# qope/starky-bn254

Hardware: AMD Instinct MI355X
Metric: G1 scalar-mult proofs/sec at trace height 2^16 (higher is better)
Workload: dtype u64

## Files before the change

starky_bn254_amd/csrc/kernels.cuh:

```cuda
#pragma once
#include "poseidon.cuh"
#include "air.cuh"

#include "kernels_ntt.cuh"

__global__ void pow_table_kernel(u64* out, size_t n, u64 base) {
  size_t i = (size_t)blockIdx.x * blockDim.x + threadIdx.x;
  if (i < n) out[i] = f_pow(F(base), i).v;
}
__global__ void shift_odd_table_kernel(u64* out, size_t n, const u64* __restrict__ shift, const u64* __restrict__ tw, u32 log_s) {
  size_t i = (size_t)blockIdx.x * blockDim.x + threadIdx.x;
  if (i < n) out[i] = (F(shift[i]) * F(tw[(i >> log_s) << log_s])).v;
}
__global__ void scale_pow_kernel(u64* v, size_t n, u64 base) {
  size_t i = (size_t)blockIdx.x * blockDim.x + threadIdx.x;
  if (i < n) v[i] = (F(v[i]) * f_pow(F(base), i)).v;
}

__global__ __launch_bounds__(256) __attribute__((amdgpu_waves_per_eu(4))) void leaf_hash_kernel(const u64* __restrict__ lde, size_t m, u32 lde_log, u32 ncols,
                                                        u64* __restrict__ digests) {
  size_t row = (size_t)blockIdx.x * blockDim.x + threadIdx.x;
  if (row >= m) return;
  F s[12];
#pragma unroll
  for (int i = 0; i < 12; i++) s[i] = F(0);
  size_t leaf = bitrev32((u32)row, lde_log);
  if (ncols <= 4) {
    for (u32 c = 0; c < 4; c++) digests[leaf * 4 + c] = c < ncols ? lde[(size_t)c * m + row] : 0;
    return;
  }
  for (u32 c = 0; c < ncols; c += 8) {
#pragma unroll
    for (u32 i = 0; i < 8; i++)
      if (c + i < ncols) s[i] = F(lde[(size_t)(c + i) * m + row]);
    poseidon_permute_keep(s, c + 8 >= ncols ? P_KEEP_DIGEST : (c + 16 <= ncols ? P_KEEP_CAPACITY : P_KEEP_ALL));
  }
#pragma unroll
  for (int i = 0; i < 4; i++) digests[leaf * 4 + i] = s[i].v;
}

__global__ __launch_bounds__(256) void merkle_level_kernel(const u64* __restrict__ child, u64* __restrict__ parent, size_t nparent) {
  size_t i = (size_t)blockIdx.x * blockDim.x + threadIdx.x;
  if (i >= nparent) return;
  F s[12];
#pragma unroll
  for (int k = 0; k < 8; k++) s[k] = F(child[i * 8 + k]);
#pragma unroll
  for (int k = 8; k < 12; k++) s[k] = F(0);
  poseidon_permute_keep(s, P_KEEP_DIGEST);
#pragma unroll
  for (int k = 0; k < 4; k++) parent[i * 4 + k] = s[k].v;
}

__global__ __launch_bounds__(256) __attribute__((amdgpu_waves_per_eu(4))) void leaf_absorb_kernel(const u64* __restrict__ lde_chunk, size_t m, u32 lde_log, u32 ncols_chunk,
                                                          u64* __restrict__ state, int first, int last, u64* __restrict__ digests, int next_full) {
  size_t row = (size_t)blockIdx.x * blockDim.x + threadIdx.x;
  if (row >= m) return;
  F s[12];
#pragma unroll
  for (int i = 0; i < 12; i++) s[i] = F(0);
  if (!first) {
#pragma unroll
    for (int i = 8; i < 12; i++) s[i] = F(state[(size_t)i * m + row]);
    if (ncols_chunk < 8) {
#pragma unroll
      for (int i = 0; i < 8; i++) s[i] = F(state[(size_t)i * m + row]);
    }
  }
  for (u32 c = 0; c < ncols_chunk; c += 8) {
#pragma unroll
    for (u32 i = 0; i < 8; i++)
      if (c + i < ncols_chunk) s[i] = F(lde_chunk[(size_t)(c + i) * m + row]);
    const bool end = c + 8 >= ncols_chunk;
    const int keep = end ? (last ? P_KEEP_DIGEST : (next_full ? P_KEEP_CAPACITY : P_KEEP_ALL)) : (c + 16 <= ncols_chunk ? P_KEEP_CAPACITY : P_KEEP_ALL);
    poseidon_permute_keep(s, keep);
  }
  u32 tid = threadIdx.x;
  asm volatile("" : "+v"(tid));
  const size_t row2 = (size_t)blockIdx.x * blockDim.x + tid;
  if (last) {
    size_t leaf = bitrev32((u32)row2, lde_log);
#pragma unroll
    for (int i = 0; i < 4; i++) digests[leaf * 4 + i] = s[i].v;
  } else {
#pragma unroll
    for (int i = 8; i < 12; i++) state[(size_t)i * m + row2] = s[i].v;
    if (!next_full) {
#pragma unroll
      for (int i = 0; i < 8; i++) state[(size_t)i * m + row2] = s[i].v;
    }
  }
}

static constexpr u32 MERKLE_SUBTREE_THREADS = 256;
__global__ __launch_bounds__(MERKLE_SUBTREE_THREADS) void merkle_subtree_kernel(u64* __restrict__ tree, size_t nleaf, u32 l0, u32 nlev, u32 nchild) {
  __shared__ u64 buf[2 * 256 * 4];
  const u32 tid = threadIdx.x, nt = blockDim.x;
  const u64* child = tree + (2 * nleaf - ((2 * nleaf) >> l0)) * 4;
  size_t base = (size_t)blockIdx.x * nchild;
  for (u32 e = tid; e < nchild * 4; e += nt) buf[e] = child[base * 4 + e];
  __syncthreads();
  u32 active = nchild / 2;
  const u32 groups = nt / 16, grp = tid / 16, lane = tid & 15;
  for (u32 lv = 1; lv <= nlev; lv++) {
    u64* out = tree + (2 * nleaf - ((2 * nleaf) >> (l0 + lv))) * 4;
    const size_t idx0 = ((size_t)blockIdx.x * nchild) >> lv;
    if (active > 4 * groups) {
      F s[12];
      if (tid < active) {
#pragma unroll
        for (int k = 0; k < 8; k++) s[k] = F(buf[tid * 8 + k]);
#pragma unroll
        for (int k = 8; k < 12; k++) s[k] = F(0);
        poseidon_permute_keep(s, P_KEEP_DIGEST);
      }
      __syncthreads();
      if (tid < active) {
#pragma unroll
        for (int k = 0; k < 4; k++) { buf[tid * 4 + k] = s[k].v; out[(idx0 + tid) * 4 + k] = s[k].v; }
      }
      __syncthreads();
    } else {
      u64 res[4];
      u32 nit = (active + groups - 1) / groups;
      for (u32 it = 0; it < nit; it++) {
        u32 parent = it * groups + grp;
        if (it * groups + (tid / 64) * 4 >= active) break;
        const u32 e = lane < 12 ? lane : lane - 12;
        u64 v = (parent < active && e < 8) ? buf[parent * 8 + e] : 0;
        res[it] = poseidon_permute_coop16(v, lane);
      }
      __syncthreads();
      for (u32 it = 0; it < nit; it++) {
        u32 parent = it * groups + grp;
        if (parent < active && lane < 4) { buf[parent * 4 + lane] = res[it]; out[(idx0 + parent) * 4 + lane] = res[it]; }
      }
      __syncthreads();
    }
    active >>= 1;
  }
}

__global__ __launch_bounds__(256) void merkle_level_thread_kernel(u64* __restrict__ tree, size_t nleaf, u32 l) {
  const size_t parents = nleaf >> (l + 1);
  const size_t i = (size_t)blockIdx.x * blockDim.x + threadIdx.x;
  if (i >= parents) return;
  const u64* child = tree + (2 * nleaf - ((2 * nleaf) >> l)) * 4;
  u64* out = tree + (2 * nleaf - ((2 * nleaf) >> (l + 1))) * 4;
  F s[12];
#pragma unroll
  for (int k = 0; k < 8; k++) s[k] = F(child[i * 8 + k]);
#pragma unroll
  for (int k = 8; k < 12; k++) s[k] = F(0);
  poseidon_permute_keep(s, P_KEEP_DIGEST);
#pragma unroll
  for (int k = 0; k < 4; k++) out[i * 4 + k] = s[k].v;
}
__global__ __launch_bounds__(256) void merkle_level_coop_kernel(u64* __restrict__ tree, size_t nleaf, u32 l) {
  const size_t parents = nleaf >> (l + 1);
  const size_t parent = ((size_t)blockIdx.x * blockDim.x + threadIdx.x) >> 4;
  const u32 lane = threadIdx.x & 15, e = lane < 12 ? lane : lane - 12;
  const u64* child = tree + (2 * nleaf - ((2 * nleaf) >> l)) * 4;
  u64* out = tree + (2 * nleaf - ((2 * nleaf) >> (l + 1))) * 4;
  const u64 v = (parent < parents && e < 8) ? child[parent * 8 + e] : 0;
  const u64 r = poseidon_permute_coop16(v, lane);
  if (parent < parents && lane < 4) out[parent * 4 + lane] = r;
}

__global__ __launch_bounds__(256) void fri_leaf_hash_kernel(const u64* __restrict__ va, const u64* __restrict__ vb, u32 log_m, u32 arity_bits,
                                                            u64* __restrict__ digests) {
  size_t leaf = (size_t)blockIdx.x * blockDim.x + threadIdx.x;
  size_t nleaf = (size_t)1 << (log_m - arity_bits);
  if (leaf >= nleaf) return;
  if (arity_bits == 1) {
    const u32 n0 = bitrev32((u32)(leaf * 2), log_m), n1 = bitrev32((u32)(leaf * 2 + 1), log_m);
    digests[leaf * 4 + 0] = va[n0]; digests[leaf * 4 + 1] = vb[n0]; digests[leaf * 4 + 2] = va[n1]; digests[leaf * 4 + 3] = vb[n1];
    return;
  }
  F s[12];
#pragma unroll
  for (int i = 0; i < 12; i++) s[i] = F(0);
  u32 arity = 1u << arity_bits;
  for (u32 t = 0; t < arity; t += 4) {
#pragma unroll
    for (u32 u = 0; u < 4; u++) {
      u32 nat = bitrev32((u32)(leaf * arity + t + u), log_m);
      s[2 * u] = F(va[nat]); s[2 * u + 1] = F(vb[nat]);
    }
    poseidon_permute_keep(s, t + 4 >= arity ? P_KEEP_DIGEST : P_KEEP_CAPACITY);
  }
#pragma unroll
  for (int i = 0; i < 4; i++) digests[leaf * 4 + i] = s[i].v;
}

__global__ __launch_bounds__(256) void fri_leaf_hash_coop_kernel(const u64* __restrict__ va, const u64* __restrict__ vb, u32 log_m, u32 arity_bits,
                                                                 u64* __restrict__ digests) {
  const size_t leaf = ((size_t)blockIdx.x * blockDim.x + threadIdx.x) >> 4;
  const size_t nleaf = (size_t)1 << (log_m - arity_bits);
  const u32 lane = threadIdx.x & 15, e = lane < 12 ? lane : lane - 12;
  const u32 arity = 1u << arity_bits;
  if (arity_bits == 1) {
    if (leaf < nleaf && lane < 4) {
      const u32 nat = bitrev32((u32)(leaf * 2 + (lane >> 1)), log_m);
      digests[leaf * 4 + lane] = (lane & 1) ? vb[nat] : va[nat];
    }
    return;
  }
  u64 st = 0;
  for (u32 t = 0; t < arity; t += 4) {
    if (leaf < nleaf && e < 8) {
      const u32 nat = bitrev32((u32)(leaf * arity + t + (e >> 1)), log_m);
      st = (e & 1) ? vb[nat] : va[nat];
    }
    st = poseidon_permute_coop16(st, lane);
  }
  if (leaf < nleaf && lane < 4) digests[leaf * 4 + lane] = st;
}

__global__ void field_mul_batch_kernel(const u64* a, const u64* b, u64* out, size_t count, int mode) {
  size_t i = (size_t)blockIdx.x * blockDim.x + threadIdx.x;
  if (i >= count) return;
#if defined(__HIP_DEVICE_COMPILE__)
  out[i] = mode ? nw::canon(nw::canon(nw::mul(a[i], b[i]))) : (F(a[i]) * F(b[i])).v;
#endif
}
__global__ void poseidon_batch_kernel(u64* states, size_t count) {
  size_t i = (size_t)blockIdx.x * blockDim.x + threadIdx.x;
  if (i >= count) return;
  F s[12];
  for (int k = 0; k < 12; k++) s[k] = F(states[i * 12 + k]);
  poseidon_permute(s);
  for (int k = 0; k < 12; k++) states[i * 12 + k] = s[k].v;
}

struct PairCols { int lhs, rhs; };

__device__ __forceinline__ F wave_scan_mul(F x, int lane) {
#pragma unroll
  for (int d = 1; d < 64; d <<= 1) {
    u64 o = __shfl_up((unsigned long long)x.v, d, 64);
    if (lane >= d) x = x * F(o);
  }
  return x;
}

template <int PZ_E>
__global__ __launch_bounds__(256) void permutation_z_kernel(const u64* __restrict__ trace, size_t n, const PairCols* __restrict__ pairs,
                                                            u64 gamma0, u64 gamma1, u64* __restrict__ zout) {
  __shared__ u64 wtot[4];
  __shared__ u64 carry_s;
  const int z = blockIdx.x;
  const u64* lhs = trace + (size_t)pairs[z].lhs * n;
  const u64* rhs = trace + (size_t)pairs[z].rhs * n;
  u64* zc = zout + (size_t)z * n;
  const int tid = threadIdx.x, lane = tid & 63, wv = tid >> 6;
  const F g0(gamma0), g1(gamma1);
  F carry(1), dprod(1);
  for (size_t base = 0; base < n; base += 256 * PZ_E) {
    const size_t i0 = base + (size_t)tid * PZ_E;
    u64 lv[PZ_E], rv[PZ_E];
#pragma unroll
    for (int e = 0; e < PZ_E; e++) { lv[e] = lhs[i0 + e]; rv[e] = rhs[i0 + e]; }
    F pr[PZ_E];
#pragma unroll
    for (int e = 0; e < PZ_E; e++) {
      const F l(lv[e]), r(rv[e]);
      const F num = (l + g0) * (l + g1);
      pr[e] = e ? pr[e - 1] * num : num;
      dprod = dprod * ((r + g0) * (r + g1));
    }
    F inc = wave_scan_mul(pr[PZ_E - 1], lane);
    if (lane == 63) wtot[wv] = inc.v;
    __syncthreads();
    F pre = carry;
    for (int w = 0; w < wv; w++) pre = pre * F(wtot[w]);
    const u64 prev = __shfl_up((unsigned long long)inc.v, 1, 64);
    const F excl = lane == 0 ? pre : pre * F(prev);
    zc[i0] = excl.v;
#pragma unroll
    for (int e = 1; e < PZ_E; e++) zc[i0 + e] = (excl * pr[e - 1]).v;
    carry = carry * F(wtot[0]) * F(wtot[1]) * F(wtot[2]) * F(wtot[3]);
    __syncthreads();
  }
  {
    F w = dprod;
#pragma unroll
    for (int d = 32; d >= 1; d >>= 1) w = w * F(__shfl_xor((unsigned long long)w.v, d, 64));
    if (lane == 0) wtot[wv] = w.v;
    __syncthreads();
    if (tid == 0) carry_s = f_inv(F(wtot[0]) * F(wtot[1]) * F(wtot[2]) * F(wtot[3])).v;
    __syncthreads();
  }
  carry = F(carry_s);
  __syncthreads();
  for (size_t base = n; base > 0; base -= 256 * PZ_E) {
    const size_t i0 = base - 1 - (size_t)tid * PZ_E;
    u64 rv[PZ_E], zv[PZ_E];
#pragma unroll
    for (int e = 0; e < PZ_E; e++) { rv[e] = rhs[i0 - e]; zv[e] = zc[i0 - e]; }
    F pr[PZ_E];
#pragma unroll
    for (int e = 0; e < PZ_E; e++) {
      const F r(rv[e]);
      const F den = (r + g0) * (r + g1);
      pr[e] = e ? pr[e - 1] * den : den;
    }
    F inc = wave_scan_mul(pr[PZ_E - 1], lane);
    if (lane == 63) wtot[wv] = inc.v;
    __syncthreads();
    F pre = carry;
    for (int w = 0; w < wv; w++) pre = pre * F(wtot[w]);
    const u64 prev = __shfl_up((unsigned long long)inc.v, 1, 64);
    const F excl = lane == 0 ? pre : pre * F(prev);
#pragma unroll
    for (int e = 0; e < PZ_E; e++) zc[i0 - e] = (F(zv[e]) * (excl * pr[e])).v;
    carry = carry * F(wtot[0]) * F(wtot[1]) * F(wtot[2]) * F(wtot[3]);
    __syncthreads();
  }
}

#include "kernels_quotient.cuh"
__global__ __launch_bounds__(256) void quotient_combine_kernel(QuotientParams p) {
  size_t i = (size_t)blockIdx.x * blockDim.x + threadIdx.x;
  if (i >= p.m) return;
  F dinv(p.zh_inv[((i << p.row_shift) | p.row_rho) & 1]);
#pragma unroll
  for (int j = 0; j < SBN_NCH; j++) {
    F acc(p.part[((size_t)(QSEG - 1) * SBN_NCH + j) * p.m + i]);
#pragma unroll
    for (u32 sgm = 0; sgm + 1 < QSEG; sgm++) acc += F(p.part[((size_t)sgm * SBN_NCH + j) * p.m + i]) * F(p.seg_shift[sgm][j]);
    p.qout[(size_t)j * p.m + i] = (acc * dinv).v;
  }
}

__global__ void domain_tables_kernel(u64* xs, u64* lag_first, u64* lag_last, size_t m, u32 lde_log, u32 degree_bits) {
  size_t i = (size_t)blockIdx.x * blockDim.x + threadIdx.x;
  if (i >= m) return;
  F w = f_root_of_unity(lde_log);
  F x = F(GL_GEN) * f_pow(w, i);
  F g = f_root_of_unity(degree_bits);
  F nn = F((u64)1 << degree_bits);
  F zx = f_exp_pow2(x, degree_bits) - F(1);
  xs[i] = x.v;
  lag_first[i] = (zx * f_inv(nn * (x - F(1)))).v;
  lag_last[i] = (zx * f_inv(nn * (g * x - F(1)))).v;
}

__device__ __forceinline__ F wave_scan_mul_rev(F x, int lane) {
#pragma unroll
  for (int d = 1; d < 64; d <<= 1) {
    u64 o = __shfl_down((unsigned long long)x.v, d, 64);
    if (lane + d < 64) x = x * F(o);
  }
  return x;
}
template <int PZ_E>
__global__ __launch_bounds__(256) void permz_chunk_products_kernel(const u64* __restrict__ trace, size_t n, const PairCols* __restrict__ pairs, u64 gamma0, u64 gamma1,
                                                                   u64* __restrict__ tot) {
  __shared__ u64 wn[4], wd[4];
  const int z = blockIdx.y;
  const size_t c = blockIdx.x, chunks = gridDim.x;
  const int tid = threadIdx.x, lane = tid & 63, wv = tid >> 6;
  const size_t i0 = c * 256 * PZ_E + (size_t)tid * PZ_E;
  const u64* lhs = trace + (size_t)pairs[z].lhs * n + i0;
  const u64* rhs = trace + (size_t)pairs[z].rhs * n + i0;
  const F g0(gamma0), g1(gamma1);
  u64 lv[PZ_E], rv[PZ_E];
#pragma unroll
  for (int e = 0; e < PZ_E; e++) { lv[e] = lhs[e]; rv[e] = rhs[e]; }
  F pn(1), pd(1);
#pragma unroll
  for (int e = 0; e < PZ_E; e++) { const F l(lv[e]), r(rv[e]); pn = pn * ((l + g0) * (l + g1)); pd = pd * ((r + g0) * (r + g1)); }
#pragma unroll
  for (int d = 32; d >= 1; d >>= 1) { pn = pn * F(__shfl_xor((unsigned long long)pn.v, d, 64)); pd = pd * F(__shfl_xor((unsigned long long)pd.v, d, 64)); }
  if (lane == 0) { wn[wv] = pn.v; wd[wv] = pd.v; }
  __syncthreads();
  if (tid == 0) {
    tot[((size_t)z * chunks + c) * 2] = (F(wn[0]) * F(wn[1]) * F(wn[2]) * F(wn[3])).v;
    tot[((size_t)z * chunks + c) * 2 + 1] = (F(wd[0]) * F(wd[1]) * F(wd[2]) * F(wd[3])).v;
  }
}
__global__ __launch_bounds__(64) void permz_chunk_scan_kernel(const u64* __restrict__ tot, u32 chunks, u64* __restrict__ pq) {
  const int z = blockIdx.x, lane = threadIdx.x;
  const u64* t = tot + (size_t)z * chunks * 2;
  u64* o = pq + (size_t)z * chunks * 2;
  F carry(1), all(1);
  for (u32 b = 0; b < chunks; b += 64) {
    const u32 idx = b + lane;
    const bool on = idx < chunks;
    const F inc = wave_scan_mul(on ? F(t[2 * idx]) : F(1), lane);
    const u64 pv = __shfl_up((unsigned long long)inc.v, 1, 64);
    if (on) o[2 * idx] = (lane == 0 ? carry : carry * F(pv)).v;
    carry = carry * F(__shfl((unsigned long long)inc.v, 63, 64));
    F d = on ? F(t[2 * idx + 1]) : F(1);
#pragma unroll
    for (int k = 32; k >= 1; k >>= 1) d = d * F(__shfl_xor((unsigned long long)d.v, k, 64));
    all = all * d;
  }
  F carry_s = f_inv(all);
  for (u32 b = ((chunks - 1) / 64) * 64;; b -= 64) {
    const u32 idx = b + lane;
    const bool on = idx < chunks;
    const F inc = wave_scan_mul_rev(on ? F(t[2 * idx + 1]) : F(1), lane);
    const u64 sv = __shfl_down((unsigned long long)inc.v, 1, 64);
    if (on) o[2 * idx + 1] = (lane == 63 ? carry_s : carry_s * F(sv)).v;
    carry_s = carry_s * F(__shfl((unsigned long long)inc.v, 0, 64));
    if (b == 0) break;
  }
}
template <int PZ_E>
__global__ __launch_bounds__(256) void permz_chunk_write_kernel(const u64* __restrict__ trace, size_t n, const PairCols* __restrict__ pairs, u64 gamma0, u64 gamma1,
                                                                const u64* __restrict__ pq, u64* __restrict__ zout) {
  __shared__ u64 wn[4], wd[4];
  const int z = blockIdx.y;
  const size_t c = blockIdx.x, chunks = gridDim.x;
  const int tid = threadIdx.x, lane = tid & 63, wv = tid >> 6;
  const size_t i0 = c * 256 * PZ_E + (size_t)tid * PZ_E;
  const u64* lhs = trace + (size_t)pairs[z].lhs * n + i0;
  const u64* rhs = trace + (size_t)pairs[z].rhs * n + i0;
  u64* zc = zout + (size_t)z * n + i0;
  const F g0(gamma0), g1(gamma1);
  u64 lv[PZ_E], rv[PZ_E];
#pragma unroll
  for (int e = 0; e < PZ_E; e++) { lv[e] = lhs[e]; rv[e] = rhs[e]; }
  F pn[PZ_E], sd[PZ_E];
#pragma unroll
  for (int e = 0; e < PZ_E; e++) { const F l(lv[e]); const F num = (l + g0) * (l + g1); pn[e] = e ? pn[e - 1] * num : num; }
#pragma unroll
  for (int e = PZ_E - 1; e >= 0; e--) { const F r(rv[e]); const F den = (r + g0) * (r + g1); sd[e] = e < PZ_E - 1 ? sd[e + 1] * den : den; }
  const F incn = wave_scan_mul(pn[PZ_E - 1], lane), incd = wave_scan_mul_rev(sd[0], lane);
  if (lane == 63) wn[wv] = incn.v;
  if (lane == 0) wd[wv] = incd.v;
  __syncthreads();
  F pre(pq[((size_t)z * chunks + c) * 2]), suf(pq[((size_t)z * chunks + c) * 2 + 1]);
  for (int w = 0; w < wv; w++) pre = pre * F(wn[w]);
  for (int w = 3; w > wv; w--) suf = suf * F(wd[w]);
  const u64 pv = __shfl_up((unsigned long long)incn.v, 1, 64), sv = __shfl_down((unsigned long long)incd.v, 1, 64);
  const F exn = lane == 0 ? pre : pre * F(pv);
  const F exd = lane == 63 ? suf : suf * F(sv);
  const F both = exn * exd;
  zc[0] = (both * sd[0]).v;
#pragma unroll
  for (int e = 1; e < PZ_E; e++) zc[e] = (both * pn[e - 1] * sd[e]).v;
}

__global__ void ext_pow_table_kernel(u64* pa, u64* pb, size_t n, u64 z0, u64 z1) {
  size_t i = (size_t)blockIdx.x * blockDim.x + threadIdx.x;
  if (i >= n) return;
  E2 r = e2_pow(E2(F(z0), F(z1)), i);
  pa[i] = r.a.v; pb[i] = r.b.v;
}
__device__ __forceinline__ F block_sum(F v, u64* sh) {
  const int lane = threadIdx.x & 63, wv = threadIdx.x >> 6;
#pragma unroll
  for (int d = 32; d >= 1; d >>= 1) v = v + F(__shfl_xor((unsigned long long)v.v, d, 64));
  __syncthreads();
  if (lane == 0) sh[wv] = v.v;
  __syncthreads();
  F t(0);
  for (unsigned w = 0; w < blockDim.x / 64; w++) t = t + F(sh[w]);
  return t;
}
template <u32 OPEN_UNROLL>
__global__ __launch_bounds__(256) void openings_kernel(const u64* __restrict__ coeffs, size_t n, const u64* __restrict__ pa0, const u64* __restrict__ pb0,
                                                       const u64* __restrict__ pa1, const u64* __restrict__ pb1, u64* __restrict__ out) {
  __shared__ u64 sh[4];
  const u64* c = coeffs + (size_t)blockIdx.x * n;
  Acc<F> s0, r0, s1, r1;
  s0.clear(); r0.clear(); s1.clear(); r1.clear();
  for (size_t i = threadIdx.x; i < n; i += 256 * OPEN_UNROLL) {
    u64 cv[OPEN_UNROLL], t0[OPEN_UNROLL], t1[OPEN_UNROLL], t2[OPEN_UNROLL], t3[OPEN_UNROLL];
#pragma unroll
    for (u32 k = 0; k < OPEN_UNROLL; k++) {
      const size_t ik = i + 256 * k;
      cv[k] = c[ik]; t0[k] = pa0[ik]; t1[k] = pb0[ik]; t2[k] = pa1[ik]; t3[k] = pb1[ik];
    }
    __builtin_amdgcn_sched_barrier(0);
#pragma unroll
    for (u32 k = 0; k < OPEN_UNROLL; k++) {
      const F v{cv[k]};
      s0.macv(v, F(t0[k])); r0.macv(v, F(t1[k]));
      s1.macv(v, F(t2[k])); r1.macv(v, F(t3[k]));
    }
  }
  const F a0 = block_sum(s0.value(), sh), b0 = block_sum(r0.value(), sh), a1 = block_sum(s1.value(), sh), b1 = block_sum(r1.value(), sh);
  if (threadIdx.x == 0) {
    u64* o = out + (size_t)blockIdx.x * 4;
    o[0] = a0.v; o[1] = b0.v; o[2] = a1.v; o[3] = b1.v;
  }
}

template <u32 OPEN_UNROLL>
__global__ __launch_bounds__(256) void openings1_kernel(const u64* __restrict__ coeffs, size_t n, const u64* __restrict__ pa, const u64* __restrict__ pb,
                                                        u64* __restrict__ out, u32 off) {
  __shared__ u64 sh[4];
  const u64* c = coeffs + (size_t)blockIdx.x * n;
  Acc<F> s0, r0;
  s0.clear(); r0.clear();
  for (size_t i = threadIdx.x; i < n; i += 256 * OPEN_UNROLL) {
    u64 cv[OPEN_UNROLL], t0[OPEN_UNROLL], t1[OPEN_UNROLL];
#pragma unroll
    for (u32 k = 0; k < OPEN_UNROLL; k++) {
      const size_t ik = i + 256 * k;
      cv[k] = c[ik]; t0[k] = pa[ik]; t1[k] = pb[ik];
    }
    __builtin_amdgcn_sched_barrier(0);
#pragma unroll
    for (u32 k = 0; k < OPEN_UNROLL; k++) {
      const F v{cv[k]};
      s0.macv(v, F(t0[k])); r0.macv(v, F(t1[k]));
    }
  }
  const F a0 = block_sum(s0.value(), sh), b0 = block_sum(r0.value(), sh);
  if (threadIdx.x == 0) {
    u64* o = out + (size_t)blockIdx.x * 4 + off;
    o[0] = a0.v; o[1] = b0.v;
  }
}

__global__ __launch_bounds__(256) void fri_combine_partial_kernel(const u64* __restrict__ coeffs, size_t n, u32 npoly, u32 group_size,
                                                                  const u64* __restrict__ pa, const u64* __restrict__ pb, u64* __restrict__ part_a,
                                                                  u64* __restrict__ part_b) {
  size_t i = (size_t)blockIdx.x * blockDim.x + threadIdx.x;
  if (i >= n) return;
  const u32 g = blockIdx.y;
  const u32 j0 = g * group_size, cnt = j0 + group_size < npoly ? group_size : npoly - j0;
  const u64* c = coeffs + (size_t)j0 * n + i;
  Acc<F> a, b;
  a.clear(); b.clear();
  u32 k = 0;
  for (; k + 8 <= cnt; k += 8) {
    u64 f[8];
#pragma unroll
    for (u32 u = 0; u < 8; u++) f[u] = c[(size_t)(k + u) * n];
#pragma unroll
    for (u32 u = 0; u < 8; u++) { const F v(f[u]); a.mac(v, F(pa[k + u])); b.mac(v, F(pb[k + u])); }
  }
  for (; k < cnt; k++) { const F v(c[(size_t)k * n]); a.mac(v, F(pa[k])); b.mac(v, F(pb[k])); }
  part_a[(size_t)g * n + i] = a.value().v; part_b[(size_t)g * n + i] = b.value().v;
}
__global__ void fri_combine_reduce_kernel(const u64* part_a, const u64* part_b, size_t n, u32 ngroups, const u64* w, u64* out_a, u64* out_b, int accumulate) {
  size_t i = (size_t)blockIdx.x * blockDim.x + threadIdx.x;
  if (i >= n) return;
  E2 acc = accumulate ? E2(F(out_a[i]), F(out_b[i])) : E2(F(0), F(0));
  for (u32 g = 0; g < ngroups; g++) acc += E2(F(part_a[(size_t)g * n + i]), F(part_b[(size_t)g * n + i])) * E2(F(w[2 * g]), F(w[2 * g + 1]));
  out_a[i] = acc.a.v; out_b[i] = acc.b.v;
}

static constexpr u32 DBL_CHUNK = 16;
__global__ __launch_bounds__(256) void divide_by_linear_pass1(const u64* __restrict__ ca, const u64* __restrict__ cb, size_t nchunks, u64 z0, u64 z1,
                                                              u64* __restrict__ ha, u64* __restrict__ hb) {
  const size_t t = (size_t)blockIdx.x * blockDim.x + threadIdx.x;
  if (t >= nchunks) return;
  const E2 z{F(z0), F(z1)};
  const size_t s = t * DBL_CHUNK;
  E2 h{F(0), F(0)};
  for (u32 k = DBL_CHUNK; k-- > 0;) h = h * z + E2(F(ca[s + k]), F(cb[s + k]));
  ha[t] = h.a.v; hb[t] = h.b.v;
}
template <u32 U> __device__ __forceinline__ void dbl_fold(const u64* ha, const u64* hb, size_t base, size_t per, const E2 zl, E2& g) {
  for (size_t j0 = per; j0 > 0; j0 -= U) {
    u64 va[U], vb[U];
#pragma unroll
    for (u32 k = 0; k < U; k++) { va[k] = ha[base + j0 - 1 - k]; vb[k] = hb[base + j0 - 1 - k]; }
#pragma unroll
    for (u32 k = 0; k < U; k++) g = E2(F(va[k]), F(vb[k])) + zl * g;
  }
}
template <u32 U> __device__ __forceinline__ void dbl_replay(u64* ha, u64* hb, size_t base, size_t per, const E2 zl, E2 carry) {
  for (size_t j0 = per; j0 > 0; j0 -= U) {
    u64 va[U], vb[U];
#pragma unroll
    for (u32 k = 0; k < U; k++) { va[k] = ha[base + j0 - 1 - k]; vb[k] = hb[base + j0 - 1 - k]; }
#pragma unroll
    for (u32 k = 0; k < U; k++) {
      ha[base + j0 - 1 - k] = carry.a.v; hb[base + j0 - 1 - k] = carry.b.v;
      carry = E2(F(va[k]), F(vb[k])) + zl * carry;
    }
  }
}
__global__ __launch_bounds__(256) void divide_by_linear_pass2(u64* __restrict__ ha, u64* __restrict__ hb, size_t nchunks, u64 z0, u64 z1) {
  __shared__ u64 sa[2][256], sb[2][256];
  const int tid = threadIdx.x;
  const int lanes = nchunks < 256 ? (int)nchunks : 256;
  const size_t per = nchunks / lanes, base = (size_t)tid * per;
  const bool live = tid < lanes;
  const E2 zl = e2_pow(E2{F(z0), F(z1)}, DBL_CHUNK);
  E2 g{F(0), F(0)};
  if (live) { if (per % 8 == 0) dbl_fold<8>(ha, hb, base, per, zl, g); else dbl_fold<1>(ha, hb, base, per, zl, g); }
  E2 m = e2_pow(zl, per);
  int cur = 0;
  sa[0][tid] = g.a.v; sb[0][tid] = g.b.v;
  __syncthreads();
  for (int d = 1; d < lanes; d <<= 1) {
    E2 v{F(sa[cur][tid]), F(sb[cur][tid])};
    if (tid + d < lanes) v = v + m * E2(F(sa[cur][tid + d]), F(sb[cur][tid + d]));
    sa[cur ^ 1][tid] = v.a.v; sb[cur ^ 1][tid] = v.b.v;
    m = m * m;
    cur ^= 1;
    __syncthreads();
  }
  E2 carry{F(0), F(0)};
  if (tid + 1 < lanes) carry = E2(F(sa[cur][tid + 1]), F(sb[cur][tid + 1]));
  if (live) { if (per % 8 == 0) dbl_replay<8>(ha, hb, base, per, zl, carry); else dbl_replay<1>(ha, hb, base, per, zl, carry); }
}
__global__ __launch_bounds__(256) void divide_by_linear_pass3(const u64* __restrict__ ca, const u64* __restrict__ cb, size_t nchunks, u64 z0, u64 z1,
                                                              const u64* __restrict__ ha, const u64* __restrict__ hb, u64 mul0, u64 mul1,
                                                              u64* __restrict__ oa, u64* __restrict__ ob, int accumulate, u32 times_x) {
  const size_t t = (size_t)blockIdx.x * blockDim.x + threadIdx.x;
  if (t >= nchunks) return;
  const E2 z{F(z0), F(z1)}, mul{F(mul0), F(mul1)};
  const size_t s = t * DBL_CHUNK, n = nchunks * DBL_CHUNK;
  E2 b{F(ha[t]), F(hb[t])};
  for (u32 k = DBL_CHUNK; k-- > 0;) {
    const size_t i = s + k;
    const E2 q = b;
    b = b * z + E2(F(ca[i]), F(cb[i]));
    const size_t j = i + times_x;
    if (j >= n) continue;
    const E2 o = accumulate ? E2(F(oa[j]), F(ob[j])) * mul + q : q;
    oa[j] = o.a.v; ob[j] = o.b.v;
  }
}

__global__ void fri_fold_kernel(const u64* ca, const u64* cb, size_t nout, u32 arity, u64 b0, u64 b1, u64* oa, u64* ob) {
  size_t i = (size_t)blockIdx.x * blockDim.x + threadIdx.x;
  if (i >= nout) return;
  E2 beta{F(b0), F(b1)}, acc(F(0), F(0));
  for (u32 t = arity; t-- > 0;) acc = acc * beta + E2(F(ca[i * arity + t]), F(cb[i * arity + t]));
  oa[i] = acc.a.v; ob[i] = acc.b.v;
}

struct PowParams { u64 state[12]; u32 wpos; u32 min_lz; u64 base; u64 count; u64* result; };
__global__ __launch_bounds__(256) void pow_kernel(PowParams p) {
  u64 gid = (u64)blockIdx.x * blockDim.x + threadIdx.x;
  if (gid >= p.count) return;
  F s[12];
#pragma unroll
  for (int i = 0; i < 12; i++) s[i] = F(p.state[i]);
  s[p.wpos] = F(p.base + gid);
  poseidon_permute(s);
  u64 resp = s[P_RATE - 1].v;
  u32 lz = resp ? (u32)__clzll((long long)resp) : 64;
  if (lz >= p.min_lz) atomicMin((unsigned long long*)p.result, (unsigned long long)(p.base + gid));
}

__global__ __launch_bounds__(256) void split_pack_kernel(const u64* __restrict__ lde, size_t m, u32 nc, u32 ob, u32 log_r, u32 me,
                                                         u64* __restrict__ send_l, u64* __restrict__ send_n, u64* __restrict__ self_l, u64* __restrict__ self_n) {
  const size_t i = (size_t)blockIdx.x * blockDim.x + threadIdx.x;
  const u32 c = blockIdx.y;
  if (i >= m || c >= nc) return;
  const u64 v = lde[(size_t)c * m + i];
  const size_t ml = m >> log_r, rmask = ((size_t)1 << log_r) - 1;
  const u32 s = bitrev32((u32)(i & rmask), log_r);
  if (s == me) self_l[(size_t)c * ml + (i >> log_r)] = v;
  else send_l[((size_t)s * ob + c) * ml + (i >> log_r)] = v;
  if (send_n) {
    const size_t p = (i + m - 2) & (m - 1);
    const u32 s2 = bitrev32((u32)(p & rmask), log_r);
    if (s2 == me) self_n[(size_t)c * ml + (p >> log_r)] = v;
    else send_n[((size_t)s2 * ob + c) * ml + (p >> log_r)] = v;
  }
}
__global__ void split_unpack_rows_kernel(const u64* __restrict__ in, size_t m, u32 nplanes, u32 log_r, u64* __restrict__ out) {
  const size_t i = (size_t)blockIdx.x * blockDim.x + threadIdx.x;
  if (i >= m) return;
  const size_t ml = m >> log_r;
  const u32 s = bitrev32((u32)(i & (((size_t)1 << log_r) - 1)), log_r);
  for (u32 p = 0; p < nplanes; p++) out[(size_t)p * m + i] = in[((size_t)s * nplanes + p) * ml + (i >> log_r)];
}
__global__ void split_modadd_kernel(const u64* __restrict__ in, size_t len, u32 nranks, u64* __restrict__ out) {
  const size_t k = (size_t)blockIdx.x * blockDim.x + threadIdx.x;
  if (k >= len) return;
  F acc(in[k]);
  for (u32 r = 1; r < nranks; r++) acc += F(in[(size_t)r * len + k]);
  out[k] = acc.v;
}

__global__ void gather_rows_kernel(const u64* mat, size_t m, u32 lde_log, u32 ncols, const u32* idx, u64* out, size_t qstride, size_t off) {
  u32 c = blockIdx.x * blockDim.x + threadIdx.x;
  u32 q = blockIdx.y;
  if (c >= ncols) return;
  size_t row = bitrev32(idx[q], lde_log);
  out[(size_t)q * qstride + off + c] = mat[(size_t)c * m + row];
}
__global__ void gather_siblings_kernel(const u64* tree, size_t nleaf, u32 nlevels, const u32* idx, u32 shift, u64* out, size_t qstride, size_t off) {
  u32 q = blockIdx.x;
  u32 e = threadIdx.x;
  if (e >= nlevels * 4) return;
  u32 l = e >> 2, k = e & 3;
  size_t x = idx[q] >> shift;
  size_t level_off = 2 * nleaf - ((2 * nleaf) >> l);
  size_t sib = (x >> l) ^ 1;
  out[(size_t)q * qstride + off + e] = tree[(level_off + sib) * 4 + k];
}
__global__ void gather_fri_leaf_kernel(const u64* va, const u64* vb, u32 log_m, u32 arity_bits, const u32* idx, u32 shift, u64* out, size_t qstride, size_t off) {
  u32 q = blockIdx.x;
  u32 e = threadIdx.x;
  u32 arity = 1u << arity_bits;
  if (e >= 2 * arity) return;
  size_t leaf = idx[q] >> shift;
  u32 nat = bitrev32((u32)(leaf * arity + (e >> 1)), log_m);
  out[(size_t)q * qstride + off + e] = (e & 1) ? vb[nat] : va[nat];
}

typedef unsigned long long u64x2_t __attribute__((ext_vector_type(2)));
__global__ __launch_bounds__(256) void first_non_canonical_kernel(const u64* __restrict__ w, size_t count, u64 base, unsigned long long* first_bad) {
  const size_t head = (((size_t)w & 8) && count) ? 1 : 0;
  const u64x2_t* __restrict__ v = reinterpret_cast<const u64x2_t*>(w + head);
  const size_t nvec = (count - head) >> 1;
  const size_t tid = (size_t)blockIdx.x * blockDim.x + threadIdx.x, stride = (size_t)gridDim.x * blockDim.x;
  u64 bad = ~(u64)0;
#pragma unroll 4
  for (size_t i = tid; i < nvec; i += stride) {
    const u64x2_t x = v[i];
    const bool b0 = x.x >= GLP, b1 = x.y >= GLP;
    if (b0 | b1) { const u64 j = head + 2 * i + (b0 ? 0 : 1); bad = bad < j ? bad : j; }
  }
  if (tid == 0) {
    const size_t last = head + 2 * nvec;
    if (last < count && w[last] >= GLP) bad = bad < last ? bad : last;
    if (head && w[0] >= GLP) bad = 0;
  }
  if (!__any(bad != ~(u64)0)) return;
  for (int d = 32; d >= 1; d >>= 1) { const u64 o = __shfl_xor((unsigned long long)bad, d, 64); bad = o < bad ? o : bad; }
  if ((threadIdx.x & 63) == 0) atomicMin(first_bad, (unsigned long long)(base + bad));
}
```

starky_bn254_amd/csrc/kernels_ntt.cuh:

```cuda
#pragma once
#include "gl.cuh"

struct NttPassParams {
  const u64* in; u64* out;
  size_t in_col_stride, out_col_stride;
  u32 log_r;
  u32 log_t;
  u32 log_n;
  size_t in_sr, in_st, out_sr, out_st;
  size_t n_in;
  u32 r_fast_load;
  u32 twiddle;
  const u64* tw;
  u32 tw_log;
  const u64* pre;
  const u64* post;
  u64 scale;
  const u64* pre2;
  u32 split;
  u32 xcd_order;
};

GL_HD F tw_lookup(const u64* tw, u32 tw_log, u64 e_of_order, u32 order_log) {
  u64 idx = (e_of_order << (tw_log - order_log)) & ((1ULL << tw_log) - 1);
  u64 half = 1ULL << (tw_log - 1);
  if (idx >= half) return -F(tw[idx - half]);
  return F(tw[idx]);
}

__device__ __forceinline__ u64 tw_full(const u64* __restrict__ tw, u32 tw_log, u32 e_of_order, u32 order_log) {
  return tw[(e_of_order << (tw_log - order_log)) & ((1u << tw_log) - 1u)];
}

static constexpr int NTT_THREADS = 256;

#ifdef SBN_NTT_KERNELS_HERE
__global__ __launch_bounds__(NTT_THREADS) void ntt_pass_kernel(NttPassParams p) {
  extern __shared__ u64 lds[];
  const u32 R = 1u << p.log_r, T = 1u << p.log_t;
  const u32 LDT = T + 1;
  const size_t col = blockIdx.y;
  const size_t t0 = (size_t)blockIdx.x << p.log_t;
  const u64* in = p.in + col * p.in_col_stride;
  u64* out = p.out + col * p.out_col_stride;
  const u32 total = R << p.log_t;
  for (u32 e = threadIdx.x; e < total; e += NTT_THREADS) {
    u32 r, t;
    if (p.r_fast_load) { r = e & (R - 1); t = e >> p.log_r; } else { t = e & (T - 1); r = e >> p.log_t; }
    size_t gi = (size_t)r * p.in_sr + (t0 + t) * p.in_st;
    u64 v = 0;
    if (gi < p.n_in) {
      v = in[gi];
      if (p.pre) v = (F(v) * F(p.pre[gi])).v;
    }
    lds[r * LDT + t] = v;
  }
  __syncthreads();
  for (u32 s = 0; s < p.log_r; s++) {
    u32 half = R >> (s + 1);
    u32 nb = total >> 1;
    for (u32 e = threadIdx.x; e < nb; e += NTT_THREADS) {
      u32 t = e & (T - 1), b = e >> p.log_t;
      u32 j = b & (half - 1), blk = b / half;
      u32 i0 = blk * 2 * half + j, i1 = i0 + half;
      F u{lds[i0 * LDT + t]}, v(lds[i1 * LDT + t]);
      F w = tw_lookup(p.tw, p.tw_log, (u64)j << s, p.log_r);
      lds[i0 * LDT + t] = (u + v).v;
      lds[i1 * LDT + t] = ((u - v) * w).v;
    }
    __syncthreads();
  }
  for (u32 e = threadIdx.x; e < total; e += NTT_THREADS) {
    u32 t = e & (T - 1), k = e >> p.log_t;
    u32 q = bitrev32(k, p.log_r);
    F v{lds[q * LDT + t]};
    if (p.twiddle) v = v * tw_lookup(p.tw, p.tw_log, (u64)k * (t0 + t), p.log_n);
    if (p.scale != 1) v = v * F(p.scale);
    size_t go = (size_t)k * p.out_sr + (t0 + t) * p.out_st;
    if (p.post) v = v * F(p.post[go]);
    out[go] = v.v;
  }
}
#else
__global__ void ntt_pass_kernel(NttPassParams p);
#endif

namespace nw {
#if !defined(SBN_NTT_CXX_ARITH)
using namespace gp;
__device__ __forceinline__ u64 repay_carry(u64 s, u64 k) { u64 k2, k3; u64 t = madm1(sel01(k), s, k2); return madm1(sel01(k2), t, k3); }
__device__ __forceinline__ u64 add(u64 a, u64 b) {
  u64 k1, k2; u32 lo = addco(lo32(a), lo32(b), k1); u32 hi = addc(hi32(a), hi32(b), k1, k2);
  return repay_carry(pack(lo, hi), k2);
}
__device__ __forceinline__ u64 sub(u64 a, u64 b) {
  u64 k1, k2, k3, k4, k5, k6;
  u32 lo = subco(lo32(a), lo32(b), k1); u32 hi = subb(hi32(a), hi32(b), k1, k2);
  u32 l2 = subco(lo, selm1(k2), k3); u32 h2 = subb0(hi, k3, k4);
  u32 l3 = subco(l2, selm1(k4), k5); u32 h3 = subb0(h2, k5, k6);
  return pack(l3, h3);
}
__device__ __forceinline__ u64 red32(u64 lo, u32 hi) { u64 k; u64 t = madm1(hi, lo, k); u64 k2; return madm1(sel01(k), t, k2); }
__device__ __forceinline__ u64 red(u64 lo, u64 hi) {
  u64 k1, k2, k3, k4, k5, k6;
  const u32 l = subco(lo32(lo), hi32(hi), k1), h = subb0(hi32(lo), k1, k2);
  const u32 t = subb0(lo32(hi), k2, k3);
  const u64 r = madm1(t, pack(l, h), k4);
  const u32 rl = addc(lo32(r), selm1(k4), k3, k5), rh = addc(hi32(r), 0u, k5, k6);
  return pack(rl, rh);
}
template <int E> __device__ __forceinline__ u64 mul_pow2(u64 x) {
  if constexpr (E == 0) return x;
  else if constexpr (E < 32) return red32(x << E, hi32(x) >> (32 - E));
  else if constexpr (E == 32) return red32(pack(0, lo32(x)), hi32(x));
  else if constexpr (E < 64) return red(pack(0, lo32(x) << (E - 32)), x >> (64 - E));
  else return mul_pow2<E - 48>(mul_pow2<48>(x));
}
__device__ __forceinline__ u64 mul(u64 a, u64 b) { return gl_mul_weak(a, b); }
__device__ __forceinline__ u64 canon(u64 x) { return gp::canon(x); }
#else
__device__ __forceinline__ u64 add(u64 a, u64 b) {
  u64 s = a + b;
  u64 c = s < a ? GLEPS : 0;
  s += c;
  if (s < c) s += GLEPS;
  return s;
}
__device__ __forceinline__ u64 sub(u64 a, u64 b) {
  u64 d = a - b;
  u64 c = a < b ? GLEPS : 0;
  u64 r = d - c;
  if (d < c) r -= GLEPS;
  return r;
}
__device__ __forceinline__ u64 red(u64 lo, u64 hi) {
  u32 hi_hi = (u32)(hi >> 32), hi_lo = (u32)hi;
  u64 t0 = lo - hi_hi;
  if (lo < hi_hi) t0 -= GLEPS;
  u64 t1 = ((u64)hi_lo << 32) - hi_lo;
  u64 r = t0 + t1;
  if (r < t1) r += GLEPS;
  return r;
}
template <int E> __device__ __forceinline__ u64 mul_pow2(u64 x) {
  if constexpr (E == 0) return x;
  else if constexpr (E < 64) return red(x << E, x >> (64 - E));
  else return mul_pow2<E - 48>(mul_pow2<48>(x));
}
__device__ __forceinline__ u64 mul(u64 a, u64 b) { return red(a * b, __umul64hi(a, b)); }
__device__ __forceinline__ u64 canon(u64 x) { return x >= GLP ? x - GLP : x; }
#endif

#define NW_BF(i, j, E) { u64 a_ = x[i], b_ = x[j]; x[i] = add(a_, b_); x[j] = mul_pow2<E>(sub(a_, b_)); }
__device__ __forceinline__ void dft16_rho(u64* x) {
  NW_BF(0, 8, 0) NW_BF(1, 9, 12) NW_BF(2, 10, 24) NW_BF(3, 11, 36) NW_BF(4, 12, 48) NW_BF(5, 13, 60) NW_BF(6, 14, 72) NW_BF(7, 15, 84)
  NW_BF(0, 4, 0) NW_BF(1, 5, 24) NW_BF(2, 6, 48) NW_BF(3, 7, 72) NW_BF(8, 12, 0) NW_BF(9, 13, 24) NW_BF(10, 14, 48) NW_BF(11, 15, 72)
  NW_BF(0, 2, 0) NW_BF(1, 3, 48) NW_BF(4, 6, 0) NW_BF(5, 7, 48) NW_BF(8, 10, 0) NW_BF(9, 11, 48) NW_BF(12, 14, 0) NW_BF(13, 15, 48)
  NW_BF(0, 1, 0) NW_BF(2, 3, 0) NW_BF(4, 5, 0) NW_BF(6, 7, 0) NW_BF(8, 9, 0) NW_BF(10, 11, 0) NW_BF(12, 13, 0) NW_BF(14, 15, 0)
}
#undef NW_BF
}

#ifdef SBN_NTT_KERNELS_HERE
template <int LOG_B>
__global__ __launch_bounds__(256) void ntt_fast_pass_kernel(NttPassParams p, u32 kperm) {
  extern __shared__ u64 lds[];
  constexpr u32 NB = 1u << LOG_B;
  constexpr u32 R = 256u << LOG_B;
  const size_t col = p.xcd_order ? blockIdx.x : blockIdx.y;
  const size_t t0 = (size_t)(p.xcd_order ? blockIdx.y : blockIdx.x) << 4;
  const u32 half = p.split ? blockIdx.z : 0u;
  const u64* __restrict__ pre = half ? p.pre2 : p.pre;
  const u64* in = p.in + col * p.in_col_stride;
  u64* out = p.out + col * p.out_col_stride;
  u32 g, t;
  if (p.r_fast_load) { g = threadIdx.x & 15; t = threadIdx.x >> 4; } else { t = threadIdx.x & 15; g = threadIdx.x >> 4; }
  const size_t tg = t0 + t;
  const u32 S1 = p.r_fast_load ? 257u : 272u;
  const u32 lane_off = p.r_fast_load ? (t * 16) : t;
  const u32 g_mul = p.r_fast_load ? 1u : 16u;
  u64 x[NB][16];
#pragma unroll
  for (u32 b = 0; b < NB; b++)
#pragma unroll
    for (u32 q = 0; q < 16; q++) {
      u32 r = g + 16 * q + 256 * b;
      size_t gi = (size_t)r * p.in_sr + tg * p.in_st;
      u64 v = 0;
      if (gi < p.n_in) {
        v = in[gi];
        if (pre) v = nw::mul(v, pre[gi]);
      }
      x[b][q] = v;
    }
  if (LOG_B == 1) {
    const bool upper_zero = p.in_st == 1 && (size_t)256 * p.in_sr >= p.n_in;
#pragma unroll
    for (u32 q = 0; q < 16; q++) {
      u32 r = g + 16 * q;
      u64 a = x[0][q], bb = x[NB - 1][q];
      u64 w = tw_full(p.tw, p.tw_log, r, 9);
      if (upper_zero) { x[NB - 1][q] = nw::mul(a, w); }
      else { x[0][q] = nw::add(a, bb); x[NB - 1][q] = nw::mul(nw::sub(a, bb), w); }
    }
  }
#pragma unroll
  for (u32 b = 0; b < NB; b++) {
    nw::dft16_rho(x[b]);
#pragma unroll
    for (u32 pidx = 0; pidx < 16; pidx++) {
      u32 m = __brev(pidx) >> 28;
      u32 k1 = (kperm * m) & 15;
      u64 v = x[b][pidx];
      if (g && k1) v = nw::mul(v, tw_full(p.tw, p.tw_log, (u32)(g * k1), 8));
      lds[(b * 16 + k1) * S1 + lane_off + g * g_mul] = v;
    }
  }
  __syncthreads();
  const u32 k1 = g;
#pragma unroll
  for (u32 b = 0; b < NB; b++) {
#pragma unroll
    for (u32 gp = 0; gp < 16; gp++) x[b][gp] = lds[(b * 16 + k1) * S1 + lane_off + gp * g_mul];
    nw::dft16_rho(x[b]);
#pragma unroll
    for (u32 pidx = 0; pidx < 16; pidx++) {
      u32 m = __brev(pidx) >> 28;
      u32 k2 = (kperm * m) & 15;
      u32 k256 = k1 + 16 * k2;
      u32 k = LOG_B == 0 ? k256 : (k256 * NB + b);
      if (LOG_B == 1) k = (k << p.split) + half;
      u64 v = x[b][pidx];
      if (p.twiddle) v = nw::mul(v, tw_full(p.tw, p.tw_log, (u32)(k * tg), p.log_n));
      if (p.scale != 1) v = nw::mul(v, p.scale);
      size_t go = (size_t)k * p.out_sr + tg * p.out_st;
      if (p.post) v = nw::mul(v, p.post[go]);
      out[go] = nw::canon(v);
    }
  }
  (void)R;
}
#else
template <int LOG_B> __global__ void ntt_fast_pass_kernel(NttPassParams p, u32 kperm);
#endif

struct NttFusedParams {
  const u64* in; size_t in_col_stride;
  u64* coef; size_t coef_col_stride;
  u64* out; size_t out_col_stride;
  size_t n1;
  u32 log_n;
  const u64* tw_i; const u64* tw_f; u32 tw_log;
  const u64* pre;
  u64 scale;
  const u64* pre2;
};
#ifdef SBN_NTT_KERNELS_HERE
__global__ __launch_bounds__(256) __attribute__((amdgpu_waves_per_eu(4))) void ntt_fused_inv_b_lde_a_kernel(NttFusedParams p) {
  extern __shared__ u64 lds[];
  const size_t col = blockIdx.x;
  const size_t t0 = (size_t)blockIdx.y << 4;
  const u64* in = p.in + col * p.in_col_stride;
  u64* coef = p.coef + col * p.coef_col_stride;
  u64* out = p.out + col * p.out_col_stride;
  const u32 g = threadIdx.x & 15, t = threadIdx.x >> 4;
  const size_t tg = t0 + t;
  u64 x[2][16];
#pragma unroll
  for (u32 q = 0; q < 16; q++) x[0][q] = in[(size_t)(g + 16 * q) + tg * 256];
  nw::dft16_rho(x[0]);
#pragma unroll
  for (u32 pidx = 0; pidx < 16; pidx++) {
    const u32 m = __brev(pidx) >> 28, k1 = (11u * m) & 15;
    u64 v = x[0][pidx];
    if (g && k1) v = nw::mul(v, tw_full(p.tw_i, p.tw_log, (u32)(g * k1), 8));
    lds[k1 * 257 + t * 16 + g] = v;
  }
  __syncthreads();
#pragma unroll
  for (u32 gp = 0; gp < 16; gp++) x[0][gp] = lds[g * 257 + t * 16 + gp];
  nw::dft16_rho(x[0]);
  u64 a[16];
#pragma unroll
  for (u32 pidx = 0; pidx < 16; pidx++) {
    const u32 m = __brev(pidx) >> 28, k2 = (11u * m) & 15;
    const u32 k = g + 16 * k2;
    const u64 v = nw::mul(x[0][pidx], p.scale);
    coef[(size_t)k * p.n1 + tg] = nw::canon(v);
    a[k2] = v;
  }
  __syncthreads();
#pragma unroll
  for (u32 q = 0; q < 16; q++) {
    const u32 r = g + 16 * q;
    const u64 v = nw::mul(a[q], p.pre[(size_t)r * p.n1 + tg]);
    x[0][q] = v;
    x[1][q] = nw::mul(v, tw_full(p.tw_f, p.tw_log, r, 9));
  }
#pragma unroll
  for (u32 b = 0; b < 2; b++) {
    nw::dft16_rho(x[b]);
#pragma unroll
    for (u32 pidx = 0; pidx < 16; pidx++) {
      const u32 m = __brev(pidx) >> 28, k1 = (5u * m) & 15;
      u64 v = x[b][pidx];
      if (g && k1) v = nw::mul(v, tw_full(p.tw_f, p.tw_log, (u32)(g * k1), 8));
      lds[(b * 16 + k1) * 272 + g * 17 + t] = v;
    }
  }
  __syncthreads();
  const u32 t2 = threadIdx.x & 15, k1o = threadIdx.x >> 4;
  const size_t tg2 = t0 + t2;
#pragma unroll
  for (u32 b = 0; b < 2; b++) {
#pragma unroll
    for (u32 gp = 0; gp < 16; gp++) x[b][gp] = lds[(b * 16 + k1o) * 272 + gp * 17 + t2];
    nw::dft16_rho(x[b]);
#pragma unroll
    for (u32 pidx = 0; pidx < 16; pidx++) {
      const u32 m = __brev(pidx) >> 28, k2 = (5u * m) & 15;
      const u32 k = (k1o + 16 * k2) * 2 + b;
      const u64 v = nw::mul(x[b][pidx], tw_full(p.tw_f, p.tw_log, (u32)(k * tg2), p.log_n + 1));
      out[(size_t)k * p.n1 + tg2] = nw::canon(v);
    }
  }
}
#else
__global__ void ntt_fused_inv_b_lde_a_kernel(NttFusedParams p);
#endif

#ifdef SBN_NTT_KERNELS_HERE
__global__ __launch_bounds__(256) __attribute__((amdgpu_waves_per_eu(4))) void ntt_fused512_inv_b_lde_a_kernel(NttFusedParams p) {
  extern __shared__ u64 lds[];
  const size_t col = blockIdx.x;
  const size_t t0 = (size_t)blockIdx.y << 4;
  const u64* in = p.in + col * p.in_col_stride;
  u64* coef = p.coef + col * p.coef_col_stride;
  u64* out = p.out + col * p.out_col_stride;
  const u32 g = threadIdx.x & 15, t = threadIdx.x >> 4;
  const size_t tg = t0 + t;
  u64 x[2][16];
#pragma unroll
  for (u32 q0 = 0; q0 < 16; q0 += 8) {
#pragma unroll
    for (u32 q = q0; q < q0 + 8; q++) {
      const u64 lo = in[(size_t)(g + 16 * q) + tg * 512], hi = in[(size_t)(g + 16 * q + 256) + tg * 512];
      x[0][q] = nw::add(lo, hi);
      x[1][q] = nw::mul(nw::sub(lo, hi), tw_full(p.tw_i, p.tw_log, g + 16 * q, 9));
    }
    asm volatile("" ::: "memory");
  }
#pragma unroll
  for (u32 b = 0; b < 2; b++) {
    nw::dft16_rho(x[b]);
#pragma unroll
    for (u32 pidx = 0; pidx < 16; pidx++) {
      const u32 m = __brev(pidx) >> 28, k1 = (11u * m) & 15;
      u64 v = x[b][pidx];
      if (g && k1) v = nw::mul(v, tw_full(p.tw_i, p.tw_log, (u32)(g * k1), 8));
      lds[(b * 16 + k1) * 257 + t * 16 + g] = v;
    }
  }
  __syncthreads();
#pragma unroll
  for (u32 b = 0; b < 2; b++) {
    u64 z[16];
#pragma unroll
    for (u32 gp = 0; gp < 16; gp++) z[gp] = lds[(b * 16 + g) * 257 + t * 16 + gp];
    nw::dft16_rho(z);
#pragma unroll
    for (u32 pidx = 0; pidx < 16; pidx++) {
      const u32 m = __brev(pidx) >> 28, k2 = (11u * m) & 15;
      const u64 v = nw::mul(z[pidx], p.scale);
      coef[(size_t)((g + 16 * k2) * 2 + b) * 512 + tg] = nw::canon(v);
      x[b][k2] = v;
    }
    asm volatile("" ::: "memory");
  }
  __syncthreads();
#pragma unroll 1
  for (u32 h = 0; h < 2; h++) {
    u32 t2 = threadIdx.x & 15, k1o = threadIdx.x >> 4;
    u32 gl = g, tl = t;
    asm volatile("" : "+v"(t2), "+v"(k1o), "+v"(gl), "+v"(tl));
    const size_t tg2 = t0 + t2, tgl = t0 + tl;
    const u64* __restrict__ pre = h ? p.pre2 : p.pre;
#pragma unroll
    for (u32 b = 0; b < 2; b++)
#pragma unroll
      for (u32 q0 = 0; q0 < 16; q0 += 8) {
#pragma unroll
        for (u32 q = q0; q < q0 + 8; q++) {
          const size_t ci = (size_t)(2 * (gl + 16 * q) + b) * 512 + tgl;
          u64 c = x[b][q];
          if (h) c = coef[ci];
          x[b][q] = nw::mul(c, pre[ci]);
        }
        asm volatile("" ::: "memory");
      }
#pragma unroll
    for (u32 b = 0; b < 2; b++) {
      nw::dft16_rho(x[b]);
#pragma unroll
      for (u32 pidx = 0; pidx < 16; pidx++) {
        const u32 m = __brev(pidx) >> 28, k1 = (5u * m) & 15;
        u64 v = x[b][pidx];
        if (gl && k1) v = nw::mul(v, tw_full(p.tw_f, p.tw_log, (u32)(gl * k1), 8));
        lds[(b * 16 + k1) * 272 + gl * 17 + tl] = v;
      }
    }
    __syncthreads();
#pragma unroll
    for (u32 b = 0; b < 2; b++) {
#pragma unroll
      for (u32 gp = 0; gp < 16; gp++) x[b][gp] = lds[(b * 16 + k1o) * 272 + gp * 17 + t2];
      nw::dft16_rho(x[b]);
    }
#pragma unroll
    for (u32 pidx = 0; pidx < 16; pidx++) {
      const u32 m = __brev(pidx) >> 28, k2 = (5u * m) & 15;
      const u32 j = k1o + 16 * k2;
      const u64 e = x[0][pidx], o = nw::mul(x[1][pidx], tw_full(p.tw_f, p.tw_log, j, 9));
      const u32 ka = 2 * j + h, kb = 2 * (j + 256) + h;
      out[(size_t)ka * 512 + tg2] = nw::canon(nw::mul(nw::add(e, o), tw_full(p.tw_f, p.tw_log, (u32)(ka * tg2), 19)));
      out[(size_t)kb * 512 + tg2] = nw::canon(nw::mul(nw::sub(e, o), tw_full(p.tw_f, p.tw_log, (u32)(kb * tg2), 19)));
    }
    __syncthreads();
  }
}
#else
__global__ void ntt_fused512_inv_b_lde_a_kernel(NttFusedParams p);
#endif
```

starky_bn254_amd/csrc/prover.hip:

```cpp
#include "prover_ctx.hpp"
#include "kernels.cuh"
#include <algorithm>
#include <cstring>
#include <cstdlib>
#include <thread>
#include <atomic>
#include <chrono>
#include <functional>

namespace sbn { thread_local std::string g_last_error; }

static std::atomic<int> g_default_device{0};
static thread_local int t_device = -1;
static inline int cur_device() { return t_device >= 0 ? t_device : g_default_device.load(); }
#define g_device (cur_device())
namespace sbn {
int current_device() { return cur_device(); }
int use_current_device(const char* why) {
  int ndev = 0;
  if (hipGetDeviceCount(&ndev) != hipSuccess || ndev == 0) return fail(SBN_ERR_NO_DEVICE, "no HIP device available: %s", why);
  HIPC(hipSetDevice(g_device));
  return 0;
}
}

static const char* STAGE_NAMES[ST_COUNT + EX_COUNT] = {
  "trace_commit", "perm_z", "z_commit", "quotient_eval", "quotient_commit",
  "openings", "fri_combine", "fri_layers", "pow", "queries",
  "trace_absorb_kernels_ms", "trace_absorb_launches", "z_absorb_kernels_ms", "z_absorb_launches", "device_tracegen_ms",
  "split_exchange_ms"};

static int dmalloc(u64** p, size_t words, size_t* bytes = nullptr) {
  HIPC(hipMalloc((void**)p, words * sizeof(u64)));
  if (bytes) *bytes += words * sizeof(u64);
  return 0;
}

static u32 pick_log_t(u32 log_r, u32 log_s) {
  u32 lt = 4;
  while (lt > 0 && ((size_t)(1u << log_r) * ((1u << lt) + 1) * 8) > 48 * 1024) lt--;
  return std::min(lt, log_s);
}
static int ntt_columns(sbn_prover* P, const u64* in, size_t in_cs, u64* out, size_t out_cs, u64* tmp, size_t tmp_cs, size_t ncols,
                       u32 log_n, bool inverse, size_t n_in, const u64* pre, const u64* post, u64 scale, hipStream_t st = nullptr, int which = 3) {
  if (ncols == 0) return 0;
  if (!st) st = P->stream;
  u32 log_n1 = (log_n + 1) / 2, log_n2 = log_n - log_n1;
  size_t n1 = (size_t)1 << log_n1, n2 = (size_t)1 << log_n2;
  NttPassParams a{};
  a.in = in; a.out = tmp; a.in_col_stride = in_cs; a.out_col_stride = tmp_cs;
  a.log_r = log_n1; a.log_t = pick_log_t(log_n1, log_n2); a.log_n = log_n;
  a.in_sr = n2; a.in_st = 1; a.out_sr = n2; a.out_st = 1; a.n_in = n_in;
  a.r_fast_load = 0; a.twiddle = 1; a.tw = inverse ? P->d_tw_i : P->d_tw_f; a.tw_log = P->lde_log;
  a.pre = pre; a.post = nullptr; a.scale = 1;
  NttPassParams b{};
  b.in = tmp; b.out = out; b.in_col_stride = tmp_cs; b.out_col_stride = out_cs;
  b.log_r = log_n2; b.log_t = pick_log_t(log_n2, log_n1); b.log_n = log_n;
  b.in_sr = 1; b.in_st = n2; b.out_sr = n1; b.out_st = 1; b.n_in = (size_t)1 << log_n;
  b.r_fast_load = 1; b.twiddle = 0; b.tw = a.tw; b.tw_log = P->lde_log;
  b.pre = nullptr; b.post = post; b.scale = scale;
  for (size_t c0 = 0; c0 < ncols; c0 += 32768) {
    size_t nc = std::min<size_t>(32768, ncols - c0);
    NttPassParams pa = a, pb = b;
    pa.in = a.in + c0 * in_cs; pa.out = a.out + c0 * tmp_cs;
    pb.in = b.in + c0 * tmp_cs; pb.out = b.out + c0 * out_cs;
    dim3 ga((unsigned)(n2 >> pa.log_t), (unsigned)nc), gb((unsigned)(n1 >> pb.log_t), (unsigned)nc);
    size_t la = ((size_t)1 << pa.log_r) * ((1u << pa.log_t) + 1) * 8, lb = ((size_t)1 << pb.log_r) * ((1u << pb.log_t) + 1) * 8;
    const u32 kperm = inverse ? 11u : 5u;
    auto launch = [&](NttPassParams q, dim3 grid, size_t lds_bytes) {
      const bool fast = q.log_t == 4 && (q.log_r == 8 || q.log_r == 9);
      if (fast) { q.xcd_order = 1; std::swap(grid.x, grid.y); }
      if (fast && q.log_r == 8) hipLaunchKernelGGL(ntt_fast_pass_kernel<0>, grid, dim3(256), 16 * 272 * 8, st, q, kperm);
      else if (fast) hipLaunchKernelGGL(ntt_fast_pass_kernel<1>, grid, dim3(256), 32 * 272 * 8, st, q, kperm);
      else hipLaunchKernelGGL(ntt_pass_kernel, grid, dim3(NTT_THREADS), lds_bytes, st, q);
    };
    if (pa.log_r == 9 && log_n2 >= 4) pa.log_t = 4;
    if (pb.log_r == 9 && log_n1 >= 4) pb.log_t = 4;
    const bool split_a = !inverse && pa.log_r == 10 && log_n2 >= 4 && pa.in_st == 1 && n_in <= (size_t)512 * pa.in_sr && pre == P->d_shift && P->d_shift_odd;
    if (split_a) { pa.log_r = 9; pa.log_t = 4; pa.split = 1; pa.pre2 = P->d_shift_odd; }
    ga = dim3((unsigned)(n2 >> pa.log_t), (unsigned)nc, split_a ? 2u : 1u); gb = dim3((unsigned)(n1 >> pb.log_t), (unsigned)nc);
    la = ((size_t)1 << pa.log_r) * ((1u << pa.log_t) + 1) * 8; lb = ((size_t)1 << pb.log_r) * ((1u << pb.log_t) + 1) * 8;
    if (which & 1) launch(pa, ga, la);
    if (which & 2) launch(pb, gb, lb);
  }
  HIPC(hipGetLastError());
  return 0;
}

static u64 host_inv_pow2(u32 k) { return f_inv(F((u64)1 << k)).v; }
static int ntt_fast_setup() {
  static std::atomic<bool> done[SBN_MAX_DEVICES];
  const int d = g_device >= 0 && g_device < SBN_MAX_DEVICES ? g_device : 0;
  if (!done[d].load()) {
    HIPC(hipFuncSetAttribute((const void*)ntt_fast_pass_kernel<1>, hipFuncAttributeMaxDynamicSharedMemorySize, 32 * 272 * 8));
    HIPC(hipFuncSetAttribute((const void*)ntt_fused_inv_b_lde_a_kernel, hipFuncAttributeMaxDynamicSharedMemorySize, 32 * 272 * 8));
    HIPC(hipFuncSetAttribute((const void*)ntt_fused512_inv_b_lde_a_kernel, hipFuncAttributeMaxDynamicSharedMemorySize, 32 * 272 * 8));
    done[d].store(true);
  }
  return 0;
}
static void ntt_plan(sbn_prover* P) {
  P->ntt_fused = P->degree_bits == 16 || P->degree_bits == 17;
  P->ntt_fused512 = P->degree_bits == 18 && P->lde_log == 19;
}

static int intt_values(sbn_prover* P, const u64* vals, u64* coef, size_t ncols) {
  for (size_t c0 = 0; c0 < ncols; c0 += P->ntt_chunk) {
    size_t nc = std::min(P->ntt_chunk, ncols - c0);
    int rc = ntt_columns(P, vals + c0 * P->n, P->n, coef + c0 * P->n, P->n, P->d_tmp, P->m, nc, P->degree_bits, true, P->n, nullptr, nullptr,
                         host_inv_pow2(P->degree_bits));
    if (rc) return rc;
  }
  return 0;
}
static int lde_coeffs(sbn_prover* P, const u64* coef, u64* lde, size_t ncols) {
  for (size_t c0 = 0; c0 < ncols; c0 += P->ntt_chunk) {
    size_t nc = std::min(P->ntt_chunk, ncols - c0);
    int rc = ntt_columns(P, coef + c0 * P->n, P->n, lde + c0 * P->m, P->m, P->d_tmp, P->m, nc, P->lde_log, false, P->n, P->d_shift, nullptr, 1);
    if (rc) return rc;
  }
  return 0;
}
static int intt_then_lde(sbn_prover* P, const u64* vals, u64* coef, u64* lde, size_t ncols) {
  for (size_t c0 = 0; c0 < ncols; c0 += P->ntt_chunk) {
    size_t nc = std::min(P->ntt_chunk, ncols - c0);
    int rc = ntt_columns(P, vals + c0 * P->n, P->n, coef + c0 * P->n, P->n, P->d_tmp, P->m, nc, P->degree_bits, true, P->n, nullptr, nullptr,
                         host_inv_pow2(P->degree_bits));
    if (rc) return rc;
    rc = ntt_columns(P, coef + c0 * P->n, P->n, lde + c0 * P->m, P->m, P->d_tmp, P->m, nc, P->lde_log, false, P->n, P->d_shift, nullptr, 1);
    if (rc) return rc;
  }
  return 0;
}

static int intt_lde_cols_fused(sbn_prover* P, const u64* v, u64* cf, u64* lde_out, size_t nc, u64* tmp2, hipStream_t lde_stream, hipEvent_t handoff) {
  int rc = ntt_columns(P, v, P->n, cf, P->n, P->d_tmp, P->m, nc, P->degree_bits, true, P->n, nullptr, nullptr, host_inv_pow2(P->degree_bits), nullptr, 1);
  if (rc) return rc;
  NttFusedParams f{};
  const u32 log_n1 = (P->degree_bits + 1) / 2;
  f.in = P->d_tmp; f.in_col_stride = P->m; f.coef = cf; f.coef_col_stride = P->n; f.out = tmp2; f.out_col_stride = P->m;
  f.n1 = (size_t)1 << log_n1; f.log_n = P->degree_bits; f.tw_i = P->d_tw_i; f.tw_f = P->d_tw_f; f.tw_log = P->lde_log; f.pre = P->d_shift; f.pre2 = P->d_shift_odd;
  f.scale = host_inv_pow2(P->degree_bits);
  if (P->ntt_fused512) hipLaunchKernelGGL(ntt_fused512_inv_b_lde_a_kernel, dim3((unsigned)nc, 32u), dim3(256), 32 * 272 * 8, P->stream, f);
  else hipLaunchKernelGGL(ntt_fused_inv_b_lde_a_kernel, dim3((unsigned)nc, (unsigned)(f.n1 >> 4)), dim3(256), 32 * 272 * 8, P->stream, f);
  if (lde_stream != P->stream) {
    HIPC(hipEventRecord(handoff, P->stream));
    HIPC(hipStreamWaitEvent(lde_stream, handoff, 0));
  }
  return ntt_columns(P, cf, P->n, lde_out, P->m, tmp2, P->m, nc, P->lde_log, false, P->n, P->d_shift, nullptr, 1, lde_stream, 2);
}
static int intt_lde_cols(sbn_prover* P, const u64* v, u64* cf, u64* lde_out, size_t nc) {
  if ((P->ntt_fused || P->ntt_fused512) && P->d_tmp2) return intt_lde_cols_fused(P, v, cf, lde_out, nc, P->d_tmp2, P->stream, nullptr);
  int rc = ntt_columns(P, v, P->n, cf, P->n, P->d_tmp, P->m, nc, P->degree_bits, true, P->n, nullptr, nullptr, host_inv_pow2(P->degree_bits));
  if (rc) return rc;
  return ntt_columns(P, cf, P->n, lde_out, P->m, P->d_tmp, P->m, nc, P->lde_log, false, P->n, P->d_shift, nullptr, 1);
}

static int tree_alloc(DevTree& t, size_t nleaf, u32 cap_height, size_t* bytes = nullptr) {
  t.nleaf = nleaf;
  u32 lg = 0; while (((size_t)1 << lg) < nleaf) lg++;
  t.nlevels = lg - cap_height;
  return dmalloc(&t.d, 2 * nleaf * 4, bytes);
}
static int tree_build_inner(sbn_prover* P, DevTree& t, hipStream_t st) {
  u32 l0 = 0;
  while (l0 < t.nlevels) {
    const size_t parents = t.nleaf >> (l0 + 1);
    if (parents <= 8192 && parents >= 16 && ((t.nleaf >> l0) % 32) == 0) {
      const u32 nlev = std::min<u32>(t.nlevels - l0, 5);
      hipLaunchKernelGGL(merkle_subtree_kernel, dim3((unsigned)((t.nleaf >> l0) / 32)), dim3(MERKLE_SUBTREE_THREADS), 0, st, t.d, t.nleaf, l0, nlev, 32u);
      l0 += nlev;
      continue;
    }
    if (parents >= 16384) {
      hipLaunchKernelGGL(merkle_level_thread_kernel, dim3((unsigned)((parents + 255) / 256)), dim3(256), 0, st, t.d, t.nleaf, l0);
      l0++;
    } else if (parents > 16) {
      hipLaunchKernelGGL(merkle_level_coop_kernel, dim3((unsigned)((parents * 16 + 255) / 256)), dim3(256), 0, st, t.d, t.nleaf, l0);
      l0++;
    } else {
      const size_t nodes = t.nleaf >> l0;
      u32 nchild = (u32)std::min<size_t>(512, nodes);
      u32 lg = 0; while ((2u << lg) < nchild) lg++;
      u32 nlev = std::min(t.nlevels - l0, lg + 1);
      hipLaunchKernelGGL(merkle_subtree_kernel, dim3((unsigned)(nodes / nchild)), dim3(MERKLE_SUBTREE_THREADS), 0, st, t.d, t.nleaf, l0, nlev, nchild);
      l0 += nlev;
    }
  }
  HIPC(hipGetLastError());
  return 0;
}
static int tree_from_matrix(sbn_prover* P, DevTree& t, const u64* lde, size_t ncols) {
  hipLaunchKernelGGL(leaf_hash_kernel, dim3((unsigned)((P->m + 255) / 256)), dim3(256), 0, P->stream, lde, P->m, P->lde_log, (u32)ncols, t.d);
  return tree_build_inner(P, t, P->stream);
}
struct HostUpload { const u64* src; hipEvent_t* done; };
static int upload_setup(sbn_prover* P) {
  if (!P->ustream) HIPC(hipStreamCreate(&P->ustream));
  for (auto& e : P->upload_done) if (!e) HIPC(hipEventCreateWithFlags(&e, hipEventDisableTiming));
  for (auto& e : P->slot_copied) if (!e) HIPC(hipEventCreateWithFlags(&e, hipEventDisableTiming));
  if (!P->h_ring) HIPC(hipHostMalloc((void**)&P->h_ring, UPLOAD_SLOTS * UPLOAD_SLOT_WORDS * sizeof(u64), hipHostMallocDefault));
  if (!P->h_first_bad) HIPC(hipHostMalloc((void**)&P->h_first_bad, sizeof(unsigned long long), hipHostMallocDefault));
  if (!P->d_first_bad) { HIPC(hipMalloc((void**)&P->d_first_bad, sizeof(unsigned long long))); P->dev_bytes += sizeof(unsigned long long); }
  return 0;
}
static void launch_first_non_canonical(const u64* d_words, size_t count, u64 base, unsigned long long* d_first_bad, hipStream_t st) {
  const size_t blocks = std::min<size_t>(std::max<size_t>((count / 2 + 255) / 256, 1), 2048);
  hipLaunchKernelGGL(first_non_canonical_kernel, dim3((unsigned)blocks), dim3(256), 0, st, d_words, count, base, d_first_bad);
}
static int upload_chunk(sbn_prover* P, const HostUpload& up, size_t k, size_t c0, size_t nc) {
  const size_t w0 = c0 * P->n, w1 = w0 + nc * P->n;
  const size_t threads = std::min<size_t>(tracegen_host_threads(), 16);
  for (size_t a = w0; a < w1; a += UPLOAD_SLOT_WORDS) {
    const size_t len = std::min(UPLOAD_SLOT_WORDS, w1 - a);
    const unsigned s = P->slot_next; P->slot_next = (s + 1) % UPLOAD_SLOTS;
    if (P->slot_used[s]) HIPC(hipEventSynchronize(P->slot_copied[s]));
    u64* slot = P->h_ring + (size_t)s * UPLOAD_SLOT_WORDS;
    const u64* from = up.src + a;
    const size_t parts = std::max<size_t>(1, std::min(threads, len >> 15)), per = (len + parts - 1) / parts;
    host_parallel_for(parts, [&](size_t t) { const size_t b0 = t * per, b1 = std::min(len, b0 + per); if (b0 < b1) memcpy(slot + b0, from + b0, (b1 - b0) * sizeof(u64)); });
    HIPC(hipMemcpyAsync(P->d_trace + a, slot, len * sizeof(u64), hipMemcpyHostToDevice, P->ustream));
    HIPC(hipEventRecord(P->slot_copied[s], P->ustream));
    P->slot_used[s] = true;
  }
  launch_first_non_canonical(P->d_trace + w0, w1 - w0, (u64)w0, P->d_first_bad, P->ustream);
  HIPC(hipGetLastError());
  HIPC(hipEventRecord(up.done[k], P->ustream));
  return 0;
}

static int commit_pipeline(sbn_prover* P, const u64* vals, u64* coef, u64* lde, size_t ncols, DevTree& t, int ex_ms, int ex_launches, const HostUpload* up = nullptr) {
  size_t ch = P->ntt_chunk;
  size_t nchunks = (ncols + ch - 1) / ch;
  if (nchunks > (size_t)MAX_CHUNKS) return fail(SBN_ERR_UNSUPPORTED, "too many column chunks");
  if (ncols <= 4) {
    if (up) {
      int rc = upload_chunk(P, *up, 0, 0, ncols);
      if (rc) return rc;
      HIPC(hipStreamWaitEvent(P->stream, up->done[0], 0));
    }
    int rc = intt_then_lde(P, vals, coef, lde, ncols);
    if (rc) return rc;
    P->stage_ms[ST_COUNT + ex_launches] = 0;
    return tree_from_matrix(P, t, lde, ncols);
  }
  for (size_t k = 0; k < nchunks; k++) {
    size_t c0 = k * ch, nc = std::min(ch, ncols - c0);
    int rc;
    if (up) {
      if ((rc = upload_chunk(P, *up, k, c0, nc))) return rc;
      HIPC(hipStreamWaitEvent(P->stream, up->done[k], 0));
    }
    if (P->ntt_two_streams && (P->ntt_fused || P->ntt_fused512) && P->d_tmp3) {
      if (k >= 2) HIPC(hipStreamWaitEvent(P->stream, P->chunk_ready[k - 2], 0));
      rc = intt_lde_cols_fused(P, vals + c0 * P->n, coef + c0 * P->n, lde + c0 * P->m, nc, (k & 1) ? P->d_tmp3 : P->d_tmp2, P->nstream, P->intt_done[k]);
      if (rc) return rc;
      HIPC(hipEventRecord(P->chunk_ready[k], P->nstream));
    } else if (P->ntt_two_streams && !P->ntt_fused && !P->ntt_fused512) {
      rc = ntt_columns(P, vals + c0 * P->n, P->n, coef + c0 * P->n, P->n, P->d_tmp, P->m, nc, P->degree_bits, true, P->n, nullptr, nullptr, host_inv_pow2(P->degree_bits));
      if (rc) return rc;
      HIPC(hipEventRecord(P->intt_done[k], P->stream));
      HIPC(hipStreamWaitEvent(P->nstream, P->intt_done[k], 0));
      rc = ntt_columns(P, coef + c0 * P->n, P->n, lde + c0 * P->m, P->m, P->d_tmp2, P->m, nc, P->lde_log, false, P->n, P->d_shift, nullptr, 1, P->nstream);
      if (rc) return rc;
      HIPC(hipEventRecord(P->chunk_ready[k], P->nstream));
    } else {
      rc = intt_lde_cols(P, vals + c0 * P->n, coef + c0 * P->n, lde + c0 * P->m, nc);
      if (rc) return rc;
      HIPC(hipEventRecord(P->chunk_ready[k], P->stream));
    }
    HIPC(hipStreamWaitEvent(P->hstream, P->chunk_ready[k], 0));
    HIPC(hipEventRecord(P->abs_ev[2 * k], P->hstream));
    hipLaunchKernelGGL(leaf_absorb_kernel, dim3((unsigned)((P->m + 255) / 256)), dim3(256), 0, P->hstream, lde + c0 * P->m, P->m, P->lde_log, (u32)nc,
                       P->d_sponge, k == 0 ? 1 : 0, k + 1 == nchunks ? 1 : 0, t.d,
                       (k + 1 < nchunks && std::min(ch, ncols - (c0 + nc)) >= 8) ? 1 : 0);
    HIPC(hipEventRecord(P->abs_ev[2 * k + 1], P->hstream));
  }
  int rc = tree_build_inner(P, t, P->hstream);
  if (rc) return rc;
  HIPC(hipEventRecord(P->hash_done, P->hstream));
  HIPC(hipStreamWaitEvent(P->stream, P->hash_done, 0));
  P->stage_ms[ST_COUNT + ex_launches] = (float)nchunks;
  (void)ex_ms;
  return 0;
}
static thread_local double t_wait_deadline_s = 0;
static inline void poll_backoff(unsigned spins) {
  if (spins < 2000) std::this_thread::yield();
  else std::this_thread::sleep_for(std::chrono::microseconds(spins < 20000 ? 20 : 200));
}
static inline hipError_t stream_wait(hipStream_t st) {
  if (t_wait_deadline_s <= 0) return hipStreamSynchronize(st);
  const auto t0 = std::chrono::steady_clock::now();
  unsigned spins = 0;
  for (;;) {
    const hipError_t e = hipStreamQuery(st);
    if (e != hipErrorNotReady) return e;
    if (std::chrono::duration<double>(std::chrono::steady_clock::now() - t0).count() > t_wait_deadline_s) return hipErrorNotReady;
    poll_backoff(++spins);
  }
}
static inline hipError_t event_wait(hipEvent_t ev) {
  if (t_wait_deadline_s <= 0) return hipEventSynchronize(ev);
  const auto t0 = std::chrono::steady_clock::now();
  unsigned spins = 0;
  for (;;) {
    const hipError_t e = hipEventQuery(ev);
    if (e != hipErrorNotReady) return e;
    if (std::chrono::duration<double>(std::chrono::steady_clock::now() - t0).count() > t_wait_deadline_s) return hipErrorNotReady;
    poll_backoff(++spins);
  }
}
static int split_exchange(sbn_prover* P, hipStream_t st, const std::vector<uint64_t>& so, const std::vector<uint64_t>& sl, const std::vector<uint64_t>& ro,
                          const std::vector<uint64_t>& rl) {
  SplitCtx* S = P->sp;
  bool any = false;
  for (u32 r = 0; r < S->comm.world; r++) any = any || sl[r] || rl[r];
  if (!any) return 0;
  const bool timed = S->tev_used + 2 <= S->tev.size();
  if (timed) HIPC(hipEventRecord(S->tev[S->tev_used], st));
  const int rc = S->comm.all_to_all(S->comm.ctx, (void*)st, so.data(), sl.data(), ro.data(), rl.data());
  if (rc) return fail(SBN_ERR_HIP, "sbn_comm.all_to_all failed (%d)", rc);
  if (timed) { HIPC(hipEventRecord(S->tev[S->tev_used + 1], st)); S->tev_used += 2; }
  return 0;
}
static int split_all_gather_host(sbn_prover* P, const void* send, void* recv, size_t bytes) {
  SplitCtx* S = P->sp;
  const int rc = S->comm.all_gather_host(S->comm.ctx, send, recv, bytes);
  if (rc) return fail(SBN_ERR_HIP, "sbn_comm.all_gather_host failed (%d)", rc);
  return 0;
}
static int split_all_gather_device(sbn_prover* P, size_t words) {
  SplitCtx* S = P->sp;
  const u32 R = S->comm.world;
  if (words * R > S->scratch_words || words * sizeof(u64) > S->comm.send_bytes) return fail(SBN_ERR_HIP, "internal: split scratch too small");
  const uint64_t base = (uint64_t)((const char*)S->scratch - (const char*)S->comm.recv_buf);
  std::vector<uint64_t> so(R, 0), sl(R, words * sizeof(u64)), ro(R), rl(R, words * sizeof(u64));
  for (u32 r = 0; r < R; r++) ro[r] = base + (uint64_t)r * words * sizeof(u64);
  return split_exchange(P, P->stream, so, sl, ro, rl);
}
static int commit_split(sbn_prover* P, const ColShare& sh, const u64* vals, bool vals_global, u64* coef_own, u64* plane_l, u64* plane_n, DevTree& t) {
  SplitCtx* S = P->sp;
  const u32 R = S->comm.world, me = S->comm.rank;
  const size_t n = P->n, m = P->m, ml = S->ml, ob = sh.ob;
  const size_t steps = sh.steps();
  if (steps > (size_t)MAX_CHUNKS) return fail(SBN_ERR_UNSUPPORTED, "too many column blocks");
  const char* rbase = (const char*)S->comm.recv_buf;
  const char* sbase = (const char*)S->comm.send_buf;
  const u32 row_log = P->lde_log - S->log_r;
  for (size_t k = 0; k < steps; k++) {
    const size_t b = k * R + me, nc = sh.block_cols(b);
    hipStream_t tstream = P->stream;
    u64* const slot = (u64*)S->comm.send_buf + (k & 1) * S->slot_words;
    u64* const slot_n = S->planes == 2 ? slot + (size_t)R * ob * ml : nullptr;
    if (nc) {
      const u64* v = vals + (vals_global ? b : k) * ob * n;
      u64* cf = coef_own + k * ob * n;
      u64* lde_out = R == 1 ? plane_l + b * ob * m : S->d_ldechunk;
      const bool fused = P->ntt_fused || P->ntt_fused512;
      const bool two = P->ntt_two_streams && P->d_tmp2 && (!fused || P->d_tmp3);
      tstream = two ? P->nstream : P->stream;
      int rc;
      if (two && fused) {
        if (k >= 2) HIPC(hipStreamWaitEvent(P->stream, P->chunk_ready[k - 2], 0));
        rc = intt_lde_cols_fused(P, v, cf, lde_out, nc, (k & 1) ? P->d_tmp3 : P->d_tmp2, P->nstream, P->intt_done[k]);
      } else if (two) {
        rc = ntt_columns(P, v, n, cf, n, P->d_tmp, m, nc, P->degree_bits, true, n, nullptr, nullptr, host_inv_pow2(P->degree_bits));
        if (rc) return rc;
        HIPC(hipEventRecord(P->intt_done[k], P->stream));
        HIPC(hipStreamWaitEvent(P->nstream, P->intt_done[k], 0));
        rc = ntt_columns(P, cf, n, lde_out, m, P->d_tmp2, m, nc, P->lde_log, false, n, P->d_shift, nullptr, 1, P->nstream);
      } else rc = intt_lde_cols(P, v, cf, lde_out, nc);
      if (rc) return rc;
      if (R > 1 && k >= 2) HIPC(hipStreamWaitEvent(tstream, S->xchg_done[k - 2], 0));
      if (R > 1)
        hipLaunchKernelGGL(split_pack_kernel, dim3((unsigned)((m + 255) / 256), (unsigned)nc), dim3(256), 0, tstream, S->d_ldechunk, m, (u32)nc, (u32)ob, S->log_r, me,
                           slot, slot_n, plane_l + b * ob * ml, plane_n ? plane_n + b * ob * ml : nullptr);
      HIPC(hipGetLastError());
    }
    HIPC(hipEventRecord(P->chunk_ready[k], tstream));
    hipEvent_t arrived = P->chunk_ready[k];
    if (R > 1) {
      HIPC(hipStreamWaitEvent(S->cstream, P->chunk_ready[k], 0));
      for (u32 pl = 0; pl < S->planes; pl++) {
        const u64* dst = pl ? plane_n : plane_l;
        std::vector<uint64_t> so(R, 0), sl(R, 0), ro(R, 0), rl(R, 0);
        for (u32 r = 0; r < R; r++) {
          if (r == me) continue;
          so[r] = (uint64_t)((const char*)(slot + ((size_t)pl * R + r) * ob * ml) - sbase);
          sl[r] = (uint64_t)(nc * ml * sizeof(u64));
          const size_t br = k * R + r;
          ro[r] = (uint64_t)((const char*)(dst + br * ob * ml) - rbase);
          rl[r] = (uint64_t)(sh.block_cols(br) * ml * sizeof(u64));
        }
        int rc = split_exchange(P, S->cstream, so, sl, ro, rl);
        if (rc) return rc;
      }
      HIPC(hipEventRecord(S->xchg_done[k], S->cstream));
      arrived = S->xchg_done[k];
    }
    HIPC(hipStreamWaitEvent(P->hstream, arrived, 0));
    const size_t c_begin = k * R * ob, c_end = std::min(sh.total, (k + 1) * R * ob);
    for (size_t c0 = c_begin; c0 < c_end; c0 += ob) {
      const size_t ncs = std::min(ob, c_end - c0);
      hipLaunchKernelGGL(leaf_absorb_kernel, dim3((unsigned)((ml + 255) / 256)), dim3(256), 0, P->hstream, plane_l + c0 * ml, ml, row_log, (u32)ncs,
                         P->d_sponge, c0 == 0 ? 1 : 0, c0 + ncs == sh.total ? 1 : 0, t.d,
                         (c0 + ncs < sh.total && sh.total - (c0 + ncs) >= 8) ? 1 : 0);
    }
    HIPC(hipGetLastError());
  }
  int rc = tree_build_inner(P, t, P->hstream);
  if (rc) return rc;
  HIPC(hipEventRecord(P->hash_done, P->hstream));
  HIPC(hipStreamWaitEvent(P->stream, P->hash_done, 0));
  return 0;
}
static int split_cap_to_host(sbn_prover* P, const DevTree& t, std::vector<u64>& cap) {
  SplitCtx* S = P->sp;
  const size_t capn = (size_t)1 << P->cfg.cap_height, own = capn >> S->log_r;
  std::vector<u64> mine(own * 4);
  HIPC(hipMemcpyAsync(mine.data(), t.level(t.nlevels), own * 4 * sizeof(u64), hipMemcpyDeviceToHost, P->stream));
  HIPC(stream_wait(P->stream));
  cap.resize(capn * 4);
  return split_all_gather_host(P, mine.data(), cap.data(), own * 4 * sizeof(u64));
}
static int absorb_times(sbn_prover* P, size_t ncols, int ex_ms) {
  size_t nchunks = (ncols + P->ntt_chunk - 1) / P->ntt_chunk;
  float tot = 0;
  for (size_t k = 0; k < nchunks; k++) { float ms = 0; HIPC(hipEventElapsedTime(&ms, P->abs_ev[2 * k], P->abs_ev[2 * k + 1])); tot += ms; }
  P->stage_ms[ST_COUNT + ex_ms] = tot;
  return 0;
}
static int tree_cap_to_host(sbn_prover* P, const DevTree& t, std::vector<u64>& cap, bool first_bad = false) {
  size_t capn = (size_t)1 << P->cfg.cap_height;
  cap.resize(capn * 4);
  HIPC(hipMemcpyAsync(cap.data(), t.level(t.nlevels), capn * 4 * sizeof(u64), hipMemcpyDeviceToHost, P->stream));
  if (first_bad) HIPC(hipMemcpyAsync(P->h_first_bad, P->d_first_bad, sizeof(unsigned long long), hipMemcpyDeviceToHost, P->stream));
  HIPC(stream_wait(P->stream));
  return 0;
}

static constexpr size_t SPLIT_BLOCK = 64;
static int split_sizes(const AirShape& as, u32 degree_bits, u32 rate_bits, u32 world, size_t ob, uint64_t* send_bytes, uint64_t* recv_bytes, size_t* scratch_words,
                       size_t* slot_words) {
  const size_t n = (size_t)1 << degree_bits, m = n << rate_bits;
  const u32 planes = world >= 4 ? 2 : 1;
  const size_t sw = std::max<size_t>(2 * m, 2 * n * world);
  const size_t slot = world > 1 ? (size_t)planes * ob * m : 0;
  *send_bytes = (uint64_t)(std::max(std::max(2 * slot, 2 * (m / world)), 2 * n) * sizeof(u64));
  *recv_bytes = (uint64_t)(((as.ncols + as.nzs) * (m / world) * planes + sw) * sizeof(u64));
  *scratch_words = sw;
  if (slot_words) *slot_words = slot;
  return 0;
}
static int create_ctx(const sbn_air_desc* air, const sbn_config* cfg, uint32_t degree_bits, const sbn_comm* comm, sbn_prover** out);
extern "C" int sbn_prover_create(const sbn_air_desc* air, const sbn_config* cfg, uint32_t degree_bits, sbn_prover** out) {
  return create_ctx(air, cfg, degree_bits, nullptr, out);
}
static int create_ctx(const sbn_air_desc* air, const sbn_config* cfg, uint32_t degree_bits, const sbn_comm* comm, sbn_prover** out) {
  if (!air || !cfg || !out) return fail(SBN_ERR_BAD_ARG, "null argument");
  *out = nullptr;
  if (!config_supported(cfg)) return fail(SBN_ERR_UNSUPPORTED, "unsupported StarkConfig (need num_challenges=2, rate_bits=1)");
  AirShape as;
  if (!air_shape(air, cfg, as)) return fail(SBN_ERR_BAD_ARG, "unknown air kind / num_io");
  if (degree_bits < 9 || degree_bits > 22) return fail(SBN_ERR_UNSUPPORTED, "degree_bits out of range");
  if (as.kind == SBN_AIR_FLAGS && (512 * (size_t)as.num_io) != ((size_t)1 << degree_bits)) return fail(SBN_ERR_BAD_ARG, "FlagStark needs 512*num_io rows");
  if (as.kind == SBN_AIR_FLAGS_U64 && (128 * (size_t)as.num_io) != ((size_t)1 << degree_bits)) return fail(SBN_ERR_BAD_ARG, "the u64 FlagStark needs 128*num_io rows");
  if (is_exp_air(as.kind)) {
    if ((exp_rows_per_instance(as.kind) * as.num_io) != ((size_t)1 << degree_bits)) return fail(SBN_ERR_BAD_ARG, "the Exp tables need 512*num_io rows (FQ12_EXP_U64: 128*num_io)");
    if (as.kind != SBN_AIR_FQ12_EXP && as.kind != SBN_AIR_FQ12_EXP_U64 && degree_bits < 16)
      return fail(SBN_ERR_UNSUPPORTED, "G1_EXP / G2_EXP / FQ_EXP need >= 2^16 rows (u16 range check, range_check.rs:26)");
  }
  if (int rc = use_current_device("the prover path has no CPU fallback")) return rc;
  sbn_prover* P = new sbn_prover();
  P->air = as; P->cfg = *cfg; P->degree_bits = degree_bits; P->lde_log = degree_bits + cfg->rate_bits;
  P->n = (size_t)1 << degree_bits; P->m = (size_t)1 << P->lde_log;
  P->fri = fri_shape(*cfg, degree_bits);
  P->device = g_device;
  int rc = 0;
  auto acc = [&](int r) { if (!rc) rc = r; };
  auto hipc = [&](hipError_t e, const char* what) { if (e != hipSuccess && !rc) rc = fail(SBN_ERR_HIP, "%s failed: %s", what, hipGetErrorString(e)); };
  if (P->fri.total_arity() > degree_bits + cfg->rate_bits - cfg->cap_height) { sbn_prover_destroy(P); return fail(SBN_ERR_UNSUPPORTED, "FRI total reduction arity is too large"); }
  P->ntt_chunk = P->lde_log >= 18 ? 48 : 64;
  {
    std::string serr;
    if (!P->set.load(serr)) { sbn_prover_destroy(P); return fail(SBN_ERR_BAD_ARG, "%s", serr.c_str()); }
  }
  const Settings& set = P->set;
  if (set.ntt_chunk) P->ntt_chunk = (size_t)set.ntt_chunk;
  ntt_plan(P);
  if (P->ntt_fused512 && !set.ntt_chunk) P->ntt_chunk = 40;
  P->chain_mode = set.device_chain >= 0 ? set.device_chain : ((tracegen_host_chains_vectorized() || tracegen_host_threads() >= 8) ? 0 : 2);
  acc(ntt_fast_setup());
  hipc(hipStreamCreate(&P->stream), "hipStreamCreate");
  hipc(hipStreamCreate(&P->hstream), "hipStreamCreate");
  P->ntt_two_streams = P->lde_log >= 19;
  if (P->ntt_two_streams) {
    hipc(hipStreamCreate(&P->nstream), "hipStreamCreate");
    for (auto& e : P->intt_done) hipc(hipEventCreateWithFlags(&e, hipEventDisableTiming), "hipEventCreate");
  }
  for (auto& e : P->ev) hipc(hipEventCreate(&e), "hipEventCreate");
  for (auto& e : P->abs_ev) hipc(hipEventCreate(&e), "hipEventCreate");
  for (auto& e : P->chunk_ready) hipc(hipEventCreateWithFlags(&e, hipEventDisableTiming), "hipEventCreate");
  hipc(hipEventCreateWithFlags(&P->hash_done, hipEventDisableTiming), "hipEventCreate");
  for (auto& v : P->stage_ms) v = 0;
  if (rc) { sbn_prover_destroy(P); return rc; }
  const size_t n = P->n, m = P->m, C = as.ncols, Z = as.nzs;
  if (comm && (C <= 4 || Z == 0)) { sbn_prover_destroy(P); return fail(SBN_ERR_UNSUPPORTED, "the split prover covers the wide tables (this one has %zu columns and %zu permutation Zs)", C, Z); }
  if (comm) {
    const u32 R = comm->world;
    u32 lr = 0; while ((1u << lr) < R) lr++;
    uint64_t sb = 0, rb = 0; size_t sw = 0, slotw = 0;
    if (comm->struct_size != sizeof(sbn_comm)) { sbn_prover_destroy(P); return fail(SBN_ERR_BAD_ARG, "sbn_comm.struct_size does not match this library (ABI %d)", SBN_ABI_VERSION); }
    if (!set.ntt_chunk) P->ntt_chunk = SPLIT_BLOCK;
    if (P->ntt_chunk != SPLIT_BLOCK) { sbn_prover_destroy(P); return fail(SBN_ERR_UNSUPPORTED, "the split prover deals columns in blocks of %zu: unset SBN_NTT_CHUNK", SPLIT_BLOCK); }
    split_sizes(as, degree_bits, cfg->rate_bits, R, SPLIT_BLOCK, &sb, &rb, &sw, &slotw);
    if ((1u << lr) != R || lr > cfg->cap_height || comm->rank >= R || !comm->all_to_all || !comm->all_gather_host || !comm->send_buf || !comm->recv_buf ||
        comm->send_bytes < sb || comm->recv_bytes < rb) {
      sbn_prover_destroy(P);
      return fail(SBN_ERR_BAD_ARG, "bad sbn_comm (world must be a power of two <= 2^cap_height; staging buffers of sbn_split_exchange_bytes)");
    }
    for (const void* buf : {(const void*)comm->send_buf, (const void*)comm->recv_buf}) {
      hipPointerAttribute_t pa{};
      if (hipPointerGetAttributes(&pa, buf) != hipSuccess || pa.device != P->device) {
        (void)hipGetLastError();
        sbn_prover_destroy(P);
        return fail(SBN_ERR_BAD_ARG, "sbn_comm staging buffers do not live on this prover's device %d (call sbn_set_device before creating the transport)", g_device);
      }
    }
    SplitCtx* S = P->sp = new SplitCtx();
    for (auto& e : S->xchg_done) e = nullptr;
    S->comm = *comm; S->log_r = lr; S->rho = bitrev32(comm->rank, lr); S->ml = m >> lr; S->planes = R >= 4 ? 2 : 1;
    S->slot_words = slotw;
    S->cs.total = C; S->cs.ob = SPLIT_BLOCK; S->cs.R = R; S->cs.rank = comm->rank;
    S->zs = S->cs; S->zs.total = Z;
    S->cr = S->cs.own(); S->zr = S->zs.own();
    hipc(hipStreamCreate(&S->cstream), "hipStreamCreate");
    for (auto& e : S->xchg_done) hipc(hipEventCreateWithFlags(&e, hipEventDisableTiming), "hipEventCreate");
    S->tev.assign(2 * (2 * (S->cs.steps() + S->zs.steps()) + 8), nullptr);
    for (auto& e : S->tev) hipc(hipEventCreate(&e), "hipEventCreate");
    u64* rbuf = (u64*)comm->recv_buf;
    S->lde_l = rbuf; rbuf += C * S->ml;
    if (S->planes == 2) { S->lde_n = rbuf; rbuf += C * S->ml; }
    S->zlde_l = rbuf; rbuf += Z * S->ml;
    if (S->planes == 2) { S->zlde_n = rbuf; rbuf += Z * S->ml; }
    S->scratch = rbuf; S->scratch_words = sw;
    P->lde_scratch_words = (size_t)(rb / sizeof(u64));
    acc(dmalloc(&P->d_trace, C * n, &P->dev_bytes)); acc(dmalloc(&P->d_coef, std::max<size_t>(S->cr, 1) * n, &P->dev_bytes));
    acc(dmalloc(&P->d_zval, std::max<size_t>(S->zr, 1) * n, &P->dev_bytes)); acc(dmalloc(&P->d_zcoef, std::max<size_t>(S->zr, 1) * n, &P->dev_bytes));
    acc(dmalloc(&S->d_ldechunk, P->ntt_chunk * m, &P->dev_bytes));
    hipc(hipMalloc((void**)&S->d_idx_local, cfg->num_query_rounds * sizeof(u32)), "hipMalloc"); P->dev_bytes += cfg->num_query_rounds * sizeof(u32);
    acc(tree_alloc(P->tree_t, S->ml, cfg->cap_height - lr, &P->dev_bytes)); acc(tree_alloc(P->tree_z, S->ml, cfg->cap_height - lr, &P->dev_bytes));
  } else {
    P->lde_scratch_words = C * m;
    acc(dmalloc(&P->d_trace, C * n, &P->dev_bytes)); acc(dmalloc(&P->d_coef, C * n, &P->dev_bytes)); acc(dmalloc(&P->d_lde, C * m, &P->dev_bytes));
    acc(dmalloc(&P->d_zval, std::max<size_t>(Z, 1) * n, &P->dev_bytes)); acc(dmalloc(&P->d_zcoef, std::max<size_t>(Z, 1) * n, &P->dev_bytes)); acc(dmalloc(&P->d_zlde, std::max<size_t>(Z, 1) * m, &P->dev_bytes));
    acc(tree_alloc(P->tree_t, m, cfg->cap_height, &P->dev_bytes)); acc(tree_alloc(P->tree_z, m, cfg->cap_height, &P->dev_bytes));
  }
  acc(dmalloc(&P->d_tmp, std::max(P->ntt_chunk, (size_t)4) * m, &P->dev_bytes));
  if (P->ntt_fused || P->ntt_fused512 || P->ntt_two_streams) acc(dmalloc(&P->d_tmp2, std::max(P->ntt_chunk, (size_t)4) * m, &P->dev_bytes));
  if ((P->ntt_fused || P->ntt_fused512) && P->ntt_two_streams) acc(dmalloc(&P->d_tmp3, std::max(P->ntt_chunk, (size_t)4) * m, &P->dev_bytes));
  acc(dmalloc(&P->d_q, 2 * m, &P->dev_bytes)); acc(dmalloc(&P->d_qlde, 4 * m, &P->dev_bytes));
  acc(tree_alloc(P->tree_q, m, cfg->cap_height, &P->dev_bytes));
  acc(dmalloc(&P->d_tw_f, m, &P->dev_bytes)); acc(dmalloc(&P->d_tw_i, m, &P->dev_bytes)); acc(dmalloc(&P->d_shift, m, &P->dev_bytes)); acc(dmalloc(&P->d_shift_inv, m, &P->dev_bytes));
  if (P->ntt_fused512) acc(dmalloc(&P->d_shift_odd, n, &P->dev_bytes));
  acc(dmalloc(&P->d_xs, m, &P->dev_bytes)); acc(dmalloc(&P->d_lag_first, m, &P->dev_bytes)); acc(dmalloc(&P->d_lag_last, m, &P->dev_bytes));
  P->apow_n = apow_len(as.nconstraints, as.nzs);
  acc(dmalloc(&P->d_apow, (size_t)SBN_NCH * P->apow_n, &P->dev_bytes));
  acc(dmalloc(&P->d_zpow, 4 * n, &P->dev_bytes)); acc(dmalloc(&P->d_open, (C + Z + 4) * 4, &P->dev_bytes));
  hipc(hipHostMalloc((void**)&P->h_open, (C + Z + 4) * 4 * sizeof(u64), hipHostMallocDefault), "hipHostMalloc");
  hipc(hipHostMalloc((void**)&P->h_open2, (C + Z) * 4 * sizeof(u64), hipHostMallocDefault), "hipHostMalloc");
  acc(dmalloc(&P->d_part, 2 * 32 * n, &P->dev_bytes)); acc(dmalloc(&P->d_w, 4096, &P->dev_bytes)); acc(dmalloc(&P->d_sponge, 12 * m, &P->dev_bytes));
  acc(dmalloc(&P->d_fa, 4 * n, &P->dev_bytes)); acc(dmalloc(&P->d_fcoef, 2 * m, &P->dev_bytes)); acc(dmalloc(&P->d_fcoef2, 2 * m, &P->dev_bytes));
  acc(dmalloc(&P->d_pow, 1, &P->dev_bytes));
  if (rc) { sbn_prover_destroy(P); return rc; }
  P->d_fb = P->d_fa + 2 * n;
  hipc(hipMalloc((void**)&P->d_pic, sizeof(ExpPiConsts<F>)), "hipMalloc"); P->dev_bytes += sizeof(ExpPiConsts<F>);
  hipc(hipMalloc((void**)&P->d_idx, cfg->num_query_rounds * sizeof(u32)), "hipMalloc"); P->dev_bytes += cfg->num_query_rounds * sizeof(u32);
  {
    u32 bits = P->lde_log;
    for (u32 ab : P->fri.arity_bits) {
      u64* v = nullptr; acc(dmalloc(&v, 2 * ((size_t)1 << bits), &P->dev_bytes)); P->fri_vals.push_back(v);
      DevTree t; acc(tree_alloc(t, (size_t)1 << (bits - ab), cfg->cap_height, &P->dev_bytes)); P->fri_trees.push_back(t);
      bits -= ab;
    }
    if (rc) { sbn_prover_destroy(P); return rc; }
  }
  {
    size_t sib = (size_t)(P->lde_log - cfg->cap_height) * 4;
    size_t s = C + sib + (Z ? Z + sib : 0) + 4 + sib;
    u32 bits = P->lde_log;
    for (u32 ab : P->fri.arity_bits) { bits -= ab; s += 2 * ((size_t)1 << ab) + (size_t)(bits - cfg->cap_height) * 4; }
    P->qstride = s;
    acc(dmalloc(&P->d_qbuf, s * cfg->num_query_rounds, &P->dev_bytes));
    if (rc) { sbn_prover_destroy(P); return rc; }
  }
  auto blocks = [](size_t k) { return dim3((unsigned)((k + 255) / 256)); };
  F w = f_root_of_unity(P->lde_log);
  hipLaunchKernelGGL(pow_table_kernel, blocks(m), dim3(256), 0, P->stream, P->d_tw_f, m, w.v);
  hipLaunchKernelGGL(pow_table_kernel, blocks(m), dim3(256), 0, P->stream, P->d_tw_i, m, f_inv(w).v);
  hipLaunchKernelGGL(pow_table_kernel, blocks(m), dim3(256), 0, P->stream, P->d_shift, m, (u64)GL_GEN);
  hipLaunchKernelGGL(pow_table_kernel, blocks(m), dim3(256), 0, P->stream, P->d_shift_inv, m, f_inv(F(GL_GEN)).v);
  hipLaunchKernelGGL(domain_tables_kernel, blocks(m), dim3(256), 0, P->stream, P->d_xs, P->d_lag_first, P->d_lag_last, m, P->lde_log, degree_bits);
  if (P->d_shift_odd) hipLaunchKernelGGL(shift_odd_table_kernel, blocks(n), dim3(256), 0, P->stream, P->d_shift_odd, n, P->d_shift, P->d_tw_f, 9u);
  {
    std::vector<PairCols> pairs(Z);
    for (size_t z = 0; z < Z; z++) {
      int l, r;
      if (as.kind == SBN_AIR_G1_OP) G1OpShape::pair((int)z, l, r);
      else if (as.kind == SBN_AIR_LOOKUP) LookupShape().pair((int)z, l, r);
      else if (is_op_air(as.kind)) OpShape(as.kind).pair((int)z, l, r);
      else exp_shape(as).pair((int)z, l, r);
      pairs[z].lhs = l; pairs[z].rhs = r;
    }
    hipc(hipMalloc((void**)&P->d_pairs, std::max<size_t>(Z, 1) * sizeof(PairCols)), "hipMalloc"); P->dev_bytes += std::max<size_t>(Z, 1) * sizeof(PairCols);
    if (!rc && Z) hipc(hipMemcpy(P->d_pairs, pairs.data(), Z * sizeof(PairCols), hipMemcpyHostToDevice), "hipMemcpy");
    if (P->sp && P->sp->zr) {
      SplitCtx* S = P->sp;
      std::vector<PairCols> own(S->zr);
      for (size_t l = 0; l < S->zr; l++) own[l] = pairs[S->zs.global_col(S->zs.rank, l)];
      hipc(hipMalloc((void**)&S->d_pairs_own, S->zr * sizeof(PairCols)), "hipMalloc"); P->dev_bytes += S->zr * sizeof(PairCols);
      if (!rc) hipc(hipMemcpy(S->d_pairs_own, own.data(), S->zr * sizeof(PairCols), hipMemcpyHostToDevice), "hipMemcpy");
    }
  }
  hipc(hipStreamSynchronize(P->stream), "hipStreamSynchronize");
  hipc(hipGetLastError(), "table kernels");
  if (rc) { sbn_prover_destroy(P); return rc; }
  *out = P;
  return SBN_OK;
}

namespace sbn { size_t prover_device_bytes(const sbn_prover* P) { return P ? P->dev_bytes : 0; } }
extern "C" void sbn_prover_destroy(sbn_prover* P) {
  if (!P) return;
  (void)hipSetDevice(P->device);
  u64* bufs[] = {P->d_trace, P->d_coef, P->d_lde, P->d_tmp, P->d_tmp2, P->d_tmp3, P->d_zval, P->d_zcoef, P->d_zlde, P->d_q, P->d_qlde, P->tree_t.d, P->tree_z.d,
                 P->tree_q.d, P->d_tw_f, P->d_tw_i, P->d_shift, P->d_shift_inv, P->d_xs, P->d_lag_first, P->d_lag_last, P->d_apow, P->d_zpow,
                 P->d_open, P->d_part, P->d_w, P->d_fa, P->d_fcoef, P->d_fcoef2, P->d_pow, P->d_qbuf, P->d_shift_odd};
  for (u64* b : bufs) if (b) (void)hipFree(b);
  for (u64* b : P->fri_vals) if (b) (void)hipFree(b);
  for (auto& t : P->fri_trees) if (t.d) (void)hipFree(t.d);
  if (P->sp) {
    if (P->sp->d_ldechunk) (void)hipFree(P->sp->d_ldechunk);
    if (P->sp->d_idx_local) (void)hipFree(P->sp->d_idx_local);
    if (P->sp->d_pairs_own) (void)hipFree(P->sp->d_pairs_own);
    for (auto& e : P->sp->xchg_done) if (e) (void)hipEventDestroy(e);
    for (auto& e : P->sp->tev) if (e) (void)hipEventDestroy(e);
    if (P->sp->cstream) (void)hipStreamDestroy(P->sp->cstream);
    delete P->sp;
  }
  if (P->d_pic) (void)hipFree(P->d_pic);
  if (P->d_idx) (void)hipFree(P->d_idx);
  if (P->d_pairs) (void)hipFree(P->d_pairs);
  for (auto& e : P->ev) if (e) (void)hipEventDestroy(e);
  for (auto& e : P->abs_ev) if (e) (void)hipEventDestroy(e);
  for (auto& e : P->chunk_ready) if (e) (void)hipEventDestroy(e);
  if (P->hash_done) (void)hipEventDestroy(P->hash_done);
  if (P->d_sponge) (void)hipFree(P->d_sponge);
  if (P->h_chain) (void)hipHostFree(P->h_chain);
  if (P->h_io) (void)hipHostFree(P->h_io);
  if (P->h_open) (void)hipHostFree(P->h_open);
  if (P->h_open2) (void)hipHostFree(P->h_open2);
  if (P->ustream) (void)hipStreamSynchronize(P->ustream);
  for (auto& e : P->upload_done) if (e) (void)hipEventDestroy(e);
  for (auto& e : P->slot_copied) if (e) (void)hipEventDestroy(e);
  if (P->h_ring) (void)hipHostFree(P->h_ring);
  if (P->h_first_bad) (void)hipHostFree(P->h_first_bad);
  if (P->d_first_bad) (void)hipFree(P->d_first_bad);
  if (P->ustream) (void)hipStreamDestroy(P->ustream);
  if (P->hstream) (void)hipStreamDestroy(P->hstream);
  if (P->nstream) { (void)hipStreamDestroy(P->nstream); for (auto& e : P->intt_done) if (e) (void)hipEventDestroy(e); }
  if (P->stream) (void)hipStreamDestroy(P->stream);
  delete P;
}

static int check_pi(sbn_prover* P, const uint64_t* pi, size_t n_pi) {
  if (n_pi != P->air.npi) return fail(SBN_ERR_BAD_ARG, "expected %zu public inputs, got %zu", P->air.npi, n_pi);
  if (n_pi && !pi) return fail(SBN_ERR_BAD_ARG, "null public inputs");
  for (size_t i = 0; i < n_pi; i++) if (pi[i] >= GLP) return fail(SBN_ERR_NON_CANONICAL, "public input %zu is not canonical", i);
  P->pi.assign(pi, pi + n_pi);
  return 0;
}
extern "C" int sbn_prover_load_trace(sbn_prover* P, const uint64_t* trace, const uint64_t* pi, size_t n_pi) {
  if (!P || !trace) return fail(SBN_ERR_BAD_ARG, "null argument");
  int rc = check_pi(P, pi, n_pi); if (rc) return rc;
  size_t words = P->air.ncols * P->n;
  {
    unsigned nt = tracegen_host_threads(); if (nt == 0) nt = 1; if (nt > 16) nt = 16;
    std::atomic<size_t> bad(words);
    std::vector<std::thread> th;
    size_t per = (words + nt - 1) / nt;
    for (unsigned t = 0; t < nt; t++)
      th.emplace_back([&, t] {
        size_t a = t * per, b = std::min(words, a + per);
        for (size_t i = a; i < b; i++) if (trace[i] >= GLP) { size_t cur = bad.load(); while (i < cur && !bad.compare_exchange_weak(cur, i)) {} break; }
      });
    for (auto& x : th) x.join();
    if (bad.load() < words) return fail(SBN_ERR_NON_CANONICAL, "trace word %zu is not canonical", bad.load());
  }
  HIPC(hipSetDevice(P->device));
  HIPC(hipMemcpy(P->d_trace, trace, words * sizeof(u64), hipMemcpyHostToDevice));
  P->loaded = true;
  return SBN_OK;
}
extern "C" int sbn_prover_load_trace_device(sbn_prover* P, const uint64_t* d_trace, const uint64_t* pi, size_t n_pi) {
  if (!P || !d_trace) return fail(SBN_ERR_BAD_ARG, "null argument");
  int rc = check_pi(P, pi, n_pi); if (rc) return rc;
  HIPC(hipSetDevice(P->device));
  if (d_trace != P->d_trace) HIPC(hipMemcpy(P->d_trace, d_trace, P->air.ncols * P->n * sizeof(u64), hipMemcpyDeviceToDevice));
  P->loaded = true;
  return SBN_OK;
}

extern "C" int sbn_prover_read_trace(sbn_prover* P, uint64_t* out) {
  if (!P || !out) return fail(SBN_ERR_BAD_ARG, "null argument");
  if (!P->loaded) return fail(SBN_ERR_BAD_ARG, "no trace loaded");
  HIPC(hipSetDevice(P->device));
  HIPC(hipMemcpy(out, P->d_trace, P->air.ncols * P->n * sizeof(u64), hipMemcpyDeviceToHost));
  return SBN_OK;
}
extern "C" uint64_t* sbn_prover_trace_device_ptr(sbn_prover* P) {
  if (!P) return nullptr;
  (void)hipSetDevice(P->device);
  return P->d_trace;
}

extern "C" int sbn_prover_stage_times(const sbn_prover* P, float* ms, int cap) {
  if (!P || !ms) return 0;
  int k = std::min(cap, (int)(ST_COUNT + EX_COUNT));
  for (int i = 0; i < k; i++) ms[i] = P->stage_ms[i];
  return k;
}
extern "C" const char* sbn_prover_stage_name(int i) { return (i >= 0 && i < ST_COUNT + EX_COUNT) ? STAGE_NAMES[i] : ""; }

template <int KIND>
static void launch_quotient_kind(sbn_prover* P, const QuotientParams& qp, size_t qblocks) {
  const dim3 g1((unsigned)qblocks, 1), g2((unsigned)qblocks, 2);
  if (qp.seg_mask & 12u) hipLaunchKernelGGL((quotient_kernel<KIND, 2>), g2, dim3(256), 0, P->hstream, qp, qp.apow[0], qp.apow[1], qp.pic);
  if (qp.seg_mask & 1u) hipLaunchKernelGGL((quotient_kernel<KIND, 0>), g1, dim3(256), 0, P->stream, qp, qp.apow[0], qp.apow[1], qp.pic);
  if (qp.seg_mask & 2u) hipLaunchKernelGGL((quotient_kernel<KIND, 1>), g1, dim3(256), 0, P->stream, qp, qp.apow[0], qp.apow[1], qp.pic);
}
static int launch_quotient_parts(sbn_prover* P, const QuotientParams& qp, size_t qblocks) {
  switch (P->air.kind) {
    case SBN_AIR_G1_OP: launch_quotient_kind<1>(P, qp, qblocks); break;
    case SBN_AIR_G1_EXP: launch_quotient_kind<2>(P, qp, qblocks); break;
    case SBN_AIR_G2_EXP: launch_quotient_kind<3>(P, qp, qblocks); break;
    case SBN_AIR_FQ_EXP: launch_quotient_kind<5>(P, qp, qblocks); break;
    case SBN_AIR_FQ12_EXP_U64: launch_quotient_kind<6>(P, qp, qblocks); break;
    case SBN_AIR_MODULAR: launch_quotient_kind<7>(P, qp, qblocks); break;
    case SBN_AIR_FQ12_MUL: launch_quotient_kind<8>(P, qp, qblocks); break;
    case SBN_AIR_LOOKUP: launch_quotient_kind<9>(P, qp, qblocks); break;
    case SBN_AIR_FLAGS: launch_quotient_kind<10>(P, qp, qblocks); break;
    case SBN_AIR_FLAGS_U64: launch_quotient_kind<11>(P, qp, qblocks); break;
    default: launch_quotient_kind<4>(P, qp, qblocks); break;
  }
  HIPC(hipGetLastError());
  return 0;
}

static int prove_impl(sbn_prover* P, sbn_proof** out, const HostUpload* up) {
  if (!P || !out) return fail(SBN_ERR_BAD_ARG, "null argument");
  *out = nullptr;
  if (!up && !P->loaded && !(P->sp && P->sp->comm.world > 1)) return fail(SBN_ERR_BAD_ARG, "no trace loaded");
  HIPC(hipSetDevice(P->device));
  hipStream_t st = P->stream;
  const size_t n = P->n, m = P->m, C = P->air.ncols, Z = P->air.nzs;
  const sbn_config& cfg = P->cfg;
  const size_t capw = ((size_t)1 << cfg.cap_height) * 4;
  auto blocks = [](size_t k) { return dim3((unsigned)((k + 255) / 256)); };
  int rc;
  Challenger ch;
  std::vector<u64> trace_cap, z_cap, q_cap;

  HIPC(hipEventRecord(P->ev[ST_TRACE_COMMIT], st));
  SplitCtx* const S = P->sp;
  struct DeadlineScope { ~DeadlineScope() { t_wait_deadline_s = 0; } } deadline_scope;
  if (S && S->comm.world > 1) {
    t_wait_deadline_s = P->set.comm_timeout_s;
    std::vector<uint32_t> st_all(S->comm.world, 0);
    const uint32_t mine = P->loaded ? 1u : 0u;
    if ((rc = split_all_gather_host(P, &mine, st_all.data(), sizeof(uint32_t)))) return rc;
    for (u32 r = 0; r < S->comm.world; r++) if (!st_all[r]) return fail(SBN_ERR_BAD_ARG, "split proof abandoned: rank %u has no trace loaded", r);
  }
  if (!up && !P->loaded) return fail(SBN_ERR_BAD_ARG, "no trace loaded");
  if (up) HIPC(hipMemsetAsync(P->d_first_bad, 0xff, sizeof(unsigned long long), P->ustream));
  if (S) {
    S->tev_used = 0;
    if ((rc = commit_split(P, S->cs, P->d_trace, true, P->d_coef, S->lde_l, S->lde_n, P->tree_t))) return rc;
  } else if ((rc = commit_pipeline(P, P->d_trace, P->d_coef, P->d_lde, C, P->tree_t, EX_TRACE_ABSORB_MS, EX_TRACE_ABSORB_LAUNCHES, up))) return rc;
  HIPC(hipEventRecord(P->ev[ST_PERM_Z], st));
  if ((rc = S ? split_cap_to_host(P, P->tree_t, trace_cap) : tree_cap_to_host(P, P->tree_t, trace_cap, up != nullptr))) return rc;
  if (up && *P->h_first_bad != ~0ull) return fail(SBN_ERR_NON_CANONICAL, "trace word %zu is not canonical", (size_t)*P->h_first_bad);
  ch.observe_words(trace_cap.data(), capw);

  F gam[2][2] = {};
  if (Z) for (int s = 0; s < 2; s++) for (int c = 0; c < (int)cfg.num_challenges; c++) { (void)ch.challenge(); gam[s][c] = ch.challenge(); }
  const F gamma0 = gam[0][0], gamma1 = gam[1][1];
  {
    const size_t zn = S ? S->zr : Z;
    const PairCols* pairs = S ? S->d_pairs_own : P->d_pairs;
    auto launch_z = [&](size_t z0, size_t cnt, hipStream_t s) {
      if (cnt == 0) return;
      const PairCols* pp = pairs + z0; u64* out = P->d_zval + z0 * n;
      const size_t chunks = n / 2048;
      if (n >= 8192 && n % 2048 == 0 && cnt <= 65535 && cnt * chunks * 4 <= 2 * 32 * n) {
        u64* tot = P->d_part; u64* pq = P->d_part + cnt * chunks * 2;
        hipLaunchKernelGGL(permz_chunk_products_kernel<8>, dim3((unsigned)chunks, (unsigned)cnt), dim3(256), 0, s, P->d_trace, n, pp, gamma0.v, gamma1.v, tot);
        hipLaunchKernelGGL(permz_chunk_scan_kernel, dim3((unsigned)cnt), dim3(64), 0, s, tot, (u32)chunks, pq);
        hipLaunchKernelGGL(permz_chunk_write_kernel<8>, dim3((unsigned)chunks, (unsigned)cnt), dim3(256), 0, s, P->d_trace, n, pp, gamma0.v, gamma1.v, pq, out);
        return;
      }
      if (n % 2048 == 0) hipLaunchKernelGGL(permutation_z_kernel<8>, dim3((unsigned)cnt), dim3(256), 0, s, P->d_trace, n, pp, gamma0.v, gamma1.v, out);
      else if (n % 1024 == 0) hipLaunchKernelGGL(permutation_z_kernel<4>, dim3((unsigned)cnt), dim3(256), 0, s, P->d_trace, n, pp, gamma0.v, gamma1.v, out);
      else hipLaunchKernelGGL(permutation_z_kernel<2>, dim3((unsigned)cnt), dim3(256), 0, s, P->d_trace, n, pp, gamma0.v, gamma1.v, out);
    };
    launch_z(0, zn, st);
  }
  HIPC(hipGetLastError());
  HIPC(hipEventRecord(P->ev[ST_Z_COMMIT], st));
  if (S) {
    if ((rc = commit_split(P, S->zs, P->d_zval, false, P->d_zcoef, S->zlde_l, S->zlde_n, P->tree_z))) return rc;
  } else {
    if (C > 4) if ((rc = absorb_times(P, C, EX_TRACE_ABSORB_MS))) return rc;
    if (Z) if ((rc = commit_pipeline(P, P->d_zval, P->d_zcoef, P->d_zlde, Z, P->tree_z, EX_Z_ABSORB_MS, EX_Z_ABSORB_LAUNCHES))) return rc;
  }
  HIPC(hipEventRecord(P->ev[ST_QUOTIENT_EVAL], st));
  if (Z) {
    if ((rc = S ? split_cap_to_host(P, P->tree_z, z_cap) : tree_cap_to_host(P, P->tree_z, z_cap))) return rc;
    ch.observe_words(z_cap.data(), capw);
  }

  F alphas[SBN_NCH];
  for (int j = 0; j < SBN_NCH; j++) alphas[j] = ch.challenge();
  {
    const size_t APN = P->apow_n;
    std::vector<u64> apow((size_t)SBN_NCH * APN);
    std::vector<F> ap[SBN_NCH];
    for (int j = 0; j < SBN_NCH; j++) {
      ap[j].resize(APN);
      F a(1);
      for (size_t k = 0; k < APN; k++) { ap[j][k] = a; apow[(size_t)j * APN + k] = a.v; a = a * alphas[j]; }
    }
    HIPC(hipMemcpyAsync(P->d_apow, apow.data(), apow.size() * sizeof(u64), hipMemcpyHostToDevice, st));
    if (is_exp_air(P->air.kind)) {
      static thread_local ExpPiConsts<F> pic;
      const F* app[SBN_NCH] = {ap[0].data(), ap[1].data()};
      std::vector<F> pif(P->pi.size());
      for (size_t i = 0; i < pif.size(); i++) pif[i] = F(P->pi[i]);
      exp_pi_consts<F>(exp_shape(P->air), app, pif.data(), pic);
      HIPC(hipMemcpyAsync(P->d_pic, &pic, sizeof(pic), hipMemcpyHostToDevice, st));
    }
    HIPC(stream_wait(st));
  }
  {
    QuotientParams qp{};
    qp.lde = P->d_lde; qp.zlde = P->d_zlde; qp.m = m; qp.next_step = 2;
    qp.lde_next = qp.lde; qp.zlde_next = qp.zlde; qp.row_shift = 0; qp.row_rho = 0;
    if (S) {
      qp.lde = S->lde_l; qp.zlde = S->zlde_l; qp.m = S->ml; qp.row_shift = S->log_r; qp.row_rho = S->rho;
      qp.lde_next = S->planes == 2 ? S->lde_n : S->lde_l; qp.zlde_next = S->planes == 2 ? S->zlde_n : S->zlde_l;
      qp.next_step = S->comm.world == 1 ? 2 : (S->comm.world == 2 ? 1 : 0);
    }
    qp.xs = P->d_xs; qp.lag_first = P->d_lag_first; qp.lag_last = P->d_lag_last;
    F gn = f_exp_pow2(F(GL_GEN), P->degree_bits);
    qp.zh_inv[0] = f_inv(gn - F(1)).v; qp.zh_inv[1] = f_inv(-gn - F(1)).v;
    qp.last = f_inv(f_root_of_unity(P->degree_bits)).v;
    for (int j = 0; j < SBN_NCH; j++) { qp.alpha[j] = alphas[j].v; qp.apow[j] = P->d_apow + (size_t)j * P->apow_n; }
    qp.gamma0 = gamma0.v; qp.gamma1 = gamma1.v; qp.num_zs = (int)Z; qp.num_io = (int)P->air.num_io; qp.pic = P->d_pic; qp.qout = P->d_q;
    if (S) qp.qout = (u64*)S->comm.send_buf;
    qp.part = P->d_part;
    {
      qp.zsplit = (int)(Z / 2);
      qp.lookups_in_perm = P->set.quotient_lookups == 1;
      const u64 n_tail = is_exp_air(P->air.kind) ? (u64)ExpShape(exp_e(P->air.kind), (int)P->air.num_io).num_tail_constraints() : 0;
      const u64 after[4] = {n_tail + 2 * (u64)Z, 2 * (u64)Z, 0, 0};
      qp.seg_count[0] = (int)(P->air.nconstraints - n_tail); qp.seg_count[1] = (int)n_tail;
      qp.seg_count[2] = qp.seg_count[3] = 2 * (int)Z;
      for (int sgm = 0; sgm < 4; sgm++) for (int j = 0; j < SBN_NCH; j++) qp.seg_shift[sgm][j] = f_pow(alphas[j], after[sgm]).v;
    }
    const size_t qblocks = (qp.m + 255) / 256;
    qp.seg_mask = 0xfu;
#ifdef SBN_DIAG
    { const char* e = std::getenv("SBN_DIAG_QUOTIENT_SEGMASK"); if (e) qp.seg_mask = (u32)atoi(e) & 0xfu; }
    if (qp.seg_mask != 0xfu) HIPC(hipMemsetAsync(qp.part, 0, (size_t)QSEG * SBN_NCH * qp.m * sizeof(u64), st));
#endif
    HIPC(hipEventRecord(P->chunk_ready[3], st));
    HIPC(hipStreamWaitEvent(P->hstream, P->chunk_ready[3], 0));
    if ((rc = launch_quotient_parts(P, qp, qblocks))) return rc;
    HIPC(hipEventRecord(P->hash_done, P->hstream));
    HIPC(hipStreamWaitEvent(st, P->hash_done, 0));
    hipLaunchKernelGGL(quotient_combine_kernel, blocks(qp.m), dim3(256), 0, st, qp);
    HIPC(hipGetLastError());
    if (S) {
      if ((rc = split_all_gather_device(P, 2 * S->ml))) return rc;
      hipLaunchKernelGGL(split_unpack_rows_kernel, blocks(m), dim3(256), 0, st, S->scratch, m, 2u, S->log_r, P->d_q);
      HIPC(hipGetLastError());
    } else if (Z > 4) { if ((rc = absorb_times(P, Z, EX_Z_ABSORB_MS))) return rc; }
  }
  HIPC(hipEventRecord(P->ev[ST_QUOTIENT_COMMIT], st));
  if ((rc = ntt_columns(P, P->d_q, m, P->d_q, m, P->d_tmp, m, 2, P->lde_log, true, m, nullptr, P->d_shift_inv, host_inv_pow2(P->lde_log)))) return rc;
  if ((rc = lde_coeffs(P, P->d_q, P->d_qlde, 4))) return rc;
  if ((rc = tree_from_matrix(P, P->tree_q, P->d_qlde, 4))) return rc;
  HIPC(hipEventRecord(P->ev[ST_OPENINGS], st));
  if ((rc = tree_cap_to_host(P, P->tree_q, q_cap))) return rc;
  ch.observe_words(q_cap.data(), capw);

  E2 zeta = ch.ext_challenge();
  F g = f_root_of_unity(P->degree_bits);
  if (e2_exp_pow2(zeta, P->degree_bits) == E2(F(1), F(0))) return fail(SBN_ERR_HIP, "opening point is in the subgroup");
  E2 zeta_next = zeta * g;
  hipLaunchKernelGGL(ext_pow_table_kernel, blocks(n), dim3(256), 0, st, P->d_zpow, P->d_zpow + n, n, zeta.a.v, zeta.b.v);
  hipLaunchKernelGGL(ext_pow_table_kernel, blocks(n), dim3(256), 0, st, P->d_zpow + 2 * n, P->d_zpow + 3 * n, n, zeta_next.a.v, zeta_next.b.v);
  const u64* open = P->h_open;
  const u64* open2 = P->h_open2;
  if (S && S->comm.world > 1) {
    const u64 *zp0 = P->d_zpow, *zp1 = P->d_zpow + n, *zp2 = P->d_zpow + 2 * n, *zp3 = P->d_zpow + 3 * n;
    auto open_k = n % 1024 == 0 ? openings_kernel<4> : openings_kernel<1>;
    if (S->cr) hipLaunchKernelGGL(open_k, dim3((unsigned)S->cr), dim3(256), 0, st, P->d_coef, n, zp0, zp1, zp2, zp3, P->d_open);
    if (S->zr) hipLaunchKernelGGL(open_k, dim3((unsigned)S->zr), dim3(256), 0, st, P->d_zcoef, n, zp0, zp1, zp2, zp3, P->d_open + C * 4);
    hipLaunchKernelGGL(open_k, dim3(4), dim3(256), 0, st, P->d_q, n, zp0, zp1, zp2, zp3, P->d_open + (C + Z) * 4);
    HIPC(hipGetLastError());
    HIPC(hipMemcpyAsync(P->h_open, P->d_open, (C + Z + 4) * 4 * sizeof(u64), hipMemcpyDeviceToHost, st));
    HIPC(hipEventRecord(P->ev[ST_FRI_COMBINE], st));
    HIPC(stream_wait(st));
    const u32 R = S->comm.world;
    const size_t cmax = S->cs.max_own(), zmax = S->zs.max_own(), per = (cmax + zmax) * 4;
    std::vector<u64> mine(per, 0), all((size_t)R * per);
    memcpy(mine.data(), P->h_open, S->cr * 4 * sizeof(u64));
    memcpy(mine.data() + cmax * 4, P->h_open + C * 4, S->zr * 4 * sizeof(u64));
    if ((rc = split_all_gather_host(P, mine.data(), all.data(), per * sizeof(u64)))) return rc;
    for (u32 r = 0; r < R; r++) {
      const u64* src = all.data() + (size_t)r * per;
      for (size_t l = 0, cnt = S->cs.own_cols(r); l < cnt; l++) memcpy(P->h_open + S->cs.global_col(r, l) * 4, src + l * 4, 4 * sizeof(u64));
      for (size_t l = 0, cnt = S->zs.own_cols(r); l < cnt; l++) memcpy(P->h_open + (C + S->zs.global_col(r, l)) * 4, src + (cmax + l) * 4, 4 * sizeof(u64));
    }
    open2 = open;
    for (size_t p = 0; p < C + Z + 4; p++) { ch.observe(F(open[4 * p])); ch.observe(F(open[4 * p + 1])); }
    for (size_t p = 0; p < C + Z; p++) { ch.observe(F(open[4 * p + 2])); ch.observe(F(open[4 * p + 3])); }
  } else {
    const bool u4 = n % 1024 == 0;
    auto open1_k = u4 ? openings1_kernel<4> : openings1_kernel<1>;
    const u64 *zp0 = P->d_zpow, *zp1 = P->d_zpow + n, *zp2 = P->d_zpow + 2 * n, *zp3 = P->d_zpow + 3 * n;
    size_t sl[5] = {0, C / 16, C / 16 + C / 8, C / 16 + C / 8 + C / 4, C};
    for (int k = 0; k < 4; k++) {
      const size_t a = sl[k], cnt = sl[k + 1] - sl[k];
      if (cnt) {
        hipLaunchKernelGGL(open1_k, dim3((unsigned)cnt), dim3(256), 0, st, P->d_coef + a * n, n, zp0, zp1, P->d_open + a * 4, 0u);
        HIPC(hipMemcpyAsync(P->h_open + a * 4, P->d_open + a * 4, cnt * 4 * sizeof(u64), hipMemcpyDeviceToHost, st));
      }
      HIPC(hipEventRecord(P->chunk_ready[8 + k], st));
    }
    if (Z) hipLaunchKernelGGL(open1_k, dim3((unsigned)Z), dim3(256), 0, st, P->d_zcoef, n, zp0, zp1, P->d_open + C * 4, 0u);
    hipLaunchKernelGGL(open1_k, dim3(4), dim3(256), 0, st, P->d_q, n, zp0, zp1, P->d_open + (C + Z) * 4, 0u);
    HIPC(hipMemcpyAsync(P->h_open + C * 4, P->d_open + C * 4, (Z + 4) * 4 * sizeof(u64), hipMemcpyDeviceToHost, st));
    HIPC(hipEventRecord(P->chunk_ready[1], st));
    size_t sn[5] = {0, C / 4, C / 2, C / 2 + C / 4, C};
    for (int k = 0; k < 4; k++) {
      const size_t a = sn[k], cnt = sn[k + 1] - sn[k];
      if (cnt) {
        hipLaunchKernelGGL(open1_k, dim3((unsigned)cnt), dim3(256), 0, st, P->d_coef + a * n, n, zp2, zp3, P->d_open + a * 4, 2u);
        HIPC(hipMemcpyAsync(P->h_open2 + a * 4, P->d_open + a * 4, cnt * 4 * sizeof(u64), hipMemcpyDeviceToHost, st));
      }
      HIPC(hipEventRecord(P->chunk_ready[12 + k], st));
    }
    if (Z) hipLaunchKernelGGL(open1_k, dim3((unsigned)Z), dim3(256), 0, st, P->d_zcoef, n, zp2, zp3, P->d_open + C * 4, 2u);
    HIPC(hipGetLastError());
    HIPC(hipMemcpyAsync(P->h_open2 + C * 4, P->d_open + C * 4, Z * 4 * sizeof(u64), hipMemcpyDeviceToHost, st));
    HIPC(hipEventRecord(P->ev[ST_FRI_COMBINE], st));
    for (int k = 0; k < 4; k++) {
      HIPC(event_wait(P->chunk_ready[8 + k]));
      for (size_t p = sl[k]; p < sl[k + 1]; p++) { ch.observe(F(open[4 * p])); ch.observe(F(open[4 * p + 1])); }
    }
    HIPC(event_wait(P->chunk_ready[1]));
    for (size_t p = C; p < C + Z + 4; p++) { ch.observe(F(open[4 * p])); ch.observe(F(open[4 * p + 1])); }
    for (int k = 0; k < 4; k++) {
      HIPC(event_wait(P->chunk_ready[12 + k]));
      for (size_t p = sn[k]; p < sn[k + 1]; p++) { ch.observe(F(open2[4 * p + 2])); ch.observe(F(open2[4 * p + 3])); }
    }
    HIPC(stream_wait(st));
    for (size_t p = C; p < C + Z; p++) { ch.observe(F(open2[4 * p + 2])); ch.observe(F(open2[4 * p + 3])); }
  }

  E2 fri_alpha = ch.ext_challenge();
  {
    const u32 RW = S ? S->comm.world : 1;
    const u32 GS = RW > 1 ? (u32)SPLIT_BLOCK : 128;
    std::vector<u64> wall;
    auto plan = [&](u32 npoly, E2 weight0, u64 stride) { size_t off = wall.size(); u32 ng = (npoly + GS - 1) / GS; E2 ag = e2_pow(fri_alpha, stride), cur = weight0;
                                                         for (u32 k = 0; k < ng; k++) { wall.push_back(cur.a.v); wall.push_back(cur.b.v); cur = cur * ag; } return off; };
    const size_t tc0 = S ? (size_t)S->comm.rank * GS : 0, tcn = S ? S->cr : C, tzn = S ? S->zr : Z;
    const u64 gstride = (u64)GS * RW;
    size_t w_t = tcn ? plan((u32)tcn, e2_pow(fri_alpha, RW > 1 ? tc0 : 0), gstride) : 0, w_z = tzn ? plan((u32)tzn, e2_pow(fri_alpha, C + (RW > 1 ? tc0 : 0)), gstride) : 0,
           w_q = plan(4, e2_pow(fri_alpha, C + Z), GS);
    if (wall.size() > 4096) return fail(SBN_ERR_UNSUPPORTED, "too many FRI combine groups");
    HIPC(hipMemcpyAsync(P->d_w, wall.data(), wall.size() * sizeof(u64), hipMemcpyHostToDevice, st));
    hipLaunchKernelGGL(ext_pow_table_kernel, dim3(1), dim3(GS), 0, st, P->d_apow, P->d_apow + GS, (size_t)GS, fri_alpha.a.v, fri_alpha.b.v);
    auto combine = [&](const u64* coeffs, u32 npoly, size_t woff, u64* oa, u64* ob, int accumulate) -> int {
      u32 ng = (npoly + GS - 1) / GS;
      for (u32 g0 = 0; g0 < ng; g0 += 32) {
        u32 gc = std::min<u32>(32, ng - g0);
        hipLaunchKernelGGL(fri_combine_partial_kernel, dim3((unsigned)((n + 255) / 256), gc), dim3(256), 0, st, coeffs + (size_t)g0 * GS * n, n,
                           npoly - g0 * GS, GS, P->d_apow, P->d_apow + GS, P->d_part, P->d_part + 32 * n);
        hipLaunchKernelGGL(fri_combine_reduce_kernel, blocks(n), dim3(256), 0, st, P->d_part, P->d_part + 32 * n, n, gc, P->d_w + woff + 2 * g0, oa, ob,
                           (accumulate || g0 > 0) ? 1 : 0);
      }
      HIPC(hipGetLastError());
      return 0;
    };
    u64 *f1a = P->d_fb, *f1b = P->d_fb + n, *f0a = P->d_fa, *f0b = P->d_fa + n;
    if (!tcn) HIPC(hipMemsetAsync(f1a, 0, 2 * n * sizeof(u64), st));
    if (tcn) if ((rc = combine(P->d_coef, (u32)tcn, w_t, f1a, f1b, 0))) return rc;
    if (tzn) if ((rc = combine(P->d_zcoef, (u32)tzn, w_z, f1a, f1b, 1))) return rc;
    if (S) {
      HIPC(hipMemcpyAsync(S->comm.send_buf, f1a, 2 * n * sizeof(u64), hipMemcpyDeviceToDevice, st));
      if ((rc = split_all_gather_device(P, 2 * n))) return rc;
      hipLaunchKernelGGL(split_modadd_kernel, blocks(2 * n), dim3(256), 0, st, S->scratch, 2 * n, S->comm.world, f1a);
      HIPC(hipGetLastError());
    }
    HIPC(hipMemcpyAsync(f0a, f1a, 2 * n * sizeof(u64), hipMemcpyDeviceToDevice, st));
    if ((rc = combine(P->d_q, 4, w_q, f0a, f0b, 1))) return rc;
    HIPC(stream_wait(st));
    HIPC(hipMemsetAsync(P->d_fcoef, 0, 2 * m * sizeof(u64), st));
    E2 shift2 = e2_pow(fri_alpha, C + Z);
    auto divide = [&](const u64* ca, const u64* cb, E2 z, E2 mul, int accumulate) {
      const size_t nch = n / DBL_CHUNK;
      u64 *ha = P->d_part, *hb = P->d_part + nch;
      hipLaunchKernelGGL(divide_by_linear_pass1, blocks(nch), dim3(256), 0, st, ca, cb, nch, z.a.v, z.b.v, ha, hb);
      hipLaunchKernelGGL(divide_by_linear_pass2, dim3(1), dim3(256), 0, st, ha, hb, nch, z.a.v, z.b.v);
      hipLaunchKernelGGL(divide_by_linear_pass3, blocks(nch), dim3(256), 0, st, ca, cb, nch, z.a.v, z.b.v, ha, hb, mul.a.v, mul.b.v, P->d_fcoef, P->d_fcoef + m, accumulate, fri_times_x(cfg));
    };
    divide(f0a, f0b, zeta, E2{F(0), F(0)}, 0);
    divide(f1a, f1b, zeta_next, shift2, 1);
    HIPC(hipGetLastError());
  }
  HIPC(hipEventRecord(P->ev[ST_FRI_LAYERS], st));
  std::vector<std::vector<u64>> fri_caps;
  std::vector<u64> final_poly;
  {
    u32 bits = P->lde_log;
    u64* coef = P->d_fcoef; u64* coef_alt = P->d_fcoef2;
    size_t clen = m;
    F shift(GL_GEN);
    for (size_t li = 0; li < P->fri.arity_bits.size(); li++) {
      u32 ab = P->fri.arity_bits[li];
      u64* va = P->fri_vals[li]; u64* vb = va + clen;
      HIPC(hipMemcpyAsync(va, coef, 2 * clen * sizeof(u64), hipMemcpyDeviceToDevice, st));
      hipLaunchKernelGGL(scale_pow_kernel, blocks(clen), dim3(256), 0, st, va, clen, shift.v);
      hipLaunchKernelGGL(scale_pow_kernel, blocks(clen), dim3(256), 0, st, vb, clen, shift.v);
      if ((rc = ntt_columns(P, va, clen, va, clen, P->d_tmp, m, 2, bits, false, clen, nullptr, nullptr, 1))) return rc;
      DevTree& t = P->fri_trees[li];
      if (t.nleaf <= 16384) hipLaunchKernelGGL(fri_leaf_hash_coop_kernel, blocks(t.nleaf * 16), dim3(256), 0, st, va, vb, bits, ab, t.d);
      else hipLaunchKernelGGL(fri_leaf_hash_kernel, blocks(t.nleaf), dim3(256), 0, st, va, vb, bits, ab, t.d);
      if ((rc = tree_build_inner(P, t, st))) return rc;
      std::vector<u64> cap;
      if ((rc = tree_cap_to_host(P, t, cap))) return rc;
      ch.observe_words(cap.data(), capw);
      fri_caps.push_back(cap);
      E2 beta = ch.ext_challenge();
      size_t nout = clen >> ab;
      hipLaunchKernelGGL(fri_fold_kernel, blocks(nout), dim3(256), 0, st, coef, coef + clen, nout, 1u << ab, beta.a.v, beta.b.v, coef_alt, coef_alt + nout);
      HIPC(hipGetLastError());
      std::swap(coef, coef_alt);
      clen = nout; bits -= ab;
      shift = f_pow(shift, (u64)1 << ab);
    }
    size_t fl = clen >> cfg.rate_bits;
    final_poly.resize(2 * fl);
    std::vector<u64> fa(fl), fb(fl);
    HIPC(hipMemcpyAsync(fa.data(), coef, fl * sizeof(u64), hipMemcpyDeviceToHost, st));
    HIPC(hipMemcpyAsync(fb.data(), coef + clen, fl * sizeof(u64), hipMemcpyDeviceToHost, st));
    HIPC(stream_wait(st));
    for (size_t i = 0; i < fl; i++) { final_poly[2 * i] = fa[i]; final_poly[2 * i + 1] = fb[i]; ch.observe(F(fa[i])); ch.observe(F(fb[i])); }
  }
  HIPC(hipEventRecord(P->ev[ST_POW], st));
  u64 pow_witness = ~0ULL;
  {
    PowParams pp{};
    for (int i = 0; i < 12; i++) pp.state[i] = ch.st[i].v;
    for (size_t i = 0; i < ch.in.size(); i++) pp.state[i] = ch.in[i].v;
    pp.wpos = (u32)ch.in.size(); pp.min_lz = cfg.proof_of_work_bits; pp.result = P->d_pow;
    u64 base = 0;
    for (int round = 0; pow_witness == ~0ULL; round++) {
      const u64 BATCH = round == 0 ? (1ULL << 17) : (1ULL << 20);
      if (base >= GLP - BATCH) return fail(SBN_ERR_HIP, "proof of work failed");
      u64 init = ~0ULL;
      HIPC(hipMemcpyAsync(P->d_pow, &init, sizeof(u64), hipMemcpyHostToDevice, st));
      pp.base = base; pp.count = BATCH;
      hipLaunchKernelGGL(pow_kernel, blocks(BATCH), dim3(256), 0, st, pp);
      HIPC(hipMemcpyAsync(&pow_witness, P->d_pow, sizeof(u64), hipMemcpyDeviceToHost, st));
      HIPC(stream_wait(st));
      base += BATCH;
    }
    ch.observe(F(pow_witness));
    F resp = ch.challenge();
    u32 lz = resp.v ? (u32)__builtin_clzll(resp.v) : 64;
    if (lz < cfg.proof_of_work_bits) return fail(SBN_ERR_HIP, "proof-of-work witness check failed");
  }
  HIPC(hipEventRecord(P->ev[ST_QUERIES], st));
  const u32 nq = cfg.num_query_rounds;
  std::vector<u64> qwords(P->qstride * nq);
  std::vector<u32> idx(nq), idx_local(nq);
  size_t split_section = 0;
  {
    for (u32 q = 0; q < nq; q++) idx[q] = (u32)(ch.challenge().v % m);
    HIPC(hipMemcpyAsync(P->d_idx, idx.data(), nq * sizeof(u32), hipMemcpyHostToDevice, st));
    size_t off = 0;
    const u32 nsib = P->lde_log - cfg.cap_height;
    auto initial = [&](const u64* mat, size_t ncols, const DevTree& t, size_t rows, u32 log_rows, const u32* d_index) {
      hipLaunchKernelGGL(gather_rows_kernel, dim3((unsigned)((ncols + 255) / 256), nq), dim3(256), 0, st, mat, rows, log_rows, (u32)ncols, d_index, P->d_qbuf, P->qstride, off);
      off += ncols;
      hipLaunchKernelGGL(gather_siblings_kernel, dim3(nq), dim3(128), 0, st, t.d, t.nleaf, nsib, d_index, 0u, P->d_qbuf, P->qstride, off);
      off += (size_t)nsib * 4;
    };
    if (S) {
      for (u32 q = 0; q < nq; q++) idx_local[q] = idx[q] & (u32)(S->ml - 1);
      HIPC(hipMemcpyAsync(S->d_idx_local, idx_local.data(), nq * sizeof(u32), hipMemcpyHostToDevice, st));
      initial(S->lde_l, C, P->tree_t, S->ml, P->lde_log - S->log_r, S->d_idx_local);
      if (Z) initial(S->zlde_l, Z, P->tree_z, S->ml, P->lde_log - S->log_r, S->d_idx_local);
      split_section = off;
    } else {
      initial(P->d_lde, C, P->tree_t, m, P->lde_log, P->d_idx);
      if (Z) initial(P->d_zlde, Z, P->tree_z, m, P->lde_log, P->d_idx);
    }
    initial(P->d_qlde, 4, P->tree_q, m, P->lde_log, P->d_idx);
    u32 bits = P->lde_log, shift = 0;
    for (size_t li = 0; li < P->fri.arity_bits.size(); li++) {
      u32 ab = P->fri.arity_bits[li];
      shift += ab;
      size_t len = (size_t)1 << bits;
      hipLaunchKernelGGL(gather_fri_leaf_kernel, dim3(nq), dim3(64), 0, st, P->fri_vals[li], P->fri_vals[li] + len, bits, ab, P->d_idx, shift, P->d_qbuf, P->qstride, off);
      off += 2 * ((size_t)1 << ab);
      const DevTree& t = P->fri_trees[li];
      hipLaunchKernelGGL(gather_siblings_kernel, dim3(nq), dim3(128), 0, st, t.d, t.nleaf, t.nlevels, P->d_idx, shift, P->d_qbuf, P->qstride, off);
      off += (size_t)t.nlevels * 4;
      bits -= ab;
    }
    HIPC(hipGetLastError());
    if (off != P->qstride) return fail(SBN_ERR_HIP, "internal: query layout mismatch (%zu vs %zu)", off, P->qstride);
    HIPC(hipMemcpyAsync(qwords.data(), P->d_qbuf, qwords.size() * sizeof(u64), hipMemcpyDeviceToHost, st));
  }
  HIPC(hipEventRecord(P->ev[ST_COUNT], st));
  HIPC(stream_wait(st));
  for (int i = 0; i < ST_COUNT; i++) HIPC(hipEventElapsedTime(&P->stage_ms[i], P->ev[i], P->ev[i + 1]));
  if (S) {
    const u32 R = S->comm.world;
    std::vector<u64> mine((size_t)nq * split_section), all((size_t)R * nq * split_section);
    for (u32 q = 0; q < nq; q++) memcpy(mine.data() + (size_t)q * split_section, qwords.data() + (size_t)q * P->qstride, split_section * sizeof(u64));
    if ((rc = split_all_gather_host(P, mine.data(), all.data(), mine.size() * sizeof(u64)))) return rc;
    for (u32 q = 0; q < nq; q++) {
      const u32 owner = idx[q] >> (P->lde_log - S->log_r);
      memcpy(qwords.data() + (size_t)q * P->qstride, all.data() + ((size_t)owner * nq + q) * split_section, split_section * sizeof(u64));
    }
    float xms = 0;
    for (size_t i = 0; i + 1 < S->tev_used; i += 2) { float t = 0; HIPC(hipEventElapsedTime(&t, S->tev[i], S->tev[i + 1])); xms += t; }
    P->stage_ms[ST_COUNT + EX_COMM_MS] = xms;
  }

  sbn_proof* pr = new sbn_proof();
  pr->degree_bits = P->degree_bits;
  std::vector<u64>& w = pr->words;
  w.reserve(12 + 3 * capw + (C + Z + 4) * 4 + fri_caps.size() * capw + qwords.size() + final_poly.size() + 1 + P->pi.size());
  u64 hdr[12] = {PROOF_MAGIC, P->degree_bits, C, Z, 4, P->pi.size(), cfg.cap_height, cfg.rate_bits, fri_caps.size(), cfg.fri_arity_bits,
                 final_poly.size() / 2, nq};
  w.insert(w.end(), hdr, hdr + 12);
  w.insert(w.end(), trace_cap.begin(), trace_cap.end());
  if (Z) w.insert(w.end(), z_cap.begin(), z_cap.end());
  w.insert(w.end(), q_cap.begin(), q_cap.end());
  for (size_t p = 0; p < C; p++) { w.push_back(open[4 * p]); w.push_back(open[4 * p + 1]); }
  for (size_t p = 0; p < C; p++) { w.push_back(open2[4 * p + 2]); w.push_back(open2[4 * p + 3]); }
  for (size_t p = C; p < C + Z; p++) { w.push_back(open[4 * p]); w.push_back(open[4 * p + 1]); }
  for (size_t p = C; p < C + Z; p++) { w.push_back(open2[4 * p + 2]); w.push_back(open2[4 * p + 3]); }
  for (size_t p = C + Z; p < C + Z + 4; p++) { w.push_back(open[4 * p]); w.push_back(open[4 * p + 1]); }
  for (auto& cap : fri_caps) w.insert(w.end(), cap.begin(), cap.end());
  w.insert(w.end(), qwords.begin(), qwords.end());
  w.insert(w.end(), final_poly.begin(), final_poly.end());
  w.push_back(pow_witness);
  w.insert(w.end(), P->pi.begin(), P->pi.end());
  *out = pr;
  return SBN_OK;
}
extern "C" int sbn_prover_prove(sbn_prover* P, sbn_proof** out) { return prove_impl(P, out, nullptr); }

extern "C" int sbn_prover_prove_host_trace(sbn_prover* P, const uint64_t* trace, const uint64_t* pi, size_t n_pi, sbn_proof** out) {
  if (!P || !out) return fail(SBN_ERR_BAD_ARG, "null argument");
  *out = nullptr;
  P->loaded = false;
  if (!trace) return fail(SBN_ERR_BAD_ARG, "null argument");
  if (P->sp) return fail(SBN_ERR_UNSUPPORTED, "sbn_prover_prove_host_trace covers single-GPU provers");
  int rc = check_pi(P, pi, n_pi); if (rc) return rc;
  HIPC(hipSetDevice(P->device));
  if ((rc = upload_setup(P))) return rc;
  const HostUpload up{trace, P->upload_done};
  if ((rc = prove_impl(P, out, &up))) {
    for (hipStream_t s : {P->ustream, P->stream, P->hstream, P->nstream}) if (s) (void)hipStreamSynchronize(s);
    return rc;
  }
  P->loaded = true;
  return SBN_OK;
}

extern "C" int sbn_commit_values(const uint64_t* cols, size_t ncols, size_t n, uint32_t rate_bits, uint32_t cap_height, uint64_t* cap_out,
                                 uint64_t* coeffs_out, uint64_t* lde_out) {
  if (!cols || !cap_out || ncols == 0) return fail(SBN_ERR_BAD_ARG, "null argument");
  if (rate_bits != 1 || n < 512 || (n & (n - 1))) return fail(SBN_ERR_UNSUPPORTED, "need rate_bits=1 and n a power of two >= 512");
  u32 lg = 0; while (((size_t)1 << lg) < n) lg++;
  if (cap_height < 1 || cap_height > 8) return fail(SBN_ERR_UNSUPPORTED, "cap_height must be 1..8");
  sbn_prover P{};
  sbn_standard_fast_config(&P.cfg); P.cfg.cap_height = cap_height;
  P.degree_bits = lg; P.lde_log = lg + 1; P.n = n; P.m = 2 * n; P.ntt_chunk = 64; P.device = g_device;
  if (int rc = use_current_device("no CPU fallback")) return rc;
  { int rc0 = ntt_fast_setup(); if (rc0) return rc0; }
  { std::string serr; if (!P.set.load(serr)) return fail(SBN_ERR_BAD_ARG, "%s", serr.c_str()); }
  ntt_plan(&P);
  HIPC(hipStreamCreate(&P.stream));
  u64 *d_vals = nullptr, *d_coef = nullptr, *d_lde = nullptr;
  int rc = 0;
  rc |= dmalloc(&d_vals, ncols * n); rc |= dmalloc(&d_coef, ncols * n); rc |= dmalloc(&d_lde, ncols * P.m); rc |= dmalloc(&P.d_tmp, 64 * P.m);
  if (P.ntt_fused || P.ntt_fused512) rc |= dmalloc(&P.d_tmp2, 64 * P.m);
  if (P.ntt_fused512) rc |= dmalloc(&P.d_shift_odd, n);
  rc |= dmalloc(&P.d_tw_f, P.m); rc |= dmalloc(&P.d_tw_i, P.m); rc |= dmalloc(&P.d_shift, P.m);
  rc |= tree_alloc(P.tree_t, P.m, cap_height);
  if (!rc) {
    auto blocks = [](size_t k) { return dim3((unsigned)((k + 255) / 256)); };
    F w = f_root_of_unity(P.lde_log);
    hipLaunchKernelGGL(pow_table_kernel, blocks(P.m), dim3(256), 0, P.stream, P.d_tw_f, P.m, w.v);
    hipLaunchKernelGGL(pow_table_kernel, blocks(P.m), dim3(256), 0, P.stream, P.d_tw_i, P.m, f_inv(w).v);
    hipLaunchKernelGGL(pow_table_kernel, blocks(P.m), dim3(256), 0, P.stream, P.d_shift, P.m, (u64)GL_GEN);
    if (P.d_shift_odd) hipLaunchKernelGGL(shift_odd_table_kernel, blocks(n), dim3(256), 0, P.stream, P.d_shift_odd, n, P.d_shift, P.d_tw_f, 9u);
    if (hipMemcpy(d_vals, cols, ncols * n * sizeof(u64), hipMemcpyHostToDevice) != hipSuccess) rc = fail(SBN_ERR_HIP, "H2D failed");
  }
  for (size_t c0 = 0; !rc && c0 < ncols; c0 += P.ntt_chunk) rc = intt_lde_cols(&P, d_vals + c0 * n, d_coef + c0 * n, d_lde + c0 * P.m, std::min(P.ntt_chunk, ncols - c0));
  if (!rc && ncols <= 4) rc = tree_from_matrix(&P, P.tree_t, d_lde, ncols);
  if (!rc && ncols > 4) {
    rc = dmalloc(&P.d_sponge, 12 * P.m);
    for (size_t c0 = 0; !rc && c0 < ncols; c0 += 64) {
      size_t nc = std::min<size_t>(64, ncols - c0);
      hipLaunchKernelGGL(leaf_absorb_kernel, dim3((unsigned)((P.m + 255) / 256)), dim3(256), 0, P.stream, d_lde + c0 * P.m, P.m, P.lde_log, (u32)nc, P.d_sponge,
                         c0 == 0 ? 1 : 0, c0 + 64 >= ncols ? 1 : 0, P.tree_t.d, (c0 + 64 < ncols && ncols - (c0 + 64) >= 8) ? 1 : 0);
    }
    if (!rc) rc = tree_build_inner(&P, P.tree_t, P.stream);
  }
  std::vector<u64> cap;
  if (!rc) rc = tree_cap_to_host(&P, P.tree_t, cap);
  if (!rc) memcpy(cap_out, cap.data(), cap.size() * sizeof(u64));
  if (!rc && coeffs_out && hipMemcpy(coeffs_out, d_coef, ncols * n * sizeof(u64), hipMemcpyDeviceToHost) != hipSuccess) rc = fail(SBN_ERR_HIP, "D2H failed");
  if (!rc && lde_out && hipMemcpy(lde_out, d_lde, ncols * P.m * sizeof(u64), hipMemcpyDeviceToHost) != hipSuccess) rc = fail(SBN_ERR_HIP, "D2H failed");
  for (u64* b : {d_vals, d_coef, d_lde, P.d_tmp, P.d_tmp2, P.d_shift_odd, P.d_tw_f, P.d_tw_i, P.d_shift, P.tree_t.d, P.d_sponge}) if (b) (void)hipFree(b);
  (void)hipStreamDestroy(P.stream);
  return rc;
}

extern "C" int sbn_poseidon_permute_batch(uint64_t* states, size_t count) {
  if (!states) return fail(SBN_ERR_BAD_ARG, "null argument");
  if (int rc = use_current_device("no CPU fallback")) return rc;
  for (size_t i = 0; i < count * 12; i++) if (states[i] >= GLP) return fail(SBN_ERR_NON_CANONICAL, "state word %zu is not canonical", i);
  u64* d = nullptr;
  HIPC(hipMalloc((void**)&d, count * 12 * sizeof(u64)));
  HIPC(hipMemcpy(d, states, count * 12 * sizeof(u64), hipMemcpyHostToDevice));
  hipLaunchKernelGGL(poseidon_batch_kernel, dim3((unsigned)((count + 255) / 256)), dim3(256), 0, 0, d, count);
  HIPC(hipMemcpy(states, d, count * 12 * sizeof(u64), hipMemcpyDeviceToHost));
  (void)hipFree(d);
  return SBN_OK;
}

extern "C" int sbn_field_mul_batch(const uint64_t* a, const uint64_t* b, uint64_t* out, size_t count, int mode) {
  if (!a || !b || !out) return fail(SBN_ERR_BAD_ARG, "null argument");
  if (int rc = use_current_device("no CPU fallback")) return rc;
  if (count == 0) return SBN_OK;
  u64* d = nullptr;
  HIPC(hipMalloc((void**)&d, 3 * count * sizeof(u64)));
  hipError_t e = hipMemcpy(d, a, count * sizeof(u64), hipMemcpyHostToDevice);
  if (e == hipSuccess) e = hipMemcpy(d + count, b, count * sizeof(u64), hipMemcpyHostToDevice);
  if (e == hipSuccess) {
    hipLaunchKernelGGL(field_mul_batch_kernel, dim3((unsigned)((count + 255) / 256)), dim3(256), 0, 0, d, d + count, d + 2 * count, count, mode);
    e = hipMemcpy(out, d + 2 * count, count * sizeof(u64), hipMemcpyDeviceToHost);
  }
  (void)hipFree(d);
  if (e != hipSuccess) return fail(SBN_ERR_HIP, "sbn_field_mul_batch: %s", hipGetErrorString(e));
  return SBN_OK;
}


extern "C" int sbn_first_non_canonical(const uint64_t* words, size_t count, int on_device, uint64_t* index_out) {
  if (!index_out || (!words && count)) return fail(SBN_ERR_BAD_ARG, "null argument");
  *index_out = count;
  if (!on_device) {
    for (size_t i = 0; i < count; i++) if (words[i] >= GLP) { *index_out = i; break; }
    return SBN_OK;
  }
  if (int rc = use_current_device("no CPU fallback")) return rc;
  if (count == 0) return SBN_OK;
  const size_t off = ((size_t)words & 8) ? 1 : 0;
  u64* d = nullptr;
  HIPC(hipMalloc((void**)&d, (2 + off + count) * sizeof(u64)));
  unsigned long long first = ~0ull;
  hipError_t e = hipMemset(d, 0xff, sizeof(u64));
  if (e == hipSuccess) e = hipMemcpy(d + 2 + off, words, count * sizeof(u64), hipMemcpyHostToDevice);
  if (e == hipSuccess) {
    launch_first_non_canonical(d + 2 + off, count, 0, (unsigned long long*)d, 0);
    e = hipGetLastError();
    if (e == hipSuccess) e = hipMemcpy(&first, d, sizeof first, hipMemcpyDeviceToHost);
  }
  (void)hipFree(d);
  if (e != hipSuccess) return fail(SBN_ERR_HIP, "sbn_first_non_canonical: %s", hipGetErrorString(e));
  if (first != ~0ull) *index_out = first;
  return SBN_OK;
}

extern "C" int sbn_poseidon_permute_host(uint64_t* states, size_t count, int use_definition) {
  if (!states) return fail(SBN_ERR_BAD_ARG, "null argument");
  for (size_t i = 0; i < count * 12; i++) if (states[i] >= GLP) return fail(SBN_ERR_NON_CANONICAL, "state word %zu is not canonical", i);
  for (size_t k = 0; k < count; k++) {
    F st[12];
    for (int i = 0; i < 12; i++) st[i] = F(states[12 * k + i]);
    if (use_definition) poseidon_permute_generic(st); else poseidon_permute(st);
    for (int i = 0; i < 12; i++) states[12 * k + i] = st[i].v;
  }
  return SBN_OK;
}

extern "C" int sbn_set_device(int device) {
  int ndev = 0;
  if (hipGetDeviceCount(&ndev) != hipSuccess || device < 0 || device >= ndev) return fail(SBN_ERR_NO_DEVICE, "device %d not available", device);
  HIPC(hipSetDevice(device));
  t_device = device; g_default_device.store(device);
  return SBN_OK;
}
extern "C" int sbn_set_thread_device(int device) {
  int ndev = 0;
  if (hipGetDeviceCount(&ndev) != hipSuccess || device < 0 || device >= ndev) return fail(SBN_ERR_NO_DEVICE, "device %d not available", device);
  HIPC(hipSetDevice(device));
  t_device = device;
  return SBN_OK;
}
extern "C" int sbn_prover_describe(const sbn_prover* P, char* out, size_t cap) {
  if (!P || !out || cap == 0) return fail(SBN_ERR_BAD_ARG, "null argument");
  const Settings& s = P->set;
  static const char* const CH[] = {"host_pool", "device_lane", "device_wave"};
  const char* chain = P->chain_mode == 0 && tracegen_host_chains_vectorized() ? "host_pool_ifma_x8" : CH[P->chain_mode < 0 || P->chain_mode > 2 ? 0 : P->chain_mode];
  char buf[1024];
  snprintf(buf, sizeof buf,
           "abi=%d device=%d ntt_chunk=%zu ntt_fused=%d ntt_streams=%d ntt_split1024=%d "
           "curve_chains=%s host_threads=%u fq12_host_chain=%d fq12_row_kernel=%d range_check=%d quotient_lookups=%d comm_timeout_s=%g experimental=%d ignored=[%s]",
           SBN_ABI_VERSION, P->device, P->ntt_chunk, (int)(P->ntt_fused || P->ntt_fused512), P->ntt_two_streams ? 2 : 1, P->d_shift_odd ? 1 : 0,
           chain, tracegen_host_threads(), (int)s.fq12_host_chain,
           (int)s.fq12_row_kernel, s.range_check, s.quotient_lookups, s.comm_timeout_s, (int)s.experimental, s.ignored.c_str());
  snprintf(out, cap, "%s", buf);
  return SBN_OK;
}
extern "C" int sbn_device_count(void) { int n = 0; return hipGetDeviceCount(&n) == hipSuccess ? n : 0; }

struct sbn_split_prover { sbn_prover* P; };
extern "C" int sbn_split_exchange_bytes(const sbn_air_desc* air, const sbn_config* cfg, uint32_t degree_bits, uint32_t world, uint64_t* send_bytes,
                                        uint64_t* recv_bytes) {
  if (!air || !cfg || !send_bytes || !recv_bytes || world == 0) return fail(SBN_ERR_BAD_ARG, "null argument");
  AirShape as;
  if (!air_shape(air, cfg, as)) return fail(SBN_ERR_BAD_ARG, "unknown air kind / num_io");
  size_t sw;
  return split_sizes(as, degree_bits, cfg->rate_bits, world, SPLIT_BLOCK, send_bytes, recv_bytes, &sw, nullptr);
}
extern "C" int sbn_split_prover_create(const sbn_air_desc* air, const sbn_config* cfg, uint32_t degree_bits, const sbn_comm* comm, sbn_split_prover** out) {
  if (!out || !comm) return fail(SBN_ERR_BAD_ARG, "null argument");
  *out = nullptr;
  sbn_prover* P = nullptr;
  int rc = create_ctx(air, cfg, degree_bits, comm, &P);
  if (rc) return rc;
  *out = new sbn_split_prover{P};
  return SBN_OK;
}
extern "C" void sbn_split_prover_destroy(sbn_split_prover* sp) {
  if (!sp) return;
  sbn_prover_destroy(sp->P);
  delete sp;
}
extern "C" int sbn_split_prover_generate_trace(sbn_split_prover* sp, const uint32_t* ios, size_t num_io, uint64_t* pi_out) {
  if (!sp) return fail(SBN_ERR_BAD_ARG, "null argument");
  return sbn_prover_generate_trace(sp->P, ios, num_io, pi_out);
}
extern "C" int sbn_split_prover_load_trace(sbn_split_prover* sp, const uint64_t* trace, const uint64_t* pi, size_t n_pi) {
  if (!sp) return fail(SBN_ERR_BAD_ARG, "null argument");
  return sbn_prover_load_trace(sp->P, trace, pi, n_pi);
}
extern "C" int sbn_split_prover_prove(sbn_split_prover* sp, sbn_proof** out) {
  if (!sp) return fail(SBN_ERR_BAD_ARG, "null argument");
  return sbn_prover_prove(sp->P, out);
}
extern "C" int sbn_split_prover_stage_times(const sbn_split_prover* sp, float* ms_out, int cap) {
  if (!sp) return 0;
  return sbn_prover_stage_times(sp->P, ms_out, cap);
}
```

starky_bn254_amd/csrc/prover_ctx.hpp:

```cpp
#pragma once
#include "host_common.hpp"
#include "settings.hpp"
#include <algorithm>

using namespace sbn;
struct PairCols;

#define HIPC(expr)                                                                                   \
  do {                                                                                               \
    hipError_t e_ = (expr);                                                                          \
    if (e_ != hipSuccess) return fail(SBN_ERR_HIP, "%s failed: %s (%s:%d)", #expr, hipGetErrorString(e_), __FILE__, __LINE__); \
  } while (0)

enum Stage {
  ST_TRACE_COMMIT, ST_PERM_Z, ST_Z_COMMIT, ST_QUOTIENT_EVAL, ST_QUOTIENT_COMMIT,
  ST_OPENINGS, ST_FRI_COMBINE, ST_FRI_LAYERS, ST_POW, ST_QUERIES, ST_COUNT
};
enum Extra { EX_TRACE_ABSORB_MS, EX_TRACE_ABSORB_LAUNCHES, EX_Z_ABSORB_MS, EX_Z_ABSORB_LAUNCHES, EX_TRACEGEN_MS, EX_COMM_MS, EX_COUNT };
static constexpr int MAX_CHUNKS = 512;
static constexpr int UPLOAD_SLOTS = 4;
static constexpr size_t UPLOAD_SLOT_WORDS = (size_t)2 << 20;
static constexpr int SBN_MAX_DEVICES = 64;

struct DevTree {
  u64* d = nullptr; size_t nleaf = 0; u32 nlevels = 0;
  u64* level(u32 l) const { return d + (2 * nleaf - ((2 * nleaf) >> l)) * 4; }
};

struct ColShare {
  size_t total = 0, ob = 64; u32 R = 1, rank = 0;
  size_t nblocks() const { return (total + ob - 1) / ob; }
  size_t steps() const { return (nblocks() + R - 1) / R; }
  size_t block_cols(size_t b) const { return b < nblocks() ? std::min(ob, total - b * ob) : 0; }
  size_t own_cols(u32 r) const { size_t s = 0; for (size_t b = r; b < nblocks(); b += R) s += block_cols(b); return s; }
  size_t own() const { return own_cols(rank); }
  size_t max_own() const { size_t s = 0; for (u32 r = 0; r < R; r++) s = std::max(s, own_cols(r)); return s; }
  size_t global_col(u32 r, size_t local) const { return ((local / ob) * R + r) * ob + local % ob; }
};
struct SplitCtx {
  sbn_comm comm;
  u32 log_r = 0, rho = 0;
  size_t ml = 0;
  ColShare cs, zs;
  size_t cr = 0, zr = 0;
  u32 planes = 1;
  u64 *lde_l = nullptr, *lde_n = nullptr, *zlde_l = nullptr, *zlde_n = nullptr, *scratch = nullptr;
  size_t scratch_words = 0;
  size_t slot_words = 0;
  u64* d_ldechunk = nullptr;
  u32* d_idx_local = nullptr;
  PairCols* d_pairs_own = nullptr;
  hipStream_t cstream = nullptr;
  hipEvent_t xchg_done[MAX_CHUNKS];
  std::vector<hipEvent_t> tev;
  size_t tev_used = 0;
};

struct sbn_prover {
  AirShape air; sbn_config cfg; FriShape fri;
  SplitCtx* sp = nullptr;
  size_t lde_scratch_words = 0;
  u32 degree_bits, lde_log; size_t n, m;
  int device; hipStream_t stream;
  u64 *d_trace = nullptr, *d_coef = nullptr, *d_lde = nullptr, *d_tmp = nullptr;
  u64 *d_zval = nullptr, *d_zcoef = nullptr, *d_zlde = nullptr;
  u64 *d_q = nullptr, *d_qlde = nullptr;
  DevTree tree_t, tree_z, tree_q;
  std::vector<DevTree> fri_trees;
  u64 *d_tw_f = nullptr, *d_tw_i = nullptr, *d_shift = nullptr, *d_shift_inv = nullptr;
  u64 *d_shift_odd = nullptr;
  u64 *d_xs = nullptr, *d_lag_first = nullptr, *d_lag_last = nullptr;
  u64 *d_apow = nullptr;
  size_t apow_n = 0;
  void* d_pic = nullptr;
  PairCols* d_pairs = nullptr;
  u64 *d_zpow = nullptr;
  u64 *d_open = nullptr;
  u64 *d_part = nullptr;
  u64 *d_w = nullptr;
  u64 *d_fa = nullptr, *d_fb = nullptr;
  u64 *d_fcoef = nullptr;
  u64 *d_fcoef2 = nullptr;
  std::vector<u64*> fri_vals;
  u64 *d_pow = nullptr;
  u32 *d_idx = nullptr;
  u64 *d_qbuf = nullptr; size_t qstride = 0;
  std::vector<u64> pi;
  bool loaded = false;
  hipEvent_t ev[ST_COUNT + 1];
  float stage_ms[ST_COUNT + EX_COUNT];
  size_t ntt_chunk;
  bool ntt_fused = false;
  u64* d_tmp2 = nullptr;
  u64* d_tmp3 = nullptr;
  bool ntt_fused512 = false;
  hipStream_t hstream = nullptr;
  hipStream_t nstream = nullptr;
  hipEvent_t intt_done[MAX_CHUNKS];
  bool ntt_two_streams = false;
  Settings set;
  int chain_mode = 0;
  hipEvent_t chunk_ready[MAX_CHUNKS];
  hipEvent_t abs_ev[2 * MAX_CHUNKS];
  hipEvent_t hash_done;
  u64* d_sponge = nullptr;
  u64* h_chain = nullptr;
  size_t h_chain_words = 0;
  u64* h_io = nullptr;
  size_t h_io_words = 0;
  u64* h_open = nullptr;
  u64* h_open2 = nullptr;
  size_t dev_bytes = 0;
  hipStream_t ustream = nullptr;
  hipEvent_t upload_done[MAX_CHUNKS];
  hipEvent_t slot_copied[UPLOAD_SLOTS];
  bool slot_used[UPLOAD_SLOTS] = {};
  unsigned slot_next = 0;
  u64* h_ring = nullptr;
  unsigned long long* d_first_bad = nullptr;
  unsigned long long* h_first_bad = nullptr;
};
```

Before: 42.80.

## Fold inverse NTT scaling into a twiddle table and streamline fast-pass addressing

Adds a precomputed inverse-root table pre-multiplied by 1/n, so the inverse NTT's scale multiply folds into the twiddle multiply and the separate scale pass is dropped (including in the fused kernels). The fast-pass and fused NTT kernels switch to 32-bit byte-offset addressing with readfirstlane uniform bases, grouped loads and stores with scheduling barriers, and incremental twiddle index arithmetic. The first pass can also skip canonical reduction when the following fast pass consumes its output. It costs one extra table of memory and narrows the fast-path eligibility to cases where 32-bit offsets cannot overflow.

Measured after the change: 43.13, median of 6. Within noise of the previous version (+0.8%).

```diff
diff --git a/starky_bn254_amd/csrc/kernels.cuh b/starky_bn254_amd/csrc/kernels.cuh
--- a/starky_bn254_amd/csrc/kernels.cuh
+++ b/starky_bn254_amd/csrc/kernels.cuh
@@ -11,6 +11,10 @@
 __global__ void shift_odd_table_kernel(u64* out, size_t n, const u64* __restrict__ shift, const u64* __restrict__ tw, u32 log_s) {
   size_t i = (size_t)blockIdx.x * blockDim.x + threadIdx.x;
   if (i < n) out[i] = (F(shift[i]) * F(tw[(i >> log_s) << log_s])).v;
+}
+__global__ void scale_table_kernel(u64* out, size_t n, const u64* __restrict__ in, u64 scale) {
+  size_t i = (size_t)blockIdx.x * blockDim.x + threadIdx.x;
+  if (i < n) out[i] = (F(in[i]) * F(scale)).v;
 }
 __global__ void scale_pow_kernel(u64* v, size_t n, u64 base) {
   size_t i = (size_t)blockIdx.x * blockDim.x + threadIdx.x;
diff --git a/starky_bn254_amd/csrc/kernels_ntt.cuh b/starky_bn254_amd/csrc/kernels_ntt.cuh
--- a/starky_bn254_amd/csrc/kernels_ntt.cuh
+++ b/starky_bn254_amd/csrc/kernels_ntt.cuh
@@ -19,6 +19,8 @@
   const u64* pre2;
   u32 split;
   u32 xcd_order;
+  const u64* tw_x;
+  u32 weak_out;
 };
 
 GL_HD F tw_lookup(const u64* tw, u32 tw_log, u64 e_of_order, u32 order_log) {
@@ -162,48 +164,72 @@
 }
 
 #ifdef SBN_NTT_KERNELS_HERE
+__device__ __forceinline__ u64 ld_off(const u64* __restrict__ base, u32 byte_off) { return *(const u64*)((const char*)base + byte_off); }
+__device__ __forceinline__ void st_off(u64* __restrict__ base, u32 byte_off, u64 v) { *(u64*)((char*)base + byte_off) = v; }
+__device__ __forceinline__ u64 ld_off(const u64* __restrict__ base, u32 uni, u32 lane) { return ld_off((const u64*)((const char*)base + (u32)__builtin_amdgcn_readfirstlane(uni)), lane); }
+__device__ __forceinline__ void st_off(u64* __restrict__ base, u32 uni, u32 lane, u64 v) { st_off((u64*)((char*)base + (u32)__builtin_amdgcn_readfirstlane(uni)), lane, v); }
+#ifndef NTT_GRP
+#define NTT_GRP 4
+#endif
+#ifndef NTT_PGRP
+#define NTT_PGRP 4
+#endif
 template <int LOG_B>
-__global__ __launch_bounds__(256) void ntt_fast_pass_kernel(NttPassParams p, u32 kperm) {
+__device__ __forceinline__ void ntt_fast_pass_body(const NttPassParams& p, u32 kperm) {
   extern __shared__ u64 lds[];
   constexpr u32 NB = 1u << LOG_B;
-  constexpr u32 R = 256u << LOG_B;
   const size_t col = p.xcd_order ? blockIdx.x : blockIdx.y;
-  const size_t t0 = (size_t)(p.xcd_order ? blockIdx.y : blockIdx.x) << 4;
+  const u32 t0 = (p.xcd_order ? blockIdx.y : blockIdx.x) << 4;
   const u32 half = p.split ? blockIdx.z : 0u;
   const u64* __restrict__ pre = half ? p.pre2 : p.pre;
   const u64* in = p.in + col * p.in_col_stride;
   u64* out = p.out + col * p.out_col_stride;
   u32 g, t;
   if (p.r_fast_load) { g = threadIdx.x & 15; t = threadIdx.x >> 4; } else { t = threadIdx.x & 15; g = threadIdx.x >> 4; }
-  const size_t tg = t0 + t;
+  const u32 tg = t0 + t;
   const u32 S1 = p.r_fast_load ? 257u : 272u;
   const u32 lane_off = p.r_fast_load ? (t * 16) : t;
   const u32 g_mul = p.r_fast_load ? 1u : 16u;
+  const u32 tw_sh = p.tw_log + 3;
   u64 x[NB][16];
-#pragma unroll
-  for (u32 b = 0; b < NB; b++)
-#pragma unroll
-    for (u32 q = 0; q < 16; q++) {
-      u32 r = g + 16 * q + 256 * b;
-      size_t gi = (size_t)r * p.in_sr + tg * p.in_st;
-      u64 v = 0;
-      if (gi < p.n_in) {
-        v = in[gi];
-        if (pre) v = nw::mul(v, pre[gi]);
-      }
-      x[b][q] = v;
-    }
+  {
+    const u32 in_sr = (u32)p.in_sr, in_st = (u32)p.in_st, step = in_sr << 7, lim = (u32)p.n_in << 3;
+    const u32 off = (g * in_sr + tg * in_st) << 3;
+#pragma unroll
+    for (u32 b = 0; b < NB; b++) {
+      if (((256u * b * in_sr + t0 * in_st) << 3) < lim) {
+#pragma unroll
+        for (u32 q = 0; q < 16; q++) x[b][q] = ld_off(in, off + (q + 16 * b) * step);
+        if (pre) {
+          u32 off2 = off;
+          asm("" : "+v"(off2));
+#pragma unroll
+          for (u32 q0 = 0; q0 < 16; q0 += NTT_PGRP) {
+#pragma unroll
+            for (u32 q = q0; q < q0 + NTT_PGRP; q++) x[b][q] = nw::mul(x[b][q], ld_off(pre, off2 + (q + 16 * b) * step));
+            __builtin_amdgcn_sched_barrier(0);
+          }
+        }
+      } else {
+#pragma unroll
+        for (u32 q = 0; q < 16; q++) x[b][q] = 0;
+      }
+    }
+  }
+  __builtin_amdgcn_sched_barrier(0);
   if (LOG_B == 1) {
     const bool upper_zero = p.in_st == 1 && (size_t)256 * p.in_sr >= p.n_in;
+    const u32 woff = g << (tw_sh - 9), wstep = 16u << (tw_sh - 9);
 #pragma unroll
     for (u32 q = 0; q < 16; q++) {
-      u32 r = g + 16 * q;
       u64 a = x[0][q], bb = x[NB - 1][q];
-      u64 w = tw_full(p.tw, p.tw_log, r, 9);
+      u64 w = ld_off(p.tw, q * wstep, woff);
       if (upper_zero) { x[NB - 1][q] = nw::mul(a, w); }
       else { x[0][q] = nw::add(a, bb); x[NB - 1][q] = nw::mul(nw::sub(a, bb), w); }
     }
   }
+  const u32 gw = g << (tw_sh - 8);
+  const u32 lds_lane = lane_off + g * g_mul;
 #pragma unroll
   for (u32 b = 0; b < NB; b++) {
     nw::dft16_rho(x[b]);
@@ -212,34 +238,54 @@
       u32 m = __brev(pidx) >> 28;
       u32 k1 = (kperm * m) & 15;
       u64 v = x[b][pidx];
-      if (g && k1) v = nw::mul(v, tw_full(p.tw, p.tw_log, (u32)(g * k1), 8));
-      lds[(b * 16 + k1) * S1 + lane_off + g * g_mul] = v;
+      if (g && k1) v = nw::mul(v, ld_off(p.tw, __umul24(gw, k1)));
+      lds[(b * 16 + k1) * S1 + lds_lane] = v;
     }
   }
   __syncthreads();
   const u32 k1 = g;
+  const u32 out_sr = (u32)p.out_sr, tw_mask = (1u << tw_sh) - 8u;
 #pragma unroll
   for (u32 b = 0; b < NB; b++) {
 #pragma unroll
     for (u32 gp = 0; gp < 16; gp++) x[b][gp] = lds[(b * 16 + k1) * S1 + lane_off + gp * g_mul];
     nw::dft16_rho(x[b]);
-#pragma unroll
-    for (u32 pidx = 0; pidx < 16; pidx++) {
-      u32 m = __brev(pidx) >> 28;
-      u32 k2 = (kperm * m) & 15;
-      u32 k256 = k1 + 16 * k2;
-      u32 k = LOG_B == 0 ? k256 : (k256 * NB + b);
-      if (LOG_B == 1) k = (k << p.split) + half;
-      u64 v = x[b][pidx];
-      if (p.twiddle) v = nw::mul(v, tw_full(p.tw, p.tw_log, (u32)(k * tg), p.log_n));
-      if (p.scale != 1) v = nw::mul(v, p.scale);
-      size_t go = (size_t)k * p.out_sr + tg * p.out_st;
-      if (p.post) v = nw::mul(v, p.post[go]);
-      out[go] = nw::canon(v);
-    }
-  }
-  (void)R;
-}
+    __builtin_amdgcn_sched_barrier(0);
+    const u32 kl = (k1 * NB) << p.split;
+    const u32 o_lane = (kl * out_sr + tg * (u32)p.out_st) << 3;
+    const u32 tgw = (tg << (tw_sh - p.log_n)) & tw_mask;
+    const u32 e_lane = __umul24(kl, tgw), e_step = (tgw << (4 + LOG_B + p.split)) & tw_mask;
+    const u32 kb = (b << p.split) + half;
+    const u32 e_b = e_lane + kb * tgw;
+#define NTT_K2(pidx) ((kperm * (__brev(pidx) >> 28)) & 15)
+#define NTT_ROW_OFF(pidx) ((((((16 * NTT_K2(pidx)) * NB + b) << p.split) + half) * out_sr) << 3)
+#pragma unroll
+    for (u32 p0 = 0; p0 < 16; p0 += NTT_GRP) {
+      if (p.twiddle) {
+#pragma unroll
+        for (u32 pidx = p0; pidx < p0 + NTT_GRP; pidx++) x[b][pidx] = nw::mul(x[b][pidx], ld_off(p.tw_x, (e_b + __umul24(NTT_K2(pidx), e_step)) & tw_mask));
+      }
+      if (p.scale != 1) {
+#pragma unroll
+        for (u32 pidx = p0; pidx < p0 + NTT_GRP; pidx++) x[b][pidx] = nw::mul(x[b][pidx], p.scale);
+      }
+      if (p.post) {
+#pragma unroll
+        for (u32 pidx = p0; pidx < p0 + NTT_GRP; pidx++) { x[b][pidx] = nw::mul(x[b][pidx], ld_off(p.post, NTT_ROW_OFF(pidx), o_lane)); __builtin_amdgcn_sched_barrier(0); }
+      }
+      if (!p.weak_out) {
+#pragma unroll
+        for (u32 pidx = p0; pidx < p0 + NTT_GRP; pidx++) x[b][pidx] = nw::canon(x[b][pidx]);
+      }
+#pragma unroll
+      for (u32 pidx = p0; pidx < p0 + NTT_GRP; pidx++) st_off(out, NTT_ROW_OFF(pidx), o_lane, x[b][pidx]);
+      asm volatile("" ::: "memory");
+    }
+#undef NTT_ROW_OFF
+#undef NTT_K2
+  }
+}
+template <int LOG_B> __global__ __launch_bounds__(256) void ntt_fast_pass_kernel(NttPassParams p, u32 kperm) { ntt_fast_pass_body<LOG_B>(p, kperm); }
 #else
 template <int LOG_B> __global__ void ntt_fast_pass_kernel(NttPassParams p, u32 kperm);
 #endif
@@ -252,50 +298,57 @@
   u32 log_n;
   const u64* tw_i; const u64* tw_f; u32 tw_log;
   const u64* pre;
-  u64 scale;
   const u64* pre2;
 };
 #ifdef SBN_NTT_KERNELS_HERE
 __global__ __launch_bounds__(256) __attribute__((amdgpu_waves_per_eu(4))) void ntt_fused_inv_b_lde_a_kernel(NttFusedParams p) {
   extern __shared__ u64 lds[];
   const size_t col = blockIdx.x;
-  const size_t t0 = (size_t)blockIdx.y << 4;
+  const u32 t0 = blockIdx.y << 4;
   const u64* in = p.in + col * p.in_col_stride;
   u64* coef = p.coef + col * p.coef_col_stride;
   u64* out = p.out + col * p.out_col_stride;
   const u32 g = threadIdx.x & 15, t = threadIdx.x >> 4;
-  const size_t tg = t0 + t;
+  const u32 tg = t0 + t;
+  const u32 n1 = (u32)p.n1, row16 = n1 << 7;
+  const u32 tw_sh = p.tw_log + 3, tw_mask = (1u << tw_sh) - 8u;
+  const u32 gw = g << (tw_sh - 8);
   u64 x[2][16];
-#pragma unroll
-  for (u32 q = 0; q < 16; q++) x[0][q] = in[(size_t)(g + 16 * q) + tg * 256];
+  {
+    const u32 off = (g + tg * 256) << 3;
+#pragma unroll
+    for (u32 q = 0; q < 16; q++) x[0][q] = ld_off(in, off + q * 128);
+  }
   nw::dft16_rho(x[0]);
 #pragma unroll
   for (u32 pidx = 0; pidx < 16; pidx++) {
     const u32 m = __brev(pidx) >> 28, k1 = (11u * m) & 15;
     u64 v = x[0][pidx];
-    if (g && k1) v = nw::mul(v, tw_full(p.tw_i, p.tw_log, (u32)(g * k1), 8));
+    if (g && k1) v = nw::mul(v, ld_off(p.tw_i, __umul24(gw, k1)));
     lds[k1 * 257 + t * 16 + g] = v;
   }
   __syncthreads();
 #pragma unroll
   for (u32 gp = 0; gp < 16; gp++) x[0][gp] = lds[g * 257 + t * 16 + gp];
   nw::dft16_rho(x[0]);
+  const u32 c_lane = (g * n1 + tg) << 3;
   u64 a[16];
 #pragma unroll
   for (u32 pidx = 0; pidx < 16; pidx++) {
     const u32 m = __brev(pidx) >> 28, k2 = (11u * m) & 15;
-    const u32 k = g + 16 * k2;
-    const u64 v = nw::mul(x[0][pidx], p.scale);
-    coef[(size_t)k * p.n1 + tg] = nw::canon(v);
+    const u64 v = x[0][pidx];
+    st_off(coef, k2 * row16, c_lane, nw::canon(v));
     a[k2] = v;
   }
   __syncthreads();
-#pragma unroll
-  for (u32 q = 0; q < 16; q++) {
-    const u32 r = g + 16 * q;
-    const u64 v = nw::mul(a[q], p.pre[(size_t)r * p.n1 + tg]);
-    x[0][q] = v;
-    x[1][q] = nw::mul(v, tw_full(p.tw_f, p.tw_log, r, 9));
+  {
+    const u32 woff = g << (tw_sh - 9), wstep = 16u << (tw_sh - 9);
+#pragma unroll
+    for (u32 q = 0; q < 16; q++) {
+      const u64 v = nw::mul(a[q], ld_off(p.pre, q * row16, c_lane));
+      x[0][q] = v;
+      x[1][q] = nw::mul(v, ld_off(p.tw_f, q * wstep, woff));
+    }
   }
 #pragma unroll
   for (u32 b = 0; b < 2; b++) {
@@ -304,24 +357,27 @@
     for (u32 pidx = 0; pidx < 16; pidx++) {
       const u32 m = __brev(pidx) >> 28, k1 = (5u * m) & 15;
       u64 v = x[b][pidx];
-      if (g && k1) v = nw::mul(v, tw_full(p.tw_f, p.tw_log, (u32)(g * k1), 8));
+      if (g && k1) v = nw::mul(v, ld_off(p.tw_f, __umul24(gw, k1)));
       lds[(b * 16 + k1) * 272 + g * 17 + t] = v;
     }
   }
   __syncthreads();
   const u32 t2 = threadIdx.x & 15, k1o = threadIdx.x >> 4;
-  const size_t tg2 = t0 + t2;
+  const u32 tg2 = t0 + t2;
+  const u32 o_lane = (2 * k1o * n1 + tg2) << 3;
+  const u32 tgw = (tg2 << (tw_sh - p.log_n - 1)) & tw_mask;
+  const u32 e_lane = __umul24(2 * k1o, tgw), e_step = (tgw << 5) & tw_mask;
 #pragma unroll
   for (u32 b = 0; b < 2; b++) {
 #pragma unroll
     for (u32 gp = 0; gp < 16; gp++) x[b][gp] = lds[(b * 16 + k1o) * 272 + gp * 17 + t2];
     nw::dft16_rho(x[b]);
+    const u32 e_b = e_lane + b * tgw;
 #pragma unroll
     for (u32 pidx = 0; pidx < 16; pidx++) {
       const u32 m = __brev(pidx) >> 28, k2 = (5u * m) & 15;
-      const u32 k = (k1o + 16 * k2) * 2 + b;
-      const u64 v = nw::mul(x[b][pidx], tw_full(p.tw_f, p.tw_log, (u32)(k * tg2), p.log_n + 1));
-      out[(size_t)k * p.n1 + tg2] = nw::canon(v);
+      const u64 v = nw::mul(x[b][pidx], ld_off(p.tw_f, (e_b + __umul24(k2, e_step)) & tw_mask));
+      st_off(out, (32 * k2 + b) * (n1 << 3), o_lane, v);
     }
   }
 }
@@ -333,46 +389,58 @@
 __global__ __launch_bounds__(256) __attribute__((amdgpu_waves_per_eu(4))) void ntt_fused512_inv_b_lde_a_kernel(NttFusedParams p) {
   extern __shared__ u64 lds[];
   const size_t col = blockIdx.x;
-  const size_t t0 = (size_t)blockIdx.y << 4;
+  const u32 t0 = blockIdx.y << 4;
   const u64* in = p.in + col * p.in_col_stride;
   u64* coef = p.coef + col * p.coef_col_stride;
   u64* out = p.out + col * p.out_col_stride;
   const u32 g = threadIdx.x & 15, t = threadIdx.x >> 4;
-  const size_t tg = t0 + t;
+  const u32 tg = t0 + t;
+  const u32 tw_sh = p.tw_log + 3, tw_mask = (1u << tw_sh) - 8u;
   u64 x[2][16];
-#pragma unroll
-  for (u32 q0 = 0; q0 < 16; q0 += 8) {
-#pragma unroll
-    for (u32 q = q0; q < q0 + 8; q++) {
-      const u64 lo = in[(size_t)(g + 16 * q) + tg * 512], hi = in[(size_t)(g + 16 * q + 256) + tg * 512];
-      x[0][q] = nw::add(lo, hi);
-      x[1][q] = nw::mul(nw::sub(lo, hi), tw_full(p.tw_i, p.tw_log, g + 16 * q, 9));
-    }
-    asm volatile("" ::: "memory");
-  }
+  {
+    const u32 off = (g + tg * 512) << 3, woff = g << (tw_sh - 9), wstep = 16u << (tw_sh - 9);
+#pragma unroll
+    for (u32 q0 = 0; q0 < 16; q0 += 4) {
+#pragma unroll
+      for (u32 q = q0; q < q0 + 4; q++) {
+        const u64 lo = ld_off(in, off + q * 128), hi = ld_off(in, off + q * 128 + 2048);
+        x[0][q] = nw::add(lo, hi);
+        x[1][q] = nw::mul(nw::sub(lo, hi), ld_off(p.tw_i, woff + q * wstep));
+      }
+      __builtin_amdgcn_sched_barrier(0);
+    }
+  }
+  {
+    u32 g1 = g, t1 = t;
+    asm volatile("" : "+v"(g1), "+v"(t1));
+    const u32 gw = g1 << (tw_sh - 8);
+#pragma unroll
+    for (u32 b = 0; b < 2; b++) {
+      nw::dft16_rho(x[b]);
+#pragma unroll
+      for (u32 pidx = 0; pidx < 16; pidx++) {
+        const u32 m = __brev(pidx) >> 28, k1 = (11u * m) & 15;
+        u64 v = x[b][pidx];
+        if (g1 && k1) v = nw::mul(v, ld_off(p.tw_i, __umul24(gw, k1)));
+        lds[(b * 16 + k1) * 257 + t1 * 16 + g1] = v;
+      }
+    }
+  }
+  __syncthreads();
 #pragma unroll
   for (u32 b = 0; b < 2; b++) {
-    nw::dft16_rho(x[b]);
-#pragma unroll
-    for (u32 pidx = 0; pidx < 16; pidx++) {
-      const u32 m = __brev(pidx) >> 28, k1 = (11u * m) & 15;
-      u64 v = x[b][pidx];
-      if (g && k1) v = nw::mul(v, tw_full(p.tw_i, p.tw_log, (u32)(g * k1), 8));
-      lds[(b * 16 + k1) * 257 + t * 16 + g] = v;
-    }
-  }
-  __syncthreads();
-#pragma unroll
-  for (u32 b = 0; b < 2; b++) {
+    u32 g2 = g, t2c = t;
+    asm volatile("" : "+v"(g2), "+v"(t2c));
     u64 z[16];
 #pragma unroll
-    for (u32 gp = 0; gp < 16; gp++) z[gp] = lds[(b * 16 + g) * 257 + t * 16 + gp];
+    for (u32 gp = 0; gp < 16; gp++) z[gp] = lds[(b * 16 + g2) * 257 + t2c * 16 + gp];
     nw::dft16_rho(z);
+    const u32 c_lane = (g2 * 1024 + t0 + t2c) << 3;
 #pragma unroll
     for (u32 pidx = 0; pidx < 16; pidx++) {
       const u32 m = __brev(pidx) >> 28, k2 = (11u * m) & 15;
-      const u64 v = nw::mul(z[pidx], p.scale);
-      coef[(size_t)((g + 16 * k2) * 2 + b) * 512 + tg] = nw::canon(v);
+      const u64 v = z[pidx];
+      st_off(coef, (32 * k2 + b) * 4096, c_lane, nw::canon(v));
       x[b][k2] = v;
     }
     asm volatile("" ::: "memory");
@@ -383,30 +451,35 @@
     u32 t2 = threadIdx.x & 15, k1o = threadIdx.x >> 4;
     u32 gl = g, tl = t;
     asm volatile("" : "+v"(t2), "+v"(k1o), "+v"(gl), "+v"(tl));
-    const size_t tg2 = t0 + t2, tgl = t0 + tl;
+    const u32 tg2 = t0 + t2, tgl = t0 + tl;
     const u64* __restrict__ pre = h ? p.pre2 : p.pre;
-#pragma unroll
-    for (u32 b = 0; b < 2; b++)
-#pragma unroll
-      for (u32 q0 = 0; q0 < 16; q0 += 8) {
-#pragma unroll
-        for (u32 q = q0; q < q0 + 8; q++) {
-          const size_t ci = (size_t)(2 * (gl + 16 * q) + b) * 512 + tgl;
-          u64 c = x[b][q];
-          if (h) c = coef[ci];
-          x[b][q] = nw::mul(c, pre[ci]);
+    {
+      const u32 c_lane = (gl * 1024 + tgl) << 3;
+#pragma unroll
+      for (u32 b = 0; b < 2; b++)
+#pragma unroll
+        for (u32 q0 = 0; q0 < 16; q0 += 8) {
+#pragma unroll
+          for (u32 q = q0; q < q0 + 8; q++) {
+            u64 c = x[b][q];
+            if (h) c = ld_off(coef, (32 * q + b) * 4096, c_lane);
+            x[b][q] = nw::mul(c, ld_off(pre, (32 * q + b) * 4096, c_lane));
+          }
+          asm volatile("" ::: "memory");
         }
-        asm volatile("" ::: "memory");
-      }
-#pragma unroll
-    for (u32 b = 0; b < 2; b++) {
-      nw::dft16_rho(x[b]);
-#pragma unroll
-      for (u32 pidx = 0; pidx < 16; pidx++) {
-        const u32 m = __brev(pidx) >> 28, k1 = (5u * m) & 15;
-        u64 v = x[b][pidx];
-        if (gl && k1) v = nw::mul(v, tw_full(p.tw_f, p.tw_log, (u32)(gl * k1), 8));
-        lds[(b * 16 + k1) * 272 + gl * 17 + tl] = v;
+    }
+    {
+      const u32 gw = gl << (tw_sh - 8);
+#pragma unroll
+      for (u32 b = 0; b < 2; b++) {
+        nw::dft16_rho(x[b]);
+#pragma unroll
+        for (u32 pidx = 0; pidx < 16; pidx++) {
+          const u32 m = __brev(pidx) >> 28, k1 = (5u * m) & 15;
+          u64 v = x[b][pidx];
+          if (gl && k1) v = nw::mul(v, ld_off(p.tw_f, __umul24(gw, k1)));
+          lds[(b * 16 + k1) * 272 + gl * 17 + tl] = v;
+        }
       }
     }
     __syncthreads();
@@ -416,14 +489,17 @@
       for (u32 gp = 0; gp < 16; gp++) x[b][gp] = lds[(b * 16 + k1o) * 272 + gp * 17 + t2];
       nw::dft16_rho(x[b]);
     }
+    const u32 jw = k1o << (tw_sh - 9), jstep = 16u << (tw_sh - 9);
+    const u32 tgw = (tg2 << (tw_sh - 19)) & tw_mask;
+    const u32 e_lane = __umul24(2 * k1o + h, tgw), e_step = (tgw << 5) & tw_mask, e_512 = (tgw << 9) & tw_mask;
+    const u32 o_lane = ((2 * k1o + h) * 512 + tg2) << 3;
 #pragma unroll
     for (u32 pidx = 0; pidx < 16; pidx++) {
       const u32 m = __brev(pidx) >> 28, k2 = (5u * m) & 15;
-      const u32 j = k1o + 16 * k2;
-      const u64 e = x[0][pidx], o = nw::mul(x[1][pidx], tw_full(p.tw_f, p.tw_log, j, 9));
-      const u32 ka = 2 * j + h, kb = 2 * (j + 256) + h;
-      out[(size_t)ka * 512 + tg2] = nw::canon(nw::mul(nw::add(e, o), tw_full(p.tw_f, p.tw_log, (u32)(ka * tg2), 19)));
-      out[(size_t)kb * 512 + tg2] = nw::canon(nw::mul(nw::sub(e, o), tw_full(p.tw_f, p.tw_log, (u32)(kb * tg2), 19)));
+      const u64 e = x[0][pidx], o = nw::mul(x[1][pidx], ld_off(p.tw_f, k2 * jstep, jw));
+      const u32 ea = (e_lane + __umul24(k2, e_step)) & tw_mask;
+      st_off(out, k2 * (32 * 512 * 8), o_lane, nw::mul(nw::add(e, o), ld_off(p.tw_f, ea)));
+      st_off(out, k2 * (32 * 512 * 8) + 512 * 512 * 8, o_lane, nw::mul(nw::sub(e, o), ld_off(p.tw_f, (ea + e_512) & tw_mask)));
     }
     __syncthreads();
   }
diff --git a/starky_bn254_amd/csrc/prover.hip b/starky_bn254_amd/csrc/prover.hip
--- a/starky_bn254_amd/csrc/prover.hip
+++ b/starky_bn254_amd/csrc/prover.hip
@@ -41,6 +41,7 @@
   while (lt > 0 && ((size_t)(1u << log_r) * ((1u << lt) + 1) * 8) > 48 * 1024) lt--;
   return std::min(lt, log_s);
 }
+static u64 host_inv_pow2(u32 k) { return f_inv(F((u64)1 << k)).v; }
 static int ntt_columns(sbn_prover* P, const u64* in, size_t in_cs, u64* out, size_t out_cs, u64* tmp, size_t tmp_cs, size_t ncols,
                        u32 log_n, bool inverse, size_t n_in, const u64* pre, const u64* post, u64 scale, hipStream_t st = nullptr, int which = 3) {
   if (ncols == 0) return 0;
@@ -52,13 +53,13 @@
   a.log_r = log_n1; a.log_t = pick_log_t(log_n1, log_n2); a.log_n = log_n;
   a.in_sr = n2; a.in_st = 1; a.out_sr = n2; a.out_st = 1; a.n_in = n_in;
   a.r_fast_load = 0; a.twiddle = 1; a.tw = inverse ? P->d_tw_i : P->d_tw_f; a.tw_log = P->lde_log;
-  a.pre = pre; a.post = nullptr; a.scale = 1;
+  a.pre = pre; a.post = nullptr; a.scale = 1; a.tw_x = a.tw;
   NttPassParams b{};
   b.in = tmp; b.out = out; b.in_col_stride = tmp_cs; b.out_col_stride = out_cs;
   b.log_r = log_n2; b.log_t = pick_log_t(log_n2, log_n1); b.log_n = log_n;
   b.in_sr = 1; b.in_st = n2; b.out_sr = n1; b.out_st = 1; b.n_in = (size_t)1 << log_n;
   b.r_fast_load = 1; b.twiddle = 0; b.tw = a.tw; b.tw_log = P->lde_log;
-  b.pre = nullptr; b.post = post; b.scale = scale;
+  b.pre = nullptr; b.post = post; b.scale = scale; b.tw_x = b.tw;
   for (size_t c0 = 0; c0 < ncols; c0 += 32768) {
     size_t nc = std::min<size_t>(32768, ncols - c0);
     NttPassParams pa = a, pb = b;
@@ -67,8 +68,12 @@
     dim3 ga((unsigned)(n2 >> pa.log_t), (unsigned)nc), gb((unsigned)(n1 >> pb.log_t), (unsigned)nc);
     size_t la = ((size_t)1 << pa.log_r) * ((1u << pa.log_t) + 1) * 8, lb = ((size_t)1 << pb.log_r) * ((1u << pb.log_t) + 1) * 8;
     const u32 kperm = inverse ? 11u : 5u;
+    auto is_fast = [&](const NttPassParams& q) {
+      const bool whole_blocks = q.n_in >= ((size_t)1 << log_n) || (q.in_st == 1 && q.n_in % (256 * q.in_sr) == 0);
+      return q.log_t == 4 && (q.log_r == 8 || q.log_r == 9) && P->lde_log <= 21 && whole_blocks;
+    };
     auto launch = [&](NttPassParams q, dim3 grid, size_t lds_bytes) {
-      const bool fast = q.log_t == 4 && (q.log_r == 8 || q.log_r == 9);
+      const bool fast = is_fast(q);
       if (fast) { q.xcd_order = 1; std::swap(grid.x, grid.y); }
       if (fast && q.log_r == 8) hipLaunchKernelGGL(ntt_fast_pass_kernel<0>, grid, dim3(256), 16 * 272 * 8, st, q, kperm);
       else if (fast) hipLaunchKernelGGL(ntt_fast_pass_kernel<1>, grid, dim3(256), 32 * 272 * 8, st, q, kperm);
@@ -80,6 +85,10 @@
     if (split_a) { pa.log_r = 9; pa.log_t = 4; pa.split = 1; pa.pre2 = P->d_shift_odd; }
     ga = dim3((unsigned)(n2 >> pa.log_t), (unsigned)nc, split_a ? 2u : 1u); gb = dim3((unsigned)(n1 >> pb.log_t), (unsigned)nc);
     la = ((size_t)1 << pa.log_r) * ((1u << pa.log_t) + 1) * 8; lb = ((size_t)1 << pb.log_r) * ((1u << pb.log_t) + 1) * 8;
+    if (is_fast(pa)) {
+      if (inverse && log_n == P->degree_bits && scale == host_inv_pow2(log_n) && P->d_tw_is) { pa.tw_x = P->d_tw_is; pb.scale = 1; }
+      pa.weak_out = (which & 2) ? is_fast(pb) : 1;
+    }
     if (which & 1) launch(pa, ga, la);
     if (which & 2) launch(pb, gb, lb);
   }
@@ -87,7 +96,6 @@
   return 0;
 }
 
-static u64 host_inv_pow2(u32 k) { return f_inv(F((u64)1 << k)).v; }
 static int ntt_fast_setup() {
   static std::atomic<bool> done[SBN_MAX_DEVICES];
   const int d = g_device >= 0 && g_device < SBN_MAX_DEVICES ? g_device : 0;
@@ -140,7 +148,7 @@
   const u32 log_n1 = (P->degree_bits + 1) / 2;
   f.in = P->d_tmp; f.in_col_stride = P->m; f.coef = cf; f.coef_col_stride = P->n; f.out = tmp2; f.out_col_stride = P->m;
   f.n1 = (size_t)1 << log_n1; f.log_n = P->degree_bits; f.tw_i = P->d_tw_i; f.tw_f = P->d_tw_f; f.tw_log = P->lde_log; f.pre = P->d_shift; f.pre2 = P->d_shift_odd;
-  f.scale = host_inv_pow2(P->degree_bits);
+  if (!P->d_tw_is) return fail(SBN_ERR_UNSUPPORTED, "fused transform without the scaled inverse root table");
   if (P->ntt_fused512) hipLaunchKernelGGL(ntt_fused512_inv_b_lde_a_kernel, dim3((unsigned)nc, 32u), dim3(256), 32 * 272 * 8, P->stream, f);
   else hipLaunchKernelGGL(ntt_fused_inv_b_lde_a_kernel, dim3((unsigned)nc, (unsigned)(f.n1 >> 4)), dim3(256), 32 * 272 * 8, P->stream, f);
   if (lde_stream != P->stream) {
@@ -563,6 +571,7 @@
   acc(dmalloc(&P->d_q, 2 * m, &P->dev_bytes)); acc(dmalloc(&P->d_qlde, 4 * m, &P->dev_bytes));
   acc(tree_alloc(P->tree_q, m, cfg->cap_height, &P->dev_bytes));
   acc(dmalloc(&P->d_tw_f, m, &P->dev_bytes)); acc(dmalloc(&P->d_tw_i, m, &P->dev_bytes)); acc(dmalloc(&P->d_shift, m, &P->dev_bytes)); acc(dmalloc(&P->d_shift_inv, m, &P->dev_bytes));
+  acc(dmalloc(&P->d_tw_is, m, &P->dev_bytes));
   if (P->ntt_fused512) acc(dmalloc(&P->d_shift_odd, n, &P->dev_bytes));
   acc(dmalloc(&P->d_xs, m, &P->dev_bytes)); acc(dmalloc(&P->d_lag_first, m, &P->dev_bytes)); acc(dmalloc(&P->d_lag_last, m, &P->dev_bytes));
   P->apow_n = apow_len(as.nconstraints, as.nzs);
@@ -599,6 +608,7 @@
   F w = f_root_of_unity(P->lde_log);
   hipLaunchKernelGGL(pow_table_kernel, blocks(m), dim3(256), 0, P->stream, P->d_tw_f, m, w.v);
   hipLaunchKernelGGL(pow_table_kernel, blocks(m), dim3(256), 0, P->stream, P->d_tw_i, m, f_inv(w).v);
+  hipLaunchKernelGGL(scale_table_kernel, blocks(m), dim3(256), 0, P->stream, P->d_tw_is, m, P->d_tw_i, host_inv_pow2(degree_bits));
   hipLaunchKernelGGL(pow_table_kernel, blocks(m), dim3(256), 0, P->stream, P->d_shift, m, (u64)GL_GEN);
   hipLaunchKernelGGL(pow_table_kernel, blocks(m), dim3(256), 0, P->stream, P->d_shift_inv, m, f_inv(F(GL_GEN)).v);
   hipLaunchKernelGGL(domain_tables_kernel, blocks(m), dim3(256), 0, P->stream, P->d_xs, P->d_lag_first, P->d_lag_last, m, P->lde_log, degree_bits);
@@ -636,7 +646,7 @@
   (void)hipSetDevice(P->device);
   u64* bufs[] = {P->d_trace, P->d_coef, P->d_lde, P->d_tmp, P->d_tmp2, P->d_tmp3, P->d_zval, P->d_zcoef, P->d_zlde, P->d_q, P->d_qlde, P->tree_t.d, P->tree_z.d,
                  P->tree_q.d, P->d_tw_f, P->d_tw_i, P->d_shift, P->d_shift_inv, P->d_xs, P->d_lag_first, P->d_lag_last, P->d_apow, P->d_zpow,
-                 P->d_open, P->d_part, P->d_w, P->d_fa, P->d_fcoef, P->d_fcoef2, P->d_pow, P->d_qbuf, P->d_shift_odd};
+                 P->d_open, P->d_part, P->d_w, P->d_fa, P->d_fcoef, P->d_fcoef2, P->d_pow, P->d_qbuf, P->d_shift_odd, P->d_tw_is};
   for (u64* b : bufs) if (b) (void)hipFree(b);
   for (u64* b : P->fri_vals) if (b) (void)hipFree(b);
   for (auto& t : P->fri_trees) if (t.d) (void)hipFree(t.d);
@@ -1218,13 +1228,14 @@
   rc |= dmalloc(&d_vals, ncols * n); rc |= dmalloc(&d_coef, ncols * n); rc |= dmalloc(&d_lde, ncols * P.m); rc |= dmalloc(&P.d_tmp, 64 * P.m);
   if (P.ntt_fused || P.ntt_fused512) rc |= dmalloc(&P.d_tmp2, 64 * P.m);
   if (P.ntt_fused512) rc |= dmalloc(&P.d_shift_odd, n);
-  rc |= dmalloc(&P.d_tw_f, P.m); rc |= dmalloc(&P.d_tw_i, P.m); rc |= dmalloc(&P.d_shift, P.m);
+  rc |= dmalloc(&P.d_tw_f, P.m); rc |= dmalloc(&P.d_tw_i, P.m); rc |= dmalloc(&P.d_tw_is, P.m); rc |= dmalloc(&P.d_shift, P.m);
   rc |= tree_alloc(P.tree_t, P.m, cap_height);
   if (!rc) {
     auto blocks = [](size_t k) { return dim3((unsigned)((k + 255) / 256)); };
     F w = f_root_of_unity(P.lde_log);
     hipLaunchKernelGGL(pow_table_kernel, blocks(P.m), dim3(256), 0, P.stream, P.d_tw_f, P.m, w.v);
     hipLaunchKernelGGL(pow_table_kernel, blocks(P.m), dim3(256), 0, P.stream, P.d_tw_i, P.m, f_inv(w).v);
+    hipLaunchKernelGGL(scale_table_kernel, blocks(P.m), dim3(256), 0, P.stream, P.d_tw_is, P.m, P.d_tw_i, host_inv_pow2(P.degree_bits));
     hipLaunchKernelGGL(pow_table_kernel, blocks(P.m), dim3(256), 0, P.stream, P.d_shift, P.m, (u64)GL_GEN);
     if (P.d_shift_odd) hipLaunchKernelGGL(shift_odd_table_kernel, blocks(n), dim3(256), 0, P.stream, P.d_shift_odd, n, P.d_shift, P.d_tw_f, 9u);
     if (hipMemcpy(d_vals, cols, ncols * n * sizeof(u64), hipMemcpyHostToDevice) != hipSuccess) rc = fail(SBN_ERR_HIP, "H2D failed");
@@ -1245,7 +1256,7 @@
   if (!rc) memcpy(cap_out, cap.data(), cap.size() * sizeof(u64));
   if (!rc && coeffs_out && hipMemcpy(coeffs_out, d_coef, ncols * n * sizeof(u64), hipMemcpyDeviceToHost) != hipSuccess) rc = fail(SBN_ERR_HIP, "D2H failed");
   if (!rc && lde_out && hipMemcpy(lde_out, d_lde, ncols * P.m * sizeof(u64), hipMemcpyDeviceToHost) != hipSuccess) rc = fail(SBN_ERR_HIP, "D2H failed");
-  for (u64* b : {d_vals, d_coef, d_lde, P.d_tmp, P.d_tmp2, P.d_shift_odd, P.d_tw_f, P.d_tw_i, P.d_shift, P.tree_t.d, P.d_sponge}) if (b) (void)hipFree(b);
+  for (u64* b : {d_vals, d_coef, d_lde, P.d_tmp, P.d_tmp2, P.d_shift_odd, P.d_tw_f, P.d_tw_i, P.d_tw_is, P.d_shift, P.tree_t.d, P.d_sponge}) if (b) (void)hipFree(b);
   (void)hipStreamDestroy(P.stream);
   return rc;
 }
diff --git a/starky_bn254_amd/csrc/prover_ctx.hpp b/starky_bn254_amd/csrc/prover_ctx.hpp
--- a/starky_bn254_amd/csrc/prover_ctx.hpp
+++ b/starky_bn254_amd/csrc/prover_ctx.hpp
@@ -68,6 +68,7 @@
   DevTree tree_t, tree_z, tree_q;
   std::vector<DevTree> fri_trees;
   u64 *d_tw_f = nullptr, *d_tw_i = nullptr, *d_shift = nullptr, *d_shift_inv = nullptr;
+  u64 *d_tw_is = nullptr;
   u64 *d_shift_odd = nullptr;
   u64 *d_xs = nullptr, *d_lag_first = nullptr, *d_lag_last = nullptr;
   u64 *d_apow = nullptr;
```
